# NVIDIA-NeMo/NeMo

Measured on AMD Instinct MI355X. Metric: audio-sec/s training throughput, Conformer-CTC-Large @ 1/2/4/8 MI355X, higher is better.
Workload: dtype bf16; 1 GPU; Conformer-CTC-Large bf16, batch=32x20s synthetic 16 kHz clips per GPU, 1xMI355X (BASELINE.json configs[1]); global_batch=32, parallelism=dp1

## Files before the change

include/mi355x_asr.h:

```cpp
#ifndef MI355X_ASR_H
#define MI355X_ASR_H
#ifdef __cplusplus
extern "C" {
#endif

#define MI355X_DT_F32 0
#define MI355X_DT_BF16 1

enum {
  MI355X_EPI_STORE = 0,
  MI355X_EPI_SWISH_DROP = 1,
  MI355X_EPI_RESID = 2,
  MI355X_EPI_DSWISH = 3,
  MI355X_EPI_RELU_MASK = 4,
  MI355X_EPI_MUL_POS = 5,
  MI355X_EPI_SWISH_DROP_G = 6,
  MI355X_EPI_DSWISH_G = 7
};
typedef struct mi355x_gemm_desc {
  const void* A; const void* B; void* C;
  int M, N, K;
  long long lda, ldb, ldc;
  long long c_col_stride;
  int transA, transB;
  int in_dtype;
  int c_dtype;
  int batch, nb0;
  long long sA0, sA1, sB0, sB1, sC0, sC1;
  const void* bias;
  float alpha;
  int epilogue;
  int atomic;
  int splitk;
  const void* aux_in; int aux_in_dtype;
  void* aux_out; int aux_out_dtype;
  long long ldaux;
  unsigned drop_key, drop_threshold; float drop_scale;
  const void* row_len; int rows_per_b; int rows_inner;
  long long colsum_stride;
  void* colsum_out;
  const struct mi355x_conv_gather* gather;
  const struct mi355x_row_map* rowmap;
} mi355x_gemm_desc;
typedef struct mi355x_conv_gather {
  int nI, nJ, SI, SJ, C, si, sj, ntaps; int di[9], dj[9];
  int operand;
} mi355x_conv_gather;
typedef struct mi355x_row_map { int nI, nJ, OI, OJ, si, sj, oi, oj; } mi355x_row_map;
int mi355x_gemm(const mi355x_gemm_desc* desc, void* stream);
int mi355x_gemm_config(int key, int value);
int mi355x_gemm_plan(const mi355x_gemm_desc* desc, int out[8]);
int mi355x_gemm_grouped(const mi355x_gemm_desc* descs, int n, void* stream);

int mi355x_ffn_fwd(const void* y, long long ldy, const void* w1_packed, const void* b1, const void* w2_packed, const void* b2,
                   const void* x_resid, long long ldx, void* h, long long ldh, void* out, long long ldo, int M, int d_model,
                   int d_ff, float alpha, unsigned drop_in_key, unsigned drop_in_threshold, float drop_in_scale,
                   unsigned drop_res_key, unsigned drop_res_threshold, float drop_res_scale, void* stream);
int mi355x_ffn_bwd_dgrad(const void* df, long long lddf, const void* w2t_packed, const void* w1t_packed, const void* h,
                         long long ldh, void* dh, void* act, void* dy, long long lddy, int M, int d_model, int d_ff,
                         unsigned drop_in_key, unsigned drop_in_threshold, float drop_in_scale, void* stream);

typedef struct mi355x_ffn_pack_entry { const void* src; void* k512; void* kchunk; int d_ff; int is_w2; } mi355x_ffn_pack_entry;
int mi355x_ffn_pack(const void* table_dev, int n_entries, int max_d_ff, void* stream);

int mi355x_logmel_fwd(const void* audio, const void* audio_len, const void* window, int win, int hop, int n_fft,
                      const void* fb_start, const void* fb_len, const void* fb_off, const void* fb_w, int n_mels,
                      float preemph, float dither, unsigned seed, float log_guard, void* out, int B, int S, int T,
                      void* stream);
int mi355x_logmel_config(int variant);
int mi355x_feat_normalize(const void* x, const void* seq_len, void* y, int y_dtype, int B, int n_mels, int T,
                          int normalize, float pad_value, void* stream);

int mi355x_subsample_conv1_fwd(const void* mel , const void* w , const void* bias,
                               void* out , int out_dtype, const void* len0, const void* len1, int B, int F,
                               int T, int C, void* stream);
int mi355x_subsample_conv1_bwd(const void* dout, int dtype, const void* mel, const void* len0, void* dw, void* db, int B,
                               int F, int T, int C, void* scratch ,
                               long long scratch_elems, void* stream);
int mi355x_im2col_3x3s2(const void* in , void* col , int dtype, int B, int T1, int F1, int C,
                        void* stream);
int mi355x_col2im_3x3s2_relu(const void* dcol, const void* act, void* din, int dtype, int B, int T1, int F1, int C,
                             void* stream);
int mi355x_subsample_conv1_fwd_pad(const void* mel, const void* w, const void* bias, void* out, int out_dtype, const void* len0,
                                   const void* len1, int B, int F, int T, int C, int pad, void* stream);
int mi355x_subsample_conv1_bwd_pad(const void* dout, int dtype, const void* mel, const void* len0, void* dw, void* db, int B,
                                   int F, int T, int C, int pad, void* scratch, long long scratch_elems, void* stream);
int mi355x_im2col_3x3s2_pad(const void* in, void* col, int dtype, int B, int T1, int F1, int C, int pad, void* stream);
int mi355x_col2im_3x3s2_relu_pad(const void* dcol, const void* act, void* din, int dtype, int B, int T1, int F1, int C, int pad,
                                 void* stream);

int mi355x_dwconv2d_s2_fwd(const void* in, const void* w, const void* bias, void* out, int dtype, int B, int T1, int F1, int C,
                           void* stream);
int mi355x_dwconv2d_s2_bwd(const void* dout, const void* in, const void* w, void* din, void* dw, void* dbias, int dtype, int B,
                           int T1, int F1, int C, void* scratch, long long scratch_elems, void* stream);
int mi355x_dwconv2d_s2_fwd_pad(const void* in, const void* w, const void* bias, void* out, int dtype, int B, int T1, int F1, int C,
                               int pad, void* stream);
int mi355x_dwconv2d_s2_bwd_pad(const void* dout, const void* in, const void* w, void* din, void* dw, void* dbias, int dtype, int B,
                               int T1, int F1, int C, int pad, void* scratch, long long scratch_elems, void* stream);

int mi355x_embed_sos_fwd(const void* targets , const void* emb , void* out, int dtype, int B, int U,
                         int H, int blank, void* stream);
int mi355x_embed_sos_bwd(const void* targets, const void* dx , int dtype, void* demb , int B, int U, int H,
                         int blank, void* stream);
int mi355x_lstm_cell_fwd(void* z, const void* b_hh, const void* c_prev, void* c, void* h, void* h_lp, int lp_dtype, int B, int H,
                         void* stream);
int mi355x_lstm_cell_bwd(const void* dh, void* dc, const void* act, const void* c, const void* c_prev, void* dz, int dz_dtype,
                         int B, int H, void* stream);
int mi355x_joint_combine_fwd(const void* f, const void* g, void* h, int dtype, unsigned drop_key, unsigned drop_threshold,
                             float drop_scale, int B, int T, int U1, int J, void* stream);
int mi355x_joint_combine_bwd(void* dh, const void* h, void* df, int dtype, float drop_scale, int B, int T, int U1, int J,
                             void* stream);
int mi355x_cast_rows(const void* src, long long ld_in, void* dst, int dst_dtype, long long ld_out, long long M, int N, int Np,
                     float alpha, void* stream);

int mi355x_scale_bias_fwd(const void* x, const void* scale, const void* bias, void* y, int y_dtype, long long M, int d, int ld,
                          void* stream);
int mi355x_scale_bias_bwd(const void* dy, int dy_dtype, int ld, const void* x, const void* scale, void* dres, void* dscale,
                          void* dbias, long long M, int d, void* scratch, long long scratch_elems, void* stream);
int mi355x_cast_pitched(const void* x, void* y, int y_dtype, long long M, int d, int ld, float alpha, unsigned drop_key,
                        unsigned drop_threshold, float drop_scale, void* stream);
int mi355x_swish_mask_fwd(const void* in, void* out, int dtype, const void* len, int T, long long M, int C, void* stream);
int mi355x_swish_mask_bwd(const void* in, const void* dout, void* din, int dtype, const void* len, int T, long long M, int C,
                          void* stream);
int mi355x_time_reduce_dwconv_fwd(const void* x, const void* len, const void* w, const void* bias, void* out, int out_dtype, int B,
                                  int T, int d, int ld, void* stream);
int mi355x_time_reduce_dwconv_bwd(const void* dout, int dout_dtype, int ld, const void* x, const void* len, const void* w, void* dx,
                                  void* dw, void* dbias, int B, int T, int d, void* stream);
int mi355x_time_recover_fwd(const void* skip, const void* ys, void* out, int B, int T, int d, void* stream);
int mi355x_time_recover_bwd(const void* dx, void* dys, int dys_dtype, int B, int T, int d, int ld, void* stream);

int mi355x_layernorm_fwd(const void* x, int x_dtype, const void* gamma, const void* beta, void* y, int y_dtype, void* mean,
                         void* rstd, int M, int d, float eps, void* stream);
int mi355x_layernorm2_fwd(const void* x, const void* gamma1, const void* beta1, void* y1, void* mean1, void* rstd1,
                          const void* gamma2, const void* beta2, void* y2, int y2_dtype, void* mean2, void* rstd2, int M, int d,
// ... 233 lines not shown
```

nemo_amd/_lib.py:

```python
from __future__ import annotations

import ctypes as C
import os

import torch

_HERE = os.path.dirname(os.path.abspath(__file__))
LIB_PATH = os.environ.get("MI355X_ASR_LIB", os.path.join(_HERE, "lib", "libmi355x_asr.so"))

vp, i32, i64, f32, f64, u32 = C.c_void_p, C.c_int, C.c_longlong, C.c_float, C.c_double, C.c_uint


class GemmDesc(C.Structure):
    _fields_ = [
        ("A", vp), ("B", vp), ("C", vp),
        ("M", i32), ("N", i32), ("K", i32),
        ("lda", i64), ("ldb", i64), ("ldc", i64), ("c_col_stride", i64),
        ("transA", i32), ("transB", i32),
        ("in_dtype", i32), ("c_dtype", i32),
        ("batch", i32), ("nb0", i32),
        ("sA0", i64), ("sA1", i64), ("sB0", i64), ("sB1", i64), ("sC0", i64), ("sC1", i64),
        ("bias", vp), ("alpha", f32),
        ("epilogue", i32), ("atomic", i32), ("splitk", i32),
        ("aux_in", vp), ("aux_in_dtype", i32),
        ("aux_out", vp), ("aux_out_dtype", i32),
        ("ldaux", i64),
        ("drop_key", u32), ("drop_threshold", u32), ("drop_scale", f32),
        ("row_len", vp), ("rows_per_b", i32), ("rows_inner", i32),
        ("colsum_stride", i64), ("colsum_out", vp),
        ("gather", vp), ("rowmap", vp),
    ]


class ConvGather(C.Structure):
    _fields_ = [("nI", i32), ("nJ", i32), ("SI", i32), ("SJ", i32), ("C", i32), ("si", i32), ("sj", i32), ("ntaps", i32),
                ("di", i32 * 9), ("dj", i32 * 9), ("operand", i32)]


class RowMap(C.Structure):
    _fields_ = [("nI", i32), ("nJ", i32), ("OI", i32), ("OJ", i32), ("si", i32), ("sj", i32), ("oi", i32), ("oj", i32)]


class FfnPackEntry(C.Structure):
    _fields_ = [("src", vp), ("k512", vp), ("kchunk", vp), ("d_ff", i32), ("is_w2", i32)]


class PackEntry(C.Structure):
    _fields_ = [
        ("src", vp), ("dst", vp),
        ("rows", i32), ("cols", i32), ("nr2", i32), ("nc2", i32),
        ("sr1", i64), ("sr2", i64), ("sc1", i64), ("sc2", i64), ("pitch", i64),
        ("tile_begin", i64),
    ]


SIGNATURES = {
    "mi355x_gemm": [C.POINTER(GemmDesc), vp],
    "mi355x_gemm_grouped": [C.POINTER(GemmDesc), i32, vp],
    "mi355x_gemm_config": [i32, i32],
    "mi355x_gemm_plan": [C.POINTER(GemmDesc), C.POINTER(i32 * 8)],
    "mi355x_set_step_counter": [vp],
    "mi355x_set_null_launch": [i32],
    "mi355x_ffn_fwd": [vp, i64, vp, vp, vp, vp, vp, i64, vp, i64, vp, i64, i32, i32, i32, f32, u32, u32, f32, u32, u32, f32, vp],
    "mi355x_ffn_pack": [vp, i32, i32, vp],
    "mi355x_ffn_bwd_dgrad": [vp, i64, vp, vp, vp, i64, vp, vp, vp, i64, i32, i32, i32, u32, u32, f32, vp],
    "mi355x_logmel_fwd": [vp, vp, vp, i32, i32, i32, vp, vp, vp, vp, i32, f32, f32, u32, f32, vp, i32, i32, i32, vp],
    "mi355x_feat_normalize": [vp, vp, vp, i32, i32, i32, i32, i32, f32, vp],
    "mi355x_subsample_conv1_fwd": [vp, vp, vp, vp, i32, vp, vp, i32, i32, i32, i32, vp],
    "mi355x_subsample_conv1_bwd": [vp, i32, vp, vp, vp, vp, i32, i32, i32, i32, vp, i64, vp],
    "mi355x_im2col_3x3s2": [vp, vp, i32, i32, i32, i32, i32, vp],
    "mi355x_col2im_3x3s2_relu": [vp, vp, vp, i32, i32, i32, i32, i32, vp],
    "mi355x_dwconv2d_s2_fwd": [vp, vp, vp, vp, i32, i32, i32, i32, i32, vp],
    "mi355x_dwconv2d_s2_bwd": [vp, vp, vp, vp, vp, vp, i32, i32, i32, i32, i32, vp, i64, vp],
    "mi355x_subsample_conv1_fwd_pad": [vp, vp, vp, vp, i32, vp, vp, i32, i32, i32, i32, i32, vp],
    "mi355x_subsample_conv1_bwd_pad": [vp, i32, vp, vp, vp, vp, i32, i32, i32, i32, i32, vp, i64, vp],
    "mi355x_im2col_3x3s2_pad": [vp, vp, i32, i32, i32, i32, i32, i32, vp],
    "mi355x_col2im_3x3s2_relu_pad": [vp, vp, vp, i32, i32, i32, i32, i32, i32, vp],
    "mi355x_dwconv2d_s2_fwd_pad": [vp, vp, vp, vp, i32, i32, i32, i32, i32, i32, vp],
    "mi355x_dwconv2d_s2_bwd_pad": [vp, vp, vp, vp, vp, vp, i32, i32, i32, i32, i32, i32, vp, i64, vp],
    "mi355x_embed_sos_fwd": [vp, vp, vp, i32, i32, i32, i32, i32, vp],
    "mi355x_embed_sos_bwd": [vp, vp, i32, vp, i32, i32, i32, i32, vp],
    "mi355x_lstm_cell_fwd": [vp, vp, vp, vp, vp, vp, i32, i32, i32, vp],
    "mi355x_lstm_cell_bwd": [vp, vp, vp, vp, vp, vp, i32, i32, i32, vp],
    "mi355x_joint_combine_fwd": [vp, vp, vp, i32, u32, u32, f32, i32, i32, i32, i32, vp],
    "mi355x_joint_combine_bwd": [vp, vp, vp, i32, f32, i32, i32, i32, i32, vp],
    "mi355x_cast_rows": [vp, i64, vp, i32, i64, i64, i32, i32, f32, vp],
    "mi355x_layernorm_fwd": [vp, i32, vp, vp, vp, i32, vp, vp, i32, i32, f32, vp],
    "mi355x_layernorm2_fwd": [vp, vp, vp, vp, vp, vp, vp, vp, vp, i32, vp, vp, i32, i32, f32, vp],
    "mi355x_layernorm2_bwd": [vp, i32, vp, vp, vp, vp, vp, vp, vp, vp, vp, vp, vp, vp, vp, vp, i32, i32, vp, f32, u32, u32, f32, vp],
    "mi355x_layernorm_bwd": [vp, i32, vp, i32, vp, vp, vp, vp, i32, vp, vp, i32, i32, vp],
    "mi355x_layernorm_bwd_cast": [vp, i32, vp, i32, vp, vp, vp, vp, i32, vp, vp, i32, i32, vp, f32, u32, u32, f32, vp],
    "mi355x_colsum": [vp, i32, i64, vp, i32, i32, f32, vp],
    "mi355x_log_softmax_fwd": [vp, i64, vp, i64, i32, i32, vp],
    "mi355x_log_softmax_bwd": [vp, vp, i64, vp, i32, i64, i32, i32, f32, vp],
    "mi355x_scale_bias_fwd": [vp, vp, vp, vp, i32, i64, i32, i32, vp],
    "mi355x_scale_bias_bwd": [vp, i32, i32, vp, vp, vp, vp, vp, i64, i32, vp, i64, vp],
    "mi355x_cast_pitched": [vp, vp, i32, i64, i32, i32, f32, u32, u32, f32, vp],
    "mi355x_swish_mask_fwd": [vp, vp, i32, vp, i32, i64, i32, vp],
    "mi355x_swish_mask_bwd": [vp, vp, vp, i32, vp, i32, i64, i32, vp],
    "mi355x_time_reduce_dwconv_fwd": [vp, vp, vp, vp, vp, i32, i32, i32, i32, i32, vp],
    "mi355x_time_reduce_dwconv_bwd": [vp, i32, i32, vp, vp, vp, vp, vp, vp, i32, i32, i32, vp],
    "mi355x_time_recover_fwd": [vp, vp, vp, i32, i32, i32, vp],
    "mi355x_time_recover_bwd": [vp, vp, i32, i32, i32, i32, i32, vp],
    "mi355x_glu_fwd": [vp, vp, i32, vp, i32, i64, i32, vp, vp],
    "mi355x_glu_bwd": [vp, vp, vp, i32, vp, i32, i64, i32, vp, vp],
    "mi355x_rows_pack": [vp, vp, i32, i64, i64, vp, vp, i32, i64, i32, i32, vp],
    "mi355x_drop_scale_cast": [vp, i32, vp, i32, i64, f32, u32, u32, f32, vp],
    "mi355x_qbias": [vp, i64, vp, vp, vp, vp, i32, i64, i32, vp],
    "mi355x_add2": [vp, vp, i32, vp, i32, i64, i64, i32, vp],
    "mi355x_ctc_greedy_decode": [vp, vp, vp, vp, vp, i32, i32, i32, i32, vp],
    "mi355x_ctc_greedy_decode_ts": [vp, vp, vp, vp, vp, vp, vp, i32, i32, i32, i32, vp],
    "mi355x_ctc_align": [vp, vp, vp, vp, vp, vp, vp, vp, vp, i32, i32, i32, i32, i32, vp],
    "mi355x_fill_rects": [vp, vp, i32, i32, i32, i32, f32, vp],
    "mi355x_specaug_rects": [vp, vp, vp, vp, vp, vp, i32, i32, i32, i32, i32, f32, i32, i32, vp],
    "mi355x_add2_colsum": [vp, vp, vp, i64, i64, i32, vp, vp, i64, vp],
    "mi355x_relpos_softmax_fwd": [vp, vp, vp, vp, i32, vp, i32, i32, i32, i32, i32, f32, u32, u32, f32, vp],
    "mi355x_relpos_softmax_fwd_ctx": [vp, vp, vp, vp, i32, vp, i32, i32, i32, i32, i32, f32, u32, u32, f32, i32, i32, i32, vp],
    "mi355x_relpos_softmax_bwd": [vp, i32, vp, vp, vp, i32, i32, i32, i32, i32, i32, f32, u32, u32, f32, vp],
    "mi355x_relpos_flash_fwd": [vp, i64, vp, i64, vp, vp, vp, vp, vp, i64, vp, i32, i32, i32, i32, i32, f32, u32, u32, f32, vp, vp],
    "mi355x_attn_delta": [vp, vp, vp, vp, i32, i32, i32, i32, vp, vp, vp],
    "mi355x_attn_bwd_prep": [vp, vp, vp, vp, vp, i64, vp, vp, vp, vp, i32, i32, i32, i32, vp, vp, vp],
    "mi355x_relpos_flash_bwd_dq": [vp, vp, vp, i64, vp, i64, vp, vp, vp, vp, vp, vp, vp, vp, i64, vp, vp, i64, i32, i32, i32, i32, i64,
                                   f32, u32, u32, f32, vp, vp],
    "mi355x_relpos_flash_bwd_dkv": [vp, vp, vp, i64, vp, i64, vp, vp, vp, vp, vp, i64, i32, i32, i32, i32, i32, f32, u32, u32, f32, vp, vp],
    "mi355x_relpos_flash_bwd_dpos": [vp, vp, vp, vp, i64, vp, vp, i64, i32, i32, i32, i32, i64, vp, vp],
    "mi355x_relpos_ds_elems": [i32, i32, i32],
    "mi355x_relpos_dpos_partial_elems": [i32, i32, i32],
    "mi355x_dwconv_fwd": [vp, vp, vp, vp, i32, vp, i32, i32, i32, i32, vp],
    "mi355x_dwconv_fwd_ctx": [vp, vp, vp, vp, i32, vp, i32, i32, i32, i32, i32, vp],
    "mi355x_dwconv_fwd_glu": [vp, vp, vp, vp, vp, vp, vp, i32, vp, i32, i32, i32, i32, i32, vp],
    "mi355x_dwconv_bwd": [vp, vp, vp, vp, vp, vp, i32, i32, i32, i32, i32, vp, i64, vp],
    "mi355x_dwconv_bwd_ctx": [vp, vp, vp, vp, vp, vp, i32, i32, i32, i32, i32, i32, vp, i64, vp],
    "mi355x_dwconv_bwd_bnswish": [vp, vp, vp, vp, vp, vp, vp, f64, vp, i32, vp, vp, vp, vp, vp, vp, vp, vp, vp, i32, i32, i32, i32, i32, i32, vp, i64, i32, vp],
    "mi355x_dwconv_tap_reduce": [vp, i64, i32, i32, i32, vp, vp, vp],
    "mi355x_bn_finalize": [vp, f64, vp, vp, vp, vp, f32, f32, i32, vp],
    "mi355x_bn_finalize_dev_count": [vp, vp, vp, vp, vp, vp, f32, f32, i32, vp],
    "mi355x_bn_eval_stats": [vp, vp, vp, vp, f32, i32, vp],
    "mi355x_bn_swish_fwd": [vp, vp, vp, vp, vp, vp, i32, i64, i32, vp],
    "mi355x_bn_swish_bwd_reduce": [vp, vp, vp, vp, vp, vp, vp, vp, vp, i32, i64, i32, vp, i64, vp],
    "mi355x_bn_stats_swish_fwd": [vp, vp, f64, vp, vp, vp, vp, vp, vp, vp, vp, f32, f32, i32, i64, i32, vp],
    "mi355x_bn_swish_bwd_apply": [vp, vp, vp, vp, vp, vp, vp, f64, i32, vp, i32, i64, i32, vp],
    "mi355x_bn_swish_bwd_apply_dev_count": [vp, vp, vp, vp, vp, vp, vp, vp, i32, vp, i32, i64, i32, vp],
    "mi355x_bn_param_grad": [vp, vp, vp, i32, vp],
# ... 83 lines not shown
```

nemo_amd/csrc/common.h:

```cpp
#pragma once
#include <hip/hip_runtime.h>
#include <stdint.h>

#define MI_OK 0
#define MI_ERR_ARG 1
#define MI_ERR_LAUNCH 2

#define MI_DT_F32 0
#define MI_DT_BF16 1

typedef uint16_t bf16_t;
typedef __attribute__((ext_vector_type(8))) __bf16 bf16x8;
typedef __attribute__((ext_vector_type(16))) float f32x16;
typedef __attribute__((ext_vector_type(4))) float f32x4;
typedef __attribute__((ext_vector_type(4))) uint32_t u32x4;
typedef __attribute__((ext_vector_type(2))) uint32_t u32x2;

static inline void mi_clear_errors() { (void)hipGetLastError(); }
static inline int mi_check_launch() {
  hipError_t e = hipGetLastError();
  return e == hipSuccess ? MI_OK : 1000 + (int)e;
}

extern "C" int mi355x_null_launch_flag;
// ... 98 lines not shown
  if (d.threshold == 0u) return 1.f;
  uint32_t s = drop_group_seed(d, idx >> 3);
  const uint32_t e = idx & 7u;
  for (uint32_t j = 0; j <= e; ++j) s = xorshift32(s);
  return s >= d.threshold ? d.scale : 0.f;
}
__device__ __forceinline__ void drop_mask8(const DropCfg& d, uint32_t idx8, float (&m)[8]) {
  if (d.threshold == 0u) {
#pragma unroll
    for (int j = 0; j < 8; ++j) m[j] = 1.f;
    return;
  }
  uint32_t s = drop_group_seed(d, idx8 >> 3);
#pragma unroll
  for (int j = 0; j < 8; ++j) { s = xorshift32(s); m[j] = s >= d.threshold ? d.scale : 0.f; }
}
__device__ __forceinline__ void drop_mask8u(const DropCfg& d, uint32_t idx, float (&m)[8]) {
  if (d.threshold == 0u || (idx & 7u) == 0u) { drop_mask8(d, idx, m); return; }
  if ((idx & 7u) == 4u) {
    uint32_t s = drop_group_seed(d, idx >> 3);
#pragma unroll
    for (int j = 0; j < 4; ++j) s = xorshift32(s);
#pragma unroll
    for (int j = 0; j < 4; ++j) { s = xorshift32(s); m[j] = s >= d.threshold ? d.scale : 0.f; }
    s = drop_group_seed(d, (idx >> 3) + 1u);
#pragma unroll
    for (int j = 0; j < 4; ++j) { s = xorshift32(s); m[4 + j] = s >= d.threshold ? d.scale : 0.f; }
    return;
  }
#pragma unroll
  for (int j = 0; j < 8; ++j) m[j] = drop_mask(d, idx + j);
}
__device__ __forceinline__ void drop_mask4u(const DropCfg& d, uint32_t idx, float (&m)[4]) {
  if (d.threshold == 0u) {
#pragma unroll
    for (int j = 0; j < 4; ++j) m[j] = 1.f;
    return;
  }
  const uint32_t o = idx & 7u;
  if (o == 0u || o == 4u) {
    uint32_t s = drop_group_seed(d, idx >> 3);
    if (o) {
#pragma unroll
      for (int j = 0; j < 4; ++j) s = xorshift32(s);
    }
#pragma unroll
    for (int j = 0; j < 4; ++j) { s = xorshift32(s); m[j] = s >= d.threshold ? d.scale : 0.f; }
    return;
  }
#pragma unroll
  for (int j = 0; j < 4; ++j) m[j] = drop_mask(d, idx + j);
}
__device__ __forceinline__ float hash_normal(uint32_t key, uint32_t idx) {
  uint32_t a = mix32(mix32(idx ^ key) + 0x9E3779B9u);
  uint32_t b = mix32(a ^ 0x85ebca6bU ^ (key * 0xc2b2ae35U));
  float u1 = ((float)(a >> 8) + 1.0f) * (1.0f / 16777217.0f);
  float u2 = (float)(b >> 8) * (1.0f / 16777216.0f);
  return sqrtf(-2.f * __logf(u1)) * __cosf(6.28318530718f * u2);
}

template <typename TT> struct VecIO;
template <> struct VecIO<bf16_t> {
  static constexpr int V = 8;
  static __device__ __forceinline__ void load(const bf16_t* p, float* dst) {
    const u32x4 t = *reinterpret_cast<const u32x4*>(p);
#pragma unroll
    for (int j = 0; j < 4; ++j) { dst[2 * j] = __uint_as_float(t[j] << 16); dst[2 * j + 1] = __uint_as_float(t[j] & 0xffff0000u); }
  }
  static __device__ __forceinline__ void store(bf16_t* p, const float* v) {
    u32x4 t = {pack_bf2(v[0], v[1]), pack_bf2(v[2], v[3]), pack_bf2(v[4], v[5]), pack_bf2(v[6], v[7])};
    *reinterpret_cast<u32x4*>(p) = t;
  }
};
template <> struct VecIO<float> {
  static constexpr int V = 4;
  static __device__ __forceinline__ void load(const float* p, float* dst) {
    const float4 t = *reinterpret_cast<const float4*>(p);
    dst[0] = t.x; dst[1] = t.y; dst[2] = t.z; dst[3] = t.w;
  }
  static __device__ __forceinline__ void store(float* p, const float* v) {
    *reinterpret_cast<float4*>(p) = make_float4(v[0], v[1], v[2], v[3]);
  }
};

static __global__ __launch_bounds__(256) void tap_reduce_kernel(const float* __restrict__ partial, int nparts, int KS, int d,
                                                                float* __restrict__ dw, float* __restrict__ dbias) {
  const int e = blockIdx.x * 256 + threadIdx.x;
  if (e >= (KS + 1) * d) return;
  const int k = e / d, c = e - k * d;
  const int per = (nparts + gridDim.y - 1) / gridDim.y;
  const int p0 = blockIdx.y * per, p1 = min(nparts, p0 + per);
  float a0 = 0.f, a1 = 0.f, a2 = 0.f, a3 = 0.f;
  const long long ps = (long long)(KS + 1) * d;
  const float* src = partial + (long long)k * d + c;
  int p = p0;
  for (; p + 4 <= p1; p += 4) {
    a0 += src[(p + 0) * ps]; a1 += src[(p + 1) * ps]; a2 += src[(p + 2) * ps]; a3 += src[(p + 3) * ps];
  }
  for (; p < p1; ++p) a0 += src[p * ps];
  const float acc = (a0 + a1) + (a2 + a3);
  if (k < KS) atomicAdd(dw + c * KS + k, acc);
  else if (dbias) atomicAdd(dbias + c, acc);
}

template <typename TOut>
static __global__ __launch_bounds__(256) void partials_reduce_kernel(const float* __restrict__ partial, int nparts, int n,
                                                                     TOut* __restrict__ out) {
  const int i = blockIdx.x * 256 + threadIdx.x;
  if (i >= n) return;
  const int per = (nparts + gridDim.y - 1) / gridDim.y;
  const int p0 = blockIdx.y * per, p1 = min(nparts, p0 + per);
  float a0 = 0.f, a1 = 0.f, a2 = 0.f, a3 = 0.f;
  int p = p0;
  for (; p + 4 <= p1; p += 4) {
    a0 += partial[(long long)(p + 0) * n + i]; a1 += partial[(long long)(p + 1) * n + i];
    a2 += partial[(long long)(p + 2) * n + i]; a3 += partial[(long long)(p + 3) * n + i];
  }
  for (; p < p1; ++p) a0 += partial[(long long)p * n + i];
  atomicAdd(out + i, (TOut)((a0 + a1) + (a2 + a3)));
}
```

nemo_amd/csrc/gemm.hip:

```cpp
#include <stdlib.h>
#include "common.h"
#include <atomic>
#include "mi355x_asr.h"

enum {
  EPI_STORE = 0,
  EPI_SWISH_DROP = 1,
  EPI_RESID = 2,
  EPI_DSWISH = 3,
  EPI_RELU_MASK = 4,
  EPI_MUL_POS = 5,
};

#define BM 128
#define BN 128
#define BK 64

struct GemmP {
  const void* A; const void* B; void* C;
  int M, N, K;
  long long lda, ldb, ldc, csc;
  int transA, transB;
  int batch, nb0;
  long long sA0, sA1, sB0, sB1, sC0, sC1;
  const float* bias; float alpha;
  int epi; int c_dt; int atomic;
  const void* aux_in; int auxin_dt; void* aux_out; int auxout_dt; long long ldaux;
  DropCfg drop;
  int swish_g;
  const long long* row_len; int rows_per_b; int rows_inner;
  int splitk; int ktiles_per_split;
  long long colsum_stride;
  float* colsum_out;
  int vec_ok;
  int v8_delay;
  int g_on, g_nI, g_nJ, g_SI, g_SJ, g_C, g_si, g_sj, g_ntaps;
  unsigned long long g_dip, g_djp;
  int r_on, r_nI, r_nJ, r_OI, r_OJ, r_si, r_sj, r_oi, r_oj;
};

__device__ __forceinline__ int tap_delta(unsigned long long packed, int tap) {
  return (int)((packed >> (__builtin_amdgcn_readfirstlane(tap) * 4)) & 15ull) - 8;
}

__device__ __forceinline__ int fdiv24(int m, int d, float inv_d) {
  int q = (int)((float)m * inv_d);
  const int r = m - q * d;
  q += (r >= d) - (r < 0);
  return q;
}
__device__ __forceinline__ long long crow(const GemmP& p, int m) {
  if (!p.r_on) return m;
  const int per_b = p.r_nI * p.r_nJ;
  int b, i;
  if ((unsigned)p.M < (1u << 24)) {
    b = fdiv24(m, per_b, __builtin_amdgcn_rcpf((float)per_b));
    const int r = m - b * per_b;
    i = fdiv24(r, p.r_nJ, __builtin_amdgcn_rcpf((float)p.r_nJ));
  } else {
    b = m / per_b;
    i = (m - b * per_b) / p.r_nJ;
  }
  const int r = m - b * per_b;
  const int j = r - i * p.r_nJ;
  return ((long long)b * p.r_OI + i * p.r_si + p.r_oi) * p.r_OJ + j * p.r_sj + p.r_oj;
}

__device__ __forceinline__ float ldx(const void* p, long long i, int dt) {
  return dt == MI_DT_F32 ? ((const float*)p)[i] : bf2f(((const bf16_t*)p)[i]);
}
__device__ __forceinline__ void stx(void* p, long long i, int dt, float v) {
  if (dt == MI_DT_F32) ((float*)p)[i] = v; else ((bf16_t*)p)[i] = f2bf(v);
}

__device__ __forceinline__ void swish_pair(float h, float dm, float& act, float& g) {
  const float s = sigmoidf_(h);
  const float sw = h * s;
  act = sw * dm;
  g = fmaf(sw, 1.f - s, s) * dm;
}

__device__ __forceinline__ void epilogue(const GemmP& p, int z, long long coff, int m, int n, float acc) {
  const long long mr = crow(p, m);
  const long long ci = coff + mr * p.ldc + (long long)n * p.csc;
  const long long ai = coff + mr * p.ldaux + n;
  float v = acc;
  if (p.bias) v += p.bias[n];
  const uint32_t didx = (uint32_t)z * (uint32_t)(p.M * p.N) + (uint32_t)m * (uint32_t)p.N + (uint32_t)n;
  switch (p.epi) {
    case EPI_STORE: v *= p.alpha * drop_mask(p.drop, didx); break;
    case EPI_SWISH_DROP:
      if (p.swish_g) {
        float a_, g_;
        swish_pair(v, drop_mask(p.drop, didx), a_, g_);
        stx(p.aux_out, ai, p.auxout_dt, g_);
        v = a_;
      } else {
        stx(p.aux_out, ai, p.auxout_dt, v);
        v = swishf_(v) * drop_mask(p.drop, didx);
      }
      break;
    case EPI_RESID:
      v = ((const float*)p.aux_in)[ai] + p.alpha * v * drop_mask(p.drop, didx);
      break;
    case EPI_DSWISH:
      v = p.swish_g ? v * ldx(p.aux_in, ai, p.auxin_dt) : v * drop_mask(p.drop, didx) * swish_grad(ldx(p.aux_in, ai, p.auxin_dt));
      break;
    case EPI_RELU_MASK: {
      int b = m / p.rows_per_b;
      int t = (m - b * p.rows_per_b) / p.rows_inner;
      v = (v > 0.f && (long long)t < p.row_len[b]) ? v : 0.f;
    } break;
    case EPI_MUL_POS: v = ldx(p.aux_in, ai, p.auxin_dt) > 0.f ? v : 0.f; break;
  }
  if (p.atomic) atomicAdd(&((float*)p.C)[ci], v);
  else stx(p.C, ci, p.c_dt, v);
}

__device__ __forceinline__ void ld8x(const void* p, long long i, int dt, float (&v)[8]) {
  if (dt == MI_DT_F32) {
    const float4 a = *reinterpret_cast<const float4*>((const float*)p + i);
    const float4 b = *reinterpret_cast<const float4*>((const float*)p + i + 4);
    v[0] = a.x; v[1] = a.y; v[2] = a.z; v[3] = a.w; v[4] = b.x; v[5] = b.y; v[6] = b.z; v[7] = b.w;
  } else {
    const u32x4 t = *reinterpret_cast<const u32x4*>((const bf16_t*)p + i);
#pragma unroll
    for (int j = 0; j < 4; ++j) { v[2 * j] = __uint_as_float(t[j] << 16); v[2 * j + 1] = __uint_as_float(t[j] & 0xffff0000u); }
  }
}
__device__ __forceinline__ void st8x(void* p, long long i, int dt, const float (&v)[8]) {
  if (dt == MI_DT_F32) {
    *reinterpret_cast<float4*>((float*)p + i) = make_float4(v[0], v[1], v[2], v[3]);
    *reinterpret_cast<float4*>((float*)p + i + 4) = make_float4(v[4], v[5], v[6], v[7]);
  } else {
    u32x4 t = {pack_bf2(v[0], v[1]), pack_bf2(v[2], v[3]), pack_bf2(v[4], v[5]), pack_bf2(v[6], v[7])};
    *reinterpret_cast<u32x4*>((bf16_t*)p + i) = t;
  }
}
__device__ __forceinline__ void epilogue8(const GemmP& p, int z, long long coff, int m, int n, float (&v)[8]) {
  const long long mr = crow(p, m);
  const long long ci = coff + mr * p.ldc + n;
  const long long ai = coff + mr * p.ldaux + n;
  if (p.bias) {
    float b[8];
    ld8x(p.bias, n, MI_DT_F32, b);
#pragma unroll
    for (int j = 0; j < 8; ++j) v[j] += b[j];
  }
// ... 81 lines not shown
  if (p.bias) {
    float b[4];
    ld4x(p.bias, n, MI_DT_F32, b);
#pragma unroll
    for (int j = 0; j < 4; ++j) v[j] += b[j];
  }
  const uint32_t didx = (uint32_t)z * (uint32_t)(p.M * p.N) + (uint32_t)m * (uint32_t)p.N + (uint32_t)n;
  float dm[4];
  drop_mask4u(p.drop, didx, dm);
  switch (p.epi) {
    case EPI_STORE:
#pragma unroll
      for (int j = 0; j < 4; ++j) v[j] *= p.alpha * dm[j];
      break;
    case EPI_SWISH_DROP:
      if (p.swish_g) {
        float g[4];
#pragma unroll
        for (int j = 0; j < 4; ++j) swish_pair(v[j], dm[j], v[j], g[j]);
        st4x(p.aux_out, ai, p.auxout_dt, g);
      } else {
        st4x(p.aux_out, ai, p.auxout_dt, v);
#pragma unroll
        for (int j = 0; j < 4; ++j) v[j] = swishf_(v[j]) * dm[j];
      }
      break;
    case EPI_RESID: {
      float r[4];
      ld4x(p.aux_in, ai, MI_DT_F32, r);
#pragma unroll
      for (int j = 0; j < 4; ++j) v[j] = r[j] + p.alpha * v[j] * dm[j];
    } break;
    case EPI_DSWISH: {
      float h[4];
      ld4x(p.aux_in, ai, p.auxin_dt, h);
      if (p.swish_g) {
#pragma unroll
        for (int j = 0; j < 4; ++j) v[j] *= h[j];
      } else {
#pragma unroll
        for (int j = 0; j < 4; ++j) v[j] = v[j] * dm[j] * swish_grad(h[j]);
      }
    } break;
    case EPI_RELU_MASK: {
      const int b = m / p.rows_per_b;
      const int t = (m - b * p.rows_per_b) / p.rows_inner;
      const bool ok = (long long)t < p.row_len[b];
#pragma unroll
      for (int j = 0; j < 4; ++j) v[j] = (ok && v[j] > 0.f) ? v[j] : 0.f;
    } break;
    case EPI_MUL_POS: {
      float h[4];
      ld4x(p.aux_in, ai, p.auxin_dt, h);
#pragma unroll
      for (int j = 0; j < 4; ++j) v[j] = h[j] > 0.f ? v[j] : 0.f;
    } break;
  }
  if (p.atomic) {
#pragma unroll
    for (int j = 0; j < 4; ++j) atomicAdd(&((float*)p.C)[ci + j], v[j]);
  } else {
    st4x(p.C, ci, p.c_dt, v);
  }
}
__device__ __forceinline__ void epilogue_chunk(const GemmP& p, int z, long long coff, int m, int n, float (&v)[8]) {
  const int nv = p.N - n;
  if ((p.vec_ok & 1) && nv >= 8) { epilogue8(p, z, coff, m, n, v); return; }
  int j0 = 0;
  if ((p.vec_ok & 2) && nv >= 4) {
    float w[4] = {v[0], v[1], v[2], v[3]};
    epilogue4(p, z, coff, m, n, w);
    j0 = 4;
    if ((p.vec_ok & 2) && nv >= 8) {
      float w2[4] = {v[4], v[5], v[6], v[7]};
      epilogue4(p, z, coff, m, n + 4, w2);
      return;
    }
  }
  for (int j = j0; j < 8; ++j)
    if (n + j < p.N) epilogue(p, z, coff, m, n + j, v[j]);
}


template <int EPI, int ITERS, int ROW_STEP, int TW = BN, bool UNAL = false, bool PART = false>
__device__ __forceinline__ void fast_epilogue(const GemmP& p, const float* sC, int z, long long coff, int m_first, int n0,
                                              int row_l0) {
  constexpr int LDS_C = TW + 4;
  constexpr bool AUX_IN = EPI == EPI_RESID || EPI == EPI_DSWISH || EPI == EPI_MUL_POS;
  const int c8 = (threadIdx.x & (TW / 8 - 1)) * 8;
  const int n = n0 + c8;
  if (PART) {
    if (n >= p.N) return;
    if (n + 8 > p.N) {
#pragma unroll 2
      for (int it = 0; it < ITERS; ++it) {
        const int m = m_first + it * ROW_STEP;
        if (m >= p.M) break;
        const float4 a = *reinterpret_cast<const float4*>(sC + (row_l0 + it * ROW_STEP) * LDS_C + c8);
        float w[4] = {a.x, a.y, a.z, a.w};
        epilogue4(p, z, coff, m, n, w);
      }
      return;
    }
  }
  float b8[8];
  if (p.bias) ld8x(p.bias, n, MI_DT_F32, b8);
  else {
#pragma unroll
    for (int j = 0; j < 8; ++j) b8[j] = 0.f;
  }
  const uint32_t dbase = (uint32_t)z * (uint32_t)(p.M * p.N) + (uint32_t)n;
  const bool lin = (EPI != EPI_MUL_POS) || !p.r_on;
  const long long ci_l = coff + (long long)m_first * p.ldc + n, ai_l = coff + (long long)m_first * p.ldaux + n;
  const long long ci_s = (long long)ROW_STEP * p.ldc, ai_s = (long long)ROW_STEP * p.ldaux;
  const uint32_t db_l = dbase + (uint32_t)m_first * (uint32_t)p.N, db_s = (uint32_t)ROW_STEP * (uint32_t)p.N;
  float aux[AUX_IN ? ITERS : 1][8];
  if (AUX_IN) {
#pragma unroll
    for (int it = 0; it < ITERS; ++it) {
      const int m = m_first + it * ROW_STEP;
      const long long ai0 = lin ? ai_l + it * ai_s : coff + crow(p, m) * p.ldaux + n;
      if (m < p.M) ld8x(p.aux_in, ai0, EPI == EPI_RESID ? MI_DT_F32 : p.auxin_dt, aux[it]);
    }
  }
  float4 ra[ITERS], rb[ITERS];
#pragma unroll
  for (int it = 0; it < ITERS; ++it) {
    const float* src = sC + (row_l0 + it * ROW_STEP) * LDS_C + c8;
    if (TW == 256) {
      const int hi = (threadIdx.x >> 4) & 1;
      const float4 x = *reinterpret_cast<const float4*>(src + 4 * hi);
      const float4 y = *reinterpret_cast<const float4*>(src + 4 * (1 - hi));
      ra[it] = hi ? y : x; rb[it] = hi ? x : y;
    } else {
      ra[it] = *reinterpret_cast<const float4*>(src);
      rb[it] = *reinterpret_cast<const float4*>(src + 4);
    }
  }
#pragma unroll
  for (int it = 0; it < ITERS; ++it) {
    const int m = m_first + it * ROW_STEP;
    if (m >= p.M) continue;
    const float4 a = ra[it], b = rb[it];
    float v[8] = {a.x + b8[0], a.y + b8[1], a.z + b8[2], a.w + b8[3], b.x + b8[4], b.y + b8[5], b.z + b8[6], b.w + b8[7]};
    float dm[8];
    if (UNAL) drop_mask8u(p.drop, db_l + (uint32_t)it * db_s, dm);
    else drop_mask8(p.drop, db_l + (uint32_t)it * db_s, dm);
    const long long mrow = lin ? 0 : crow(p, m);
    const long long ci = lin ? ci_l + it * ci_s : coff + mrow * p.ldc + n;
    const long long ai = lin ? ai_l + it * ai_s : coff + mrow * p.ldaux + n;
    if (EPI == EPI_STORE) {
#pragma unroll
      for (int j = 0; j < 8; ++j) v[j] *= p.alpha * dm[j];
    } else if (EPI == EPI_SWISH_DROP) {
      if (p.swish_g) {
        float g[8];
#pragma unroll
        for (int j = 0; j < 8; ++j) swish_pair(v[j], dm[j], v[j], g[j]);
        st8x(p.aux_out, ai, p.auxout_dt, g);
      } else {
        st8x(p.aux_out, ai, p.auxout_dt, v);
#pragma unroll
        for (int j = 0; j < 8; ++j) v[j] = swishf_(v[j]) * dm[j];
      }
    } else if (EPI == EPI_RESID) {
#pragma unroll
      for (int j = 0; j < 8; ++j) v[j] = aux[AUX_IN ? it : 0][j] + p.alpha * v[j] * dm[j];
    } else if (EPI == EPI_DSWISH) {
      if (p.swish_g) {
#pragma unroll
        for (int j = 0; j < 8; ++j) v[j] *= aux[AUX_IN ? it : 0][j];
      } else {
#pragma unroll
        for (int j = 0; j < 8; ++j) v[j] = v[j] * dm[j] * swish_grad(aux[AUX_IN ? it : 0][j]);
      }
    } else if (EPI == EPI_RELU_MASK) {
      const int bb = m / p.rows_per_b;
      const int t = (m - bb * p.rows_per_b) / p.rows_inner;
      const bool ok = (long long)t < p.row_len[bb];
#pragma unroll
      for (int j = 0; j < 8; ++j) v[j] = (ok && v[j] > 0.f) ? v[j] : 0.f;
    } else {
#pragma unroll
      for (int j = 0; j < 8; ++j) v[j] = aux[AUX_IN ? it : 0][j] > 0.f ? v[j] : 0.f;
    }
#if defined(V8_EPI_ABL) && V8_EPI_ABL == 3
    asm volatile("" :: "v"(v[0]), "v"(v[1]), "v"(v[2]), "v"(v[3]), "v"(v[4]), "v"(v[5]), "v"(v[6]), "v"(v[7]), "v"(ci));
#else
    st8x(p.C, ci, p.c_dt, v);
#endif
  }
}
template <int ITERS, int ROW_STEP, int TW = BN, bool UNAL = false, bool PART = false>
__device__ __forceinline__ void fast_epilogue_any(const GemmP& p, const float* sC, int z, long long coff, int m_first, int n0,
                                                  int row_l0) {
  switch (p.epi) {
    case EPI_STORE: fast_epilogue<EPI_STORE, ITERS, ROW_STEP, TW, UNAL, PART>(p, sC, z, coff, m_first, n0, row_l0); break;
    case EPI_SWISH_DROP: fast_epilogue<EPI_SWISH_DROP, ITERS, ROW_STEP, TW, UNAL, PART>(p, sC, z, coff, m_first, n0, row_l0); break;
    case EPI_RESID: fast_epilogue<EPI_RESID, ITERS, ROW_STEP, TW, UNAL, PART>(p, sC, z, coff, m_first, n0, row_l0); break;
    case EPI_DSWISH: fast_epilogue<EPI_DSWISH, ITERS, ROW_STEP, TW, UNAL, PART>(p, sC, z, coff, m_first, n0, row_l0); break;
    case EPI_RELU_MASK: fast_epilogue<EPI_RELU_MASK, ITERS, ROW_STEP, TW, UNAL, PART>(p, sC, z, coff, m_first, n0, row_l0); break;
    default: fast_epilogue<EPI_MUL_POS, ITERS, ROW_STEP, TW, UNAL, PART>(p, sC, z, coff, m_first, n0, row_l0); break;
  }
}


__device__ __forceinline__ int lds_off(int r, int chunk) {
  return r * BK + ((chunk ^ ((r >> 1) & 7)) << 3);
}

struct StageN { u32x4 v[4]; };
__device__ __forceinline__ void load_n(StageN& s, const bf16_t* base, long long ld, int row0, int rows, int k0, int K) {
#pragma unroll
  for (int i = 0; i < 4; ++i) {
    const int q = threadIdx.x + i * 256;
    const int r = q >> 3, ck = q & 7;
    const int gr = row0 + r, gk = k0 + ck * 8;
    u32x4 v = {0u, 0u, 0u, 0u};
    if (gr < rows && gk < K) v = *reinterpret_cast<const u32x4*>(base + (long long)gr * ld + gk);
    s.v[i] = v;
  }
}
__device__ __forceinline__ void store_n(const StageN& s, bf16_t* lds) {
#pragma unroll
  for (int i = 0; i < 4; ++i) {
    const int q = threadIdx.x + i * 256;
    const int r = q >> 3, ck = q & 7;
    *reinterpret_cast<u32x4*>(lds + lds_off(r, ck)) = s.v[i];
  }
}
typedef __attribute__((address_space(3))) void lds_void_t;
typedef const __attribute__((address_space(1))) void glb_void_t;
__device__ __attribute__((aligned(16))) uint32_t g_zero16[4] = {0u, 0u, 0u, 0u};
__device__ __forceinline__ void glds_n(const bf16_t* base, long long ld, int row0, int rows, int k0, int K, bf16_t* lds_tile) {
  const int wave = threadIdx.x >> 6;
#pragma unroll
  for (int i = 0; i < 4; ++i) {
    const int q = threadIdx.x + i * 256;
    const int r = q >> 3, ck = q & 7;
    const int gck = ck ^ ((r >> 1) & 7);
    int gr = row0 + r;
    gr = gr < rows ? gr : rows - 1;
    const int gk = k0 + gck * 8;
    const bf16_t* src = (gk < K) ? base + (long long)gr * ld + gk : reinterpret_cast<const bf16_t*>(g_zero16);
    bf16_t* dst = lds_tile + (wave * 64 + i * 256) * 8;
    __builtin_amdgcn_global_load_lds((glb_void_t*)src, (lds_void_t*)dst, 16, 0, 0);
  }
}
struct StageT { u32x4 v[4]; };
__device__ __forceinline__ void load_t(StageT& s, const bf16_t* base, long long ld, int col0, int cols, int k0, int K) {
  const int g = threadIdx.x & 15, c = threadIdx.x >> 4;
  const int gc = col0 + c * 8;
#pragma unroll
  for (int j = 0; j < 4; ++j) {
    const int gk = k0 + g * 4 + j;
    u32x4 v = {0u, 0u, 0u, 0u};
    if (gk < K && gc < cols) v = *reinterpret_cast<const u32x4*>(base + (long long)gk * ld + gc);
    s.v[j] = v;
  }
}
__device__ __forceinline__ void store_t(const StageT& s, bf16_t* lds) {
  const int g = threadIdx.x & 15, c = threadIdx.x >> 4;
#pragma unroll
  for (int e = 0; e < 8; ++e) {
    const int w = e >> 1, hi = e & 1;
    uint32_t x0 = s.v[0][w], x1 = s.v[1][w], x2 = s.v[2][w], x3 = s.v[3][w];
    uint32_t lo01, lo23;
// ... 251 lines not shown
    g.row[c] = m;
    g.off[c] = ((b * p.g_SI + g.i[c] * p.g_si) * p.g_SJ + g.j[c] * p.g_sj) * p.g_C + (g.colok[c] ? gc : 0);
  }
}
template <int R>
__device__ __forceinline__ void gatherT_issue(DmaGatherT<R>& g, const GemmP& p, const bf16_t* base, int tap,
                                              bf16_t* lds_tile, const bool load = true ) {
  const int wave = threadIdx.x >> 6;
  const int di = tap_delta(p.g_dip, tap), dj = tap_delta(p.g_djp, tap);
  const int toff = (di * p.g_SJ + dj) * p.g_C;
  const int step_j = BK * p.g_sj * p.g_C;
  const int wrap_j = p.g_si * p.g_SJ * p.g_C - p.g_nJ * p.g_sj * p.g_C;
  const int wrap_i = p.g_SI * p.g_SJ * p.g_C - p.g_nI * p.g_si * p.g_SJ * p.g_C;
#pragma unroll
  for (int c = 0; c < DmaGatherT<R>::PER; ++c) {
    const int si = g.i[c] * p.g_si + di, sj = g.j[c] * p.g_sj + dj;
    const bool ok = g.colok[c] && g.row[c] < p.K && (unsigned)si < (unsigned)p.g_SI && (unsigned)sj < (unsigned)p.g_SJ;
    const bf16_t* src = ok ? base + (g.off[c] + toff) : reinterpret_cast<const bf16_t*>(g_zero16);
    bf16_t* dst = lds_tile + (wave * 64 + c * 512) * 8;
    if (load) __builtin_amdgcn_global_load_lds((glb_void_t*)src, (lds_void_t*)dst, 16, 0, 0);
    g.row[c] += BK; g.j[c] += BK; g.off[c] += step_j;
    while (g.j[c] >= p.g_nJ) { g.j[c] -= p.g_nJ; ++g.i[c]; g.off[c] += wrap_j; }
    while (g.i[c] >= p.g_nI) { g.i[c] -= p.g_nI; g.off[c] += wrap_i; }
  }
}

template <int R>
__device__ __forceinline__ void dma_issue(const DmaSrc<R>& d, int it, int k0, int K, bool ktail, bf16_t* lds_tile) {
  const int wave = threadIdx.x >> 6;
  const bool tail = ktail && (k0 + BK > K);
  const unsigned long long zero = (unsigned long long)(const void*)g_zero16;
#pragma unroll
  for (int i = 0; i < DmaSrc<R>::PER; ++i) {
    unsigned long long src = (unsigned long long)(const void*)(d.ptr[i] + (long long)it * d.step[i]);
    if (tail) src = (k0 + d.kin[i] < K) ? src : zero;
    bf16_t* dst = lds_tile + (wave * 64 + i * 512) * 8;
    __builtin_amdgcn_global_load_lds((glb_void_t*)src, (lds_void_t*)dst, 16, 0, 0);
  }
}

template <bool T, int R>
__device__ __forceinline__ bf16x8 frag_v2(const bf16_t* tile, int row_tile, int kk, int lane) {
  if (!T) {
    return *reinterpret_cast<const bf16x8*>(tile + lds_off(row_tile + (lane & 31), kk * 2 + (lane >> 5)));
  } else {
    const int t = lane & 15, g4 = (lane >> 4) & 1, lh = lane >> 5;
    const int col = row_tile + g4 * 16 + (t & 3) * 4;
    union { bf16x8 v; s16x4 h[2]; } u;
#pragma unroll
    for (int r = 0; r < 2; ++r) {
      const int krow = kk * 16 + lh * 8 + r * 4 + (t >> 2);
      const int off = krow * R + ((((col >> 3) ^ ((t >> 2) << 2))) << 3) + (col & 7);
      u.h[r] = __builtin_amdgcn_ds_read_tr16_b64_v4i16((lds_s16x4_t*)(tile + off));
    }
    return u.v;
  }
}

typedef __attribute__((address_space(3))) const char lds_cchar_t;
__device__ __forceinline__ uint32_t lds_addr(const void* p) { return (uint32_t)(uintptr_t)(lds_cchar_t*)p; }
union FragU { bf16x8 v; s16x4 h[2]; };
template <int OFF>
__device__ __forceinline__ void tr_rd(s16x4& dst, uint32_t addr) {
  asm volatile("ds_read_b64_tr_b16 %0, %1 offset:%2" : "=v"(dst) : "v"(addr), "i"(OFF) : "memory");
}
template <int R>
__device__ __forceinline__ uint32_t tr_base(const bf16_t* tile, int row_tile, int lane) {
  const int t = lane & 15, g4 = (lane >> 4) & 1, lh = lane >> 5;
  const int col = row_tile + g4 * 16 + (t & 3) * 4;
  const int krow = lh * 8 + (t >> 2);
  return lds_addr(tile) + (uint32_t)((krow * R + ((((col >> 3) ^ ((t >> 2) << 2))) << 3) + (col & 7)) * 2);
}
template <int R, int KK>
__device__ __forceinline__ void tr_frag_rd(FragU& f, uint32_t base) {
  tr_rd<(KK * 16) * R * 2>(f.h[0], base);
  tr_rd<(KK * 16 + 4) * R * 2>(f.h[1], base);
}
__device__ __forceinline__ u32x2 lds_rd64_sync(uint32_t addr) {
  u32x2 v;
  asm volatile("ds_read_b64 %0, %1\n\ts_waitcnt lgkmcnt(0)" : "=v"(v) : "v"(addr) : "memory");
  return v;
}

template <bool TA, bool TB, bool REG = false>
__device__ __forceinline__ void gemm_v2_body(const GemmP& p, bf16_t* smem2, const int bid, const int kslice, const int z
                                             , const bool direct = false
) {
  const int tn = (p.N + BN - 1) / BN, tm = (p.M + BM2 - 1) / BM2;
  const int ntiles = tm * tn;
  const int q8 = ntiles >> 3, r8 = ntiles & 7;
  const int xcd = bid & 7, idx = bid >> 3;
  const int logical = direct ? bid : (xcd < r8 ? xcd * (q8 + 1) : r8 * (q8 + 1) + (xcd - r8) * q8) + idx;
  const int tile_m = logical / tn, tile_n = logical - tile_m * tn;
  const int m0 = tile_m * BM2, n0 = tile_n * BN;
  const int z0 = z % p.nb0, z1 = z / p.nb0;
  const bf16_t* A = (const bf16_t*)p.A + z0 * p.sA0 + z1 * p.sA1;
  const bf16_t* B = (const bf16_t*)p.B + z0 * p.sB0 + z1 * p.sB1;
  const long long coff = z0 * p.sC0 + z1 * p.sC1;
  const int nk_total = (p.K + BK - 1) / BK;
  int kt0 = 0, kt1 = nk_total;
  if (p.splitk > 1) {
    kt0 = kslice * p.ktiles_per_split;
    kt1 = min(nk_total, kt0 + p.ktiles_per_split);
    if (kt0 >= kt1) return;
  }
#ifdef GEMM_ABLATE
  const int dbg = p.vec_ok >> 8;
  const int nk = (dbg & 2) ? 0 : kt1 - kt0;
#else
  const int nk = kt1 - kt0;
#endif
  const int lane = threadIdx.x & 63, wave = threadIdx.x >> 6;
  const int wm = wave >> 1, wn = wave & 1;
  const int lr = lane & 31, lh = lane >> 5;

  f32x16 acc[2][2];
#pragma unroll
  for (int i = 0; i < 2; ++i)
#pragma unroll
    for (int j = 0; j < 2; ++j)
#pragma unroll
      for (int r = 0; r < 16; ++r) acc[i][j][r] = 0.f;

  DmaSrc<BM2> dA;
  DmaSrc<BN> dB;
  DmaGather<BM2> gA;
  const bool gatherA = !TA && p.g_on == 1;
  if (gatherA) gather_setup<BM2>(gA, p, A, m0);
  else dma_setup<TA, BM2>(dA, A, p.lda, m0, p.M, kt0 * BK);
  DmaGatherT<BN> gB;
  const bool gatherB = TB && p.g_on == 2;
  if (gatherB) gatherT_setup<BN>(gB, p, n0, p.N, kt0 * BK);
  else dma_setup<TB, BN>(dB, B, p.ldb, n0, p.N, kt0 * BK);
  const bool ktail = (p.K & (BK - 1)) != 0;
  auto issue_a = [&](int it) {
    bf16_t* st = smem2 + (it % 3) * NT2_STAGE;
    if (gatherA) gather_issue<BM2>(gA, p, kt0 + it, st);
    else dma_issue<BM2>(dA, it, (kt0 + it) * BK, p.K, ktail, st);
  };
  auto issue_b = [&](int it) {
    bf16_t* st = smem2 + (it % 3) * NT2_STAGE;
    if (gatherB) gatherT_issue<BN>(gB, p, (const bf16_t*)p.B, z0, st + BM2 * BK);
    else dma_issue<BN>(dB, it, (kt0 + it) * BK, p.K, ktail, st + BM2 * BK);
  };
  auto issue = [&](int it) { issue_a(it); issue_b(it); };
  const int cs_step = tn < 8 ? tn : 8;
  const bool do_colsum = TA && p.colsum_out != nullptr && tile_n < cs_step;
  float csum[4] = {0.f, 0.f, 0.f, 0.f};

  constexpr bool PIPELINED = TA && TB;
  if constexpr (REG) {
  static_assert(!REG || (!TA && !TB), "register prefetch: K-contiguous operands");
  const char* Ab = (const char*)A + (long long)kt0 * (BK * 2);
  const char* Bb = (const char*)B + (long long)kt0 * (BK * 2);
  uint32_t oa[4], ob[2];
#pragma unroll
  for (int i = 0; i < 4; ++i) {
    const int q = threadIdx.x + i * 512;
    const int r = q >> 3, ck = q & 7;
    const int gck = ck ^ ((r >> 1) & 7);
    int ga = m0 + r; ga = ga < p.M ? ga : p.M - 1;
    oa[i] = (uint32_t)((long long)ga * p.lda + gck * 8) * 2u;
    if (i < 2) {
      int gb = n0 + r; gb = gb < p.N ? gb : p.N - 1;
      ob[i] = (uint32_t)((long long)gb * p.ldb + gck * 8) * 2u;
    }
  }
// ... 167 lines not shown
      } else
#endif
#pragma unroll
      for (int i = 0; i < 2; ++i)
#pragma unroll
        for (int j = 0; j < 2; ++j)
          acc[i][j] = __builtin_amdgcn_mfma_f32_32x32x16_bf16(af[kk][i], bfr[kk][j], acc[i][j], 0, 0, 0);
    }
    if (TA && do_colsum) {
      const int col = lane * 4;
      for (int kr = tile_n; kr < 8; kr += cs_step) {
        const int krow = wave * 8 + kr;
        const int off = krow * BM2 + (((col >> 3) ^ ((krow & 3) << 2)) << 3) + (col & 7);
        const u32x2 v = *reinterpret_cast<const u32x2*>(a_s + off);
        csum[0] += __uint_as_float(v[0] << 16); csum[1] += __uint_as_float(v[0] & 0xffff0000u);
        csum[2] += __uint_as_float(v[1] << 16); csum[3] += __uint_as_float(v[1] & 0xffff0000u);
      }
    }
    if (it + 2 < nk) asm volatile("s_waitcnt vmcnt(6)" ::: "memory"); else asm volatile("s_waitcnt vmcnt(0)" ::: "memory");
    asm volatile("s_waitcnt lgkmcnt(0)" ::: "memory");
    __builtin_amdgcn_s_barrier();
  }

  }

  float* sC = reinterpret_cast<float*>(smem2);
#ifdef GEMM_ABLATE
  if (dbg & 1) {
    float sacc = 0.f;
#pragma unroll
    for (int i = 0; i < 2; ++i)
#pragma unroll
      for (int j = 0; j < 2; ++j)
#pragma unroll
        for (int r = 0; r < 16; ++r) sacc += acc[i][j][r];
    if (sacc == 123.456f) ((float*)p.C)[0] = sacc;
    return;
  }
#endif
  if (TA && do_colsum) {
#pragma unroll
    for (int e = 0; e < 4; ++e) sC[wave * BM2 + lane * 4 + e] = csum[e];
    __syncthreads();
    if (threadIdx.x < BM2) {
      float v = 0.f;
#pragma unroll
      for (int w = 0; w < 8; ++w) v += sC[w * BM2 + threadIdx.x];
      const int m = m0 + threadIdx.x;
      if (m < p.M) atomicAdd(p.colsum_out + z0 * p.colsum_stride + m, v);
    }
    __syncthreads();
  }

  constexpr int LDS_C = BN + 4;
#pragma unroll
  for (int i = 0; i < 2; ++i)
#pragma unroll
    for (int j = 0; j < 2; ++j)
#pragma unroll
      for (int r = 0; r < 16; ++r) {
        const int row_l = wm * 64 + i * 32 + (r & 3) + 8 * (r >> 2) + 4 * lh;
        sC[row_l * LDS_C + wn * 64 + j * 32 + lr] = acc[i][j][r];
      }
  __syncthreads();
  if (p.atomic) {
    const bool plain = p.epi == EPI_STORE && !p.bias && p.alpha == 1.f && p.drop.threshold == 0u && !p.r_on;
    if (plain) {
      float* Cb = (float*)p.C + coff;
#pragma unroll 4
      for (int e = threadIdx.x; e < BM2 * BN; e += 512) {
        const int row_l = e >> 7, col = e & (BN - 1);
        const int m = m0 + row_l, n = n0 + col;
        if (m < p.M && n < p.N) atomicAdd(Cb + (long long)m * p.ldc + (long long)n * p.csc, sC[row_l * LDS_C + col]);
      }
    } else {
      for (int e = threadIdx.x; e < BM2 * BN; e += 512) {
        const int row_l = e >> 7, col = e & (BN - 1);
        const int m = m0 + row_l, n = n0 + col;
        if (m < p.M && n < p.N) epilogue(p, z, coff, m, n, sC[row_l * LDS_C + col]);
      }
    }
    return;
  }
  if ((p.vec_ok & 1) && !(p.N & 3)) {
    if (n0 + BN <= p.N) {
      if (p.N & 7) fast_epilogue_any<8, 32, BN, true>(p, sC, z, coff, m0 + (threadIdx.x >> 4), n0, threadIdx.x >> 4);
      else fast_epilogue_any<8, 32>(p, sC, z, coff, m0 + (threadIdx.x >> 4), n0, threadIdx.x >> 4);
      return;
    }
    if (p.vec_ok & 2) {
      fast_epilogue_any<8, 32, BN, true, true>(p, sC, z, coff, m0 + (threadIdx.x >> 4), n0, threadIdx.x >> 4);
      return;
    }
  }
#pragma unroll 2
  for (int it = 0; it < 8; ++it) {
    const int row_l = (threadIdx.x >> 4) + 32 * it;
    const int c8 = (threadIdx.x & 15) * 8;
    const int m = m0 + row_l, n = n0 + c8;
    if (m < p.M && n < p.N) {
      float v[8];
      const float4 a = *reinterpret_cast<const float4*>(sC + row_l * LDS_C + c8);
      const float4 b = *reinterpret_cast<const float4*>(sC + row_l * LDS_C + c8 + 4);
      v[0] = a.x; v[1] = a.y; v[2] = a.z; v[3] = a.w; v[4] = b.x; v[5] = b.y; v[6] = b.z; v[7] = b.w;
      epilogue_chunk(p, z, coff, m, n, v);
    }
  }
}

template <bool TA, bool TB, bool REG = false>
__global__ __launch_bounds__(512) void gemm_bf16_v2_kernel(GemmP p) {
  drop_resolve(p.drop);
  extern __shared__ __attribute__((aligned(16))) bf16_t smem2[];
  gemm_v2_body<TA, TB, REG>(p, smem2, blockIdx.x, blockIdx.y, blockIdx.z);
}

#define GRP_MAX 40
struct GroupP {
  const void* A[GRP_MAX]; const void* B[GRP_MAX]; void* C[GRP_MAX]; float* colsum[GRP_MAX];
  int M[GRP_MAX], N[GRP_MAX];
  long long lda[GRP_MAX], ldb[GRP_MAX], ldc[GRP_MAX];
  int tile_begin[GRP_MAX + 1];
  int n, K, splitk, ktiles_per_split;
};
__global__ __launch_bounds__(512) void gemm_bf16_grouped_tn_kernel(GroupP g) {
  extern __shared__ __attribute__((aligned(16))) bf16_t smem2[];
  int pi = 0;
  const int tiles_total = g.tile_begin[g.n];
  const int W = tiles_total * g.splitk;
  const int L = (int)blockIdx.y * (int)gridDim.x + (int)blockIdx.x;
  const int q8w = W >> 3, r8w = W & 7, xw = L & 7;
  const int w = (xw < r8w ? xw * (q8w + 1) : r8w * (q8w + 1) + (xw - r8w) * q8w) + (L >> 3);
  while (pi + 1 < g.n && w >= g.splitk * g.tile_begin[pi + 1]) ++pi;
  const int ntile_p = g.tile_begin[pi + 1] - g.tile_begin[pi];
  const int rel = w - g.splitk * g.tile_begin[pi];
  const int exp_ks = rel / ntile_p, exp_tile = rel - exp_ks * ntile_p;
  GemmP p;
  p.A = g.A[pi]; p.B = g.B[pi]; p.C = g.C[pi];
  p.M = g.M[pi]; p.N = g.N[pi]; p.K = g.K;
  p.lda = g.lda[pi]; p.ldb = g.ldb[pi]; p.ldc = g.ldc[pi]; p.csc = 1;
  p.transA = 1; p.transB = 1; p.batch = 1; p.nb0 = 1;
  p.sA0 = p.sA1 = p.sB0 = p.sB1 = p.sC0 = p.sC1 = 0;
  p.bias = nullptr; p.alpha = 1.f; p.epi = EPI_STORE; p.c_dt = MI_DT_F32; p.atomic = 1; p.swish_g = 0;
  p.aux_in = nullptr; p.auxin_dt = 0; p.aux_out = nullptr; p.auxout_dt = 0; p.ldaux = 0;
  p.drop.key = 0u; p.drop.threshold = 0u; p.drop.scale = 1.f; p.drop.step = nullptr;
  p.row_len = nullptr; p.rows_per_b = 1; p.rows_inner = 1;
  p.splitk = g.splitk; p.ktiles_per_split = g.ktiles_per_split;
  p.colsum_stride = 0; p.colsum_out = g.colsum[pi];
  p.vec_ok = 0; p.g_on = 0; p.r_on = 0;
  gemm_v2_body<true, true>(p, smem2, exp_tile, exp_ks, 0, true);
}

#define BN4 256
#define NT4_STAGE ((BM2 + BN4) * BK)

__device__ __forceinline__ void v4_round_out(const GemmP& p, const float* sC, int z, long long coff, int m0, int n0, int rbase,
                                          bool fast, const int hstride = 128) {
  constexpr int LDS_C = BN4 + 4;
  if (fast) {
    const int rl0 = threadIdx.x >> 5;
    fast_epilogue_any<2, 16, BN4>(p, sC, z, coff, m0 + rbase + rl0, n0, rl0);
    fast_epilogue_any<2, 16, BN4>(p, sC + 32 * LDS_C, z, coff, m0 + hstride + rbase + rl0, n0, rl0);
  } else if (p.atomic) {
    const bool plain = p.epi == EPI_STORE && !p.bias && p.alpha == 1.f && p.drop.threshold == 0u && !p.r_on;
    float* Cb = (float*)p.C + coff;
#pragma unroll 4
    for (int e = threadIdx.x; e < 64 * BN4; e += 512) {
      const int rl = e >> 8, col = e & (BN4 - 1);
      const int m = m0 + (rl >> 5) * hstride + rbase + (rl & 31), n = n0 + col;
      if (m < p.M && n < p.N) {
        if (plain) atomicAdd(Cb + (long long)m * p.ldc + (long long)n * p.csc, sC[rl * LDS_C + col]);
        else epilogue(p, z, coff, m, n, sC[rl * LDS_C + col]);
      }
    }
  } else {
    for (int it = 0; it < 4; ++it) {
      const int rl = (threadIdx.x >> 5) + 16 * it;
      const int c8 = (threadIdx.x & 31) * 8;
      const int m = m0 + (rl >> 5) * hstride + rbase + (rl & 31), n = n0 + c8;
      if (m < p.M && n < p.N) {
        float v[8];
        const float4 a = *reinterpret_cast<const float4*>(sC + rl * LDS_C + c8);
        const float4 b = *reinterpret_cast<const float4*>(sC + rl * LDS_C + c8 + 4);
        v[0] = a.x; v[1] = a.y; v[2] = a.z; v[3] = a.w; v[4] = b.x; v[5] = b.y; v[6] = b.z; v[7] = b.w;
        epilogue_chunk(p, z, coff, m, n, v);
      }
    }
  }
}

__device__ __forceinline__ void v4_tile_epilogue(const GemmP& p, f32x16 (&acc)[4][2], float* sC, int z, long long coff, int m0,
                                                 int n0, int wm, int wn, int lr, int lh) {
  constexpr int LDS_C = BN4 + 4;
  const bool fast = (p.vec_ok & 1) && !(p.N & 7) && n0 + BN4 <= p.N && !p.atomic;
#pragma nounroll
  for (int i = 0; i < 4; ++i) {
    f32x16 t0, t1;
// ... 324 lines not shown
  auto step_spread = [&](RegTile& t, int wr, int rd, int next_it) {
    const bf16_t* a_s = smem6 + rd * NT4_STAGE;
    const bf16_t* b_s = a_s + BM2 * BK;
    bf16_t* st = smem6 + wr * NT4_STAGE;
    const bool in = next_it < nk;
    const uint32_t msk = in ? 0xffffffffu : 0u;
    const char* ga = in ? A + (long long)next_it * (BK * 2) : reinterpret_cast<const char*>(g_zero16);
    const char* gb = in ? B + (long long)next_it * (BK * 2) : reinterpret_cast<const char*>(g_zero16);
#pragma unroll
    for (int kk = 0; kk < 4; ++kk) {
      bf16x8 af[4], bfr[2];
#pragma unroll
      for (int j = 0; j < 2; ++j) bfr[j] = frag_v2<false, BN4>(b_s, wn * 64 + j * 32, kk, lane);
#pragma unroll
      for (int i = 0; i < 4; ++i) af[i] = frag_v2<false, BM2>(a_s, wm * 128 + i * 32, kk, lane);
#pragma unroll
      for (int c = 0; c < 2; ++c) {
        const int i = (kk & 1) * 2 + c;
        if (kk < 2) {
          *reinterpret_cast<u32x4*>(st + (threadIdx.x + i * 512) * 8) = t.a[i];
          t.a[i] = *reinterpret_cast<const u32x4*>(ga + (oa[i] & msk));
        } else {
          *reinterpret_cast<u32x4*>(st + BM2 * BK + (threadIdx.x + i * 512) * 8) = t.b[i];
          t.b[i] = *reinterpret_cast<const u32x4*>(gb + (ob[i] & msk));
        }
      }
#pragma unroll
      for (int i = 0; i < 4; ++i)
#pragma unroll
        for (int j = 0; j < 2; ++j)
          acc[i][j] = __builtin_amdgcn_mfma_f32_32x32x16_bf16(af[i], bfr[j], acc[i][j], 0, 0, 0);
      __builtin_amdgcn_sched_barrier(0);
    }
  };

  RegTile r0, r1;
  load_tile(r0, 0);
  load_tile(r1, 1);
  store_tile(r0, 0);
  load_tile(r0, 2);
  __syncthreads();
  for (int it = 0; it < nk; it += 2) {
    if constexpr (G == 1) {
      step_spread(r1, 1, 0, it + 3);
      __syncthreads();
      step_spread(r0, 0, 1, it + 4);
      __syncthreads();
    } else {
      store_tile(r1, 1);
      load_tile(r1, it + 3);
      compute(0);
      __syncthreads();
      store_tile(r0, 0);
      load_tile(r0, it + 4);
      compute(1);
      __syncthreads();
    }
  }
  v4_tile_epilogue(p, acc, reinterpret_cast<float*>(smem6), z, coff, m0, n0, wm, wn, lr, lh);
}

#define V8_HALF_B 16384
#define V8_BUF_B 65536
#ifdef V8_TRACE
__device__ unsigned long long* g_v8_trace = nullptr;
extern "C" int mi355x_gemm_debug_trace(void* buf) {
  return hipMemcpyToSymbol(HIP_SYMBOL(g_v8_trace), &buf, sizeof(buf)) == hipSuccess ? 0 : 1;
}
#define V8_STAMP(i)                                                                                              \
  if (g_v8_trace && threadIdx.x == 0) {                                                                          \
    unsigned long long tr_, tc_;                                                                                 \
    asm volatile("s_memrealtime %0\n\ts_memtime %1\n\ts_waitcnt lgkmcnt(0)" : "=s"(tr_), "=s"(tc_)::"memory");  \
    const int wg_ = blockIdx.x + gridDim.x * (blockIdx.y + gridDim.y * blockIdx.z);                              \
    g_v8_trace[wg_ * 16 + 2 * (i)] = tr_; g_v8_trace[wg_ * 16 + 2 * (i) + 1] = tc_;                              \
  }
#else
#define V8_STAMP(i)
#endif
template <int OFF>
__device__ __forceinline__ void v8_rd128(bf16x8& dst, uint32_t addr) {
  asm volatile("ds_read_b128 %0, %1 offset:%2" : "=v"(dst) : "v"(addr), "n"(OFF) : "memory");
}

template <int EPI>
__device__ __forceinline__ void v8_round_fast(const GemmP& p, const float* win, const float (&b8)[8], int z, long long coff, int m_base,
                                              int hstride, int n0) {
  constexpr bool AUX_IN = EPI == EPI_RESID || EPI == EPI_DSWISH || EPI == EPI_MUL_POS;
  const int k = threadIdx.x & 31, rl0 = threadIdx.x >> 5;
  const int n = n0 + k * 8;
  const bool lin = (EPI != EPI_MUL_POS) || !p.r_on;
  int mrow[4];
  long long ci[4], ai[4];
#pragma unroll
  for (int it = 0; it < 4; ++it) {
    mrow[it] = m_base + (it >> 1) * hstride + rl0 + 16 * (it & 1);
    const long long mr = lin ? (long long)mrow[it] : crow(p, mrow[it] < p.M ? mrow[it] : p.M - 1);
    ci[it] = coff + mr * p.ldc + n;
    ai[it] = coff + mr * p.ldaux + n;
  }
  float aux[AUX_IN ? 4 : 1][8];
  if (AUX_IN) {
#pragma unroll
    for (int it = 0; it < 4; ++it)
      if (mrow[it] < p.M) ld8x(p.aux_in, ai[it], EPI == EPI_RESID ? MI_DT_F32 : p.auxin_dt, aux[it]);
  }
  const int hi = (threadIdx.x >> 4) & 1, sw = rl0 & 7;
  float4 x[4], y[4];
#pragma unroll
  for (int it = 0; it < 4; ++it) {
    const float* row = win + (rl0 + 16 * it) * 256;
    x[it] = *reinterpret_cast<const float4*>(row + (((2 * k + hi) ^ sw) << 2));
    y[it] = *reinterpret_cast<const float4*>(row + (((2 * k + 1 - hi) ^ sw) << 2));
  }
  const uint32_t dbase = (uint32_t)z * (uint32_t)(p.M * p.N) + (uint32_t)n;
#pragma unroll
  for (int it = 0; it < 4; ++it) {
    const int m = mrow[it];
    if (m >= p.M) continue;
    const float4 a = hi ? y[it] : x[it], b = hi ? x[it] : y[it];
    float v[8] = {a.x + b8[0], a.y + b8[1], a.z + b8[2], a.w + b8[3], b.x + b8[4], b.y + b8[5], b.z + b8[6], b.w + b8[7]};
    float dm[8];
    drop_mask8(p.drop, dbase + (uint32_t)m * (uint32_t)p.N, dm);
    if (EPI == EPI_STORE) {
#pragma unroll
      for (int j = 0; j < 8; ++j) v[j] *= p.alpha * dm[j];
    } else if (EPI == EPI_SWISH_DROP) {
      if (p.swish_g) {
        float g[8];
#pragma unroll
        for (int j = 0; j < 8; ++j) swish_pair(v[j], dm[j], v[j], g[j]);
        st8x(p.aux_out, ai[it], p.auxout_dt, g);
      } else {
        st8x(p.aux_out, ai[it], p.auxout_dt, v);
#pragma unroll
        for (int j = 0; j < 8; ++j) v[j] = swishf_(v[j]) * dm[j];
      }
    } else if (EPI == EPI_RESID) {
#pragma unroll
      for (int j = 0; j < 8; ++j) v[j] = aux[AUX_IN ? it : 0][j] + p.alpha * v[j] * dm[j];
    } else if (EPI == EPI_DSWISH) {
      if (p.swish_g) {
#pragma unroll
        for (int j = 0; j < 8; ++j) v[j] *= aux[AUX_IN ? it : 0][j];
      } else {
#pragma unroll
        for (int j = 0; j < 8; ++j) v[j] = v[j] * dm[j] * swish_grad(aux[AUX_IN ? it : 0][j]);
      }
    } else if (EPI == EPI_RELU_MASK) {
      const int bb = m / p.rows_per_b;
      const int t = (m - bb * p.rows_per_b) / p.rows_inner;
      const bool ok = (long long)t < p.row_len[bb];
#pragma unroll
      for (int j = 0; j < 8; ++j) v[j] = (ok && v[j] > 0.f) ? v[j] : 0.f;
    } else {
#pragma unroll
      for (int j = 0; j < 8; ++j) v[j] = aux[AUX_IN ? it : 0][j] > 0.f ? v[j] : 0.f;
    }
#if defined(V8_EPI_ABL) && V8_EPI_ABL == 3
    asm volatile("" :: "v"(v[0]), "v"(v[1]), "v"(v[2]), "v"(v[3]), "v"(v[4]), "v"(v[5]), "v"(v[6]), "v"(v[7]), "v"(ci[it]));
#else
    st8x(p.C, ci[it], p.c_dt, v);
#endif
  }
}

#define V8_ES_SWISH_G_DROP 1
#define V8_ES_SWISH_G 2
#define V8_ES_DSWISH_G 3
#define V8_ES_STORE 4
template <int OFF>
__device__ __forceinline__ void v8_rdw(f32x4& dst, uint32_t addr) {
  asm volatile("ds_read_b128 %0, %1 offset:%2" : "=v"(dst) : "v"(addr), "n"(OFF) : "memory");
}
template <int EPI, bool DROP, bool FULL>
__device__ __forceinline__ void v8_round_spec(const GemmP& p, const float* win, const float (&b8)[8], int z, long long coff, int m_base,
                                              int n0) {
  static_assert(EPI == EPI_STORE || EPI == EPI_SWISH_DROP || EPI == EPI_DSWISH, "specialised kinds");
  const int k = threadIdx.x & 31, rl0 = threadIdx.x >> 5;
  const uint32_t vC = (uint32_t)(rl0 * p.ldc + k * 8) * 2u, vA = (uint32_t)(rl0 * p.ldaux + k * 8) * 2u;
  u32x4 h4[EPI == EPI_DSWISH ? 4 : 1];
  if (EPI == EPI_DSWISH) {
#pragma unroll
    for (int it = 0; it < 4; ++it) {
      const int ro = (it >> 1) * 64 + 16 * (it & 1);
      if (FULL || m_base + ro + rl0 < p.M)
        h4[EPI == EPI_DSWISH ? it : 0] =
            *reinterpret_cast<const u32x4*>((const char*)p.aux_in + (coff + (long long)(m_base + ro) * p.ldaux + n0) * 2 + vA);
    }
  }
  const int hi = (threadIdx.x >> 4) & 1, sw = rl0 & 7;
  const uint32_t wrow = lds_addr(win) + (uint32_t)rl0 * 1024u;
  const uint32_t ax = wrow + (uint32_t)(((2 * k + hi) ^ sw) << 4), ay = wrow + (uint32_t)(((2 * k + 1 - hi) ^ sw) << 4);
  f32x4 x[4], y[4];
  v8_rdw<0>(x[0], ax); v8_rdw<0>(y[0], ay);
  v8_rdw<16384>(x[1], ax); v8_rdw<16384>(y[1], ay);
  v8_rdw<32768>(x[2], ax); v8_rdw<32768>(y[2], ay);
  v8_rdw<49152>(x[3], ax); v8_rdw<49152>(y[3], ay);
  if (!FULL)
    asm volatile("s_waitcnt lgkmcnt(0)" : "+v"(x[0]), "+v"(y[0]), "+v"(x[1]), "+v"(y[1]), "+v"(x[2]), "+v"(y[2]), "+v"(x[3]), "+v"(y[3]) : : "memory");
  const uint32_t d0 = (uint32_t)z * (uint32_t)(p.M * p.N) + (uint32_t)(n0 + k * 8) + (uint32_t)(m_base + rl0) * (uint32_t)p.N;
#pragma unroll
  for (int it = 0; it < 4; ++it) {
    const int ro = (it >> 1) * 64 + 16 * (it & 1);
    if (!FULL && m_base + ro + rl0 >= p.M) continue;
    if (FULL) {
      if (it == 0) asm volatile("s_waitcnt lgkmcnt(6)" : "+v"(x[0]), "+v"(y[0]) : : "memory");
      else if (it == 1) asm volatile("s_waitcnt lgkmcnt(4)" : "+v"(x[1]), "+v"(y[1]) : : "memory");
      else if (it == 2) asm volatile("s_waitcnt lgkmcnt(2)" : "+v"(x[2]), "+v"(y[2]) : : "memory");
      else asm volatile("s_waitcnt lgkmcnt(0)" : "+v"(x[3]), "+v"(y[3]) : : "memory");
    }
    const f32x4 a = hi ? y[it] : x[it], b = hi ? x[it] : y[it];
    float v[8] = {a[0] + b8[0], a[1] + b8[1], a[2] + b8[2], a[3] + b8[3], b[0] + b8[4], b[1] + b8[5], b[2] + b8[6], b[3] + b8[7]};
    float dm[8];
    if (DROP) {
      uint32_t s = drop_group_seed(p.drop, (d0 + (uint32_t)ro * (uint32_t)p.N) >> 3);
#pragma unroll
      for (int j = 0; j < 8; ++j) { s = xorshift32(s); dm[j] = s >= p.drop.threshold ? p.drop.scale : 0.f; }
    } else {
#pragma unroll
      for (int j = 0; j < 8; ++j) dm[j] = 1.f;
    }
    if (EPI == EPI_STORE) {
#pragma unroll
      for (int j = 0; j < 8; ++j) v[j] *= p.alpha * dm[j];
    } else if (EPI == EPI_SWISH_DROP) {
      float g[8];
#pragma unroll
      for (int j = 0; j < 8; ++j) swish_pair(v[j], dm[j], v[j], g[j]);
      const u32x4 t = {pack_bf2(g[0], g[1]), pack_bf2(g[2], g[3]), pack_bf2(g[4], g[5]), pack_bf2(g[6], g[7])};
      *reinterpret_cast<u32x4*>((char*)p.aux_out + (coff + (long long)(m_base + ro) * p.ldaux + n0) * 2 + vA) = t;
    } else {
      const u32x4 t = h4[EPI == EPI_DSWISH ? it : 0];
#pragma unroll
      for (int j = 0; j < 4; ++j) {
        v[2 * j] *= __uint_as_float(t[j] << 16);
        v[2 * j + 1] *= __uint_as_float(t[j] & 0xffff0000u);
      }
    }
    const u32x4 t = {pack_bf2(v[0], v[1]), pack_bf2(v[2], v[3]), pack_bf2(v[4], v[5]), pack_bf2(v[6], v[7])};
    *reinterpret_cast<u32x4*>((char*)p.C + (coff + (long long)(m_base + ro) * p.ldc + n0) * 2 + vC) = t;
  }
}

template <int G, bool TN, int AH = 2, int ES = 0>
__device__ __forceinline__ void gemm_v8_body(const GemmP& p, bf16_t* smem8, const int tile_m, const int tile_n, const int kslice,
                                             const int z) {
  const int tn = (p.N + BN4 - 1) / BN4;
  static_assert(AH == 2 || (AH == 1 && G == 0 && !TN), "the one-A-half tile: dense K-contiguous operands");
  constexpr int BMT = 128 * AH;
  constexpr int BUF_B = (AH + 2) * V8_HALF_B;
  const int m0 = tile_m * BMT, n0 = tile_n * BN4;
  const int z0 = z % p.nb0, z1 = z / p.nb0;
  const bf16_t* A = (const bf16_t*)p.A + z0 * p.sA0 + z1 * p.sA1;
  const bf16_t* B = (const bf16_t*)p.B + z0 * p.sB0 + z1 * p.sB1;
  const long long coff = z0 * p.sC0 + z1 * p.sC1;
  if constexpr (!TN) {
    const bool mask_tile = p.epi == EPI_RELU_MASK && !p.r_on;
    const bool gate_tile = p.epi == EPI_MUL_POS && p.row_len != nullptr;
    if ((mask_tile || gate_tile) && p.splitk <= 1 && !p.aux_out && p.c_dt == MI_DT_BF16 && p.csc == 1 && (p.vec_ok & 1) && !(p.N & 7)) {
      const int mlast = min(m0 + BMT, p.M) - 1;
      const int b0 = m0 / p.rows_per_b, b1 = mlast / p.rows_per_b;
      const int t0 = (m0 - b0 * p.rows_per_b) / p.rows_inner;
      if (b0 == b1 && (long long)t0 >= p.row_len[b0]) {
        bf16_t* Cz = (bf16_t*)p.C + coff;
        const int ncol = min(BN4, p.N - n0), nrow = mlast - m0 + 1, cpr = ncol >> 3;
        const u32x4 zero = {0u, 0u, 0u, 0u};
        for (int e = threadIdx.x; e < nrow * cpr; e += 512) {
          const int r = e / cpr, c = e - r * cpr;
          *reinterpret_cast<u32x4*>(Cz + crow(p, m0 + r) * p.ldc + n0 + c * 8) = zero;
        }
        return;
      }
    }
  }
  const int nk_total = (p.K + BK - 1) / BK;
  int kt0 = 0, kt1 = nk_total;
  if (p.splitk > 1) {
    kt0 = kslice * p.ktiles_per_split;
    kt1 = min(nk_total, kt0 + p.ktiles_per_split);
    if (kt0 >= kt1) return;
  }
  const int nk = kt1 - kt0;
  const int lane = threadIdx.x & 63;
  const int wave = __builtin_amdgcn_readfirstlane(threadIdx.x >> 6);
  const int wm = wave >> 2, wn = wave & 3;

  f32x4 acc[AH][4][2][2];
#pragma unroll
  for (int h = 0; h < AH; ++h)
#pragma unroll
    for (int mi = 0; mi < 4; ++mi)
#pragma unroll
      for (int hb = 0; hb < 2; ++hb)
#pragma unroll
        for (int ni = 0; ni < 2; ++ni) acc[h][mi][hb][ni] = f32x4{0.f, 0.f, 0.f, 0.f};

  uint32_t oA[2][2], oB[2][2], gin[2][2];
  uint32_t okbits = 0u;
  int g2i[2], g2j[2], g2off[2], g2row[2];
#pragma unroll
  for (int h = 0; h < 2; ++h)
#pragma unroll
    for (int i = 0; i < 2; ++i) {
      const int q = threadIdx.x + i * 512;
      gin[h][i] = 0u;
      if constexpr (!TN) {
        const int r = q >> 3, gck = (q & 7) ^ ((r >> 1) & 7);
        int ga = m0 + h * 128 + r; ga = ga < p.M ? ga : p.M - 1;
        int gb = n0 + h * 128 + r; gb = gb < p.N ? gb : p.N - 1;
        oB[h][i] = (uint32_t)((long long)gb * p.ldb + gck * 8) * 2u;
        if constexpr (G == 1) {
          const int per_b = p.g_nI * p.g_nJ;
          const int b = ga / per_b, rr = ga - b * per_b;
          const int oi = rr / p.g_nJ, oj = rr - oi * p.g_nJ;
          const int gi = oi * p.g_si, gj = oj * p.g_sj;
          oA[h][i] = (uint32_t)((((long long)b * p.g_SI + gi) * p.g_SJ + gj) * p.g_C + gck * 8) * 2u;
          uint32_t in = 0u;
          for (int t = 0; t < p.g_ntaps; ++t) {
            const int di = tap_delta(p.g_dip, t), dj = tap_delta(p.g_djp, t);
            if ((unsigned)(gi + di) < (unsigned)p.g_SI && (unsigned)(gj + dj) < (unsigned)p.g_SJ) in |= 1u << t;
          }
          gin[h][i] = in;
        } else {
          oA[h][i] = (uint32_t)((long long)ga * p.lda + gck * 8) * 2u;
        }
      } else {
        const int k = q >> 4, c = (q & 15) ^ ((k & 3) << 2) ^ (((k >> 3) & 1) << 1);
        const int ga = m0 + h * 128 + c * 8, gb = n0 + h * 128 + c * 8;
        if (ga < p.M) okbits |= 1u << (h * 2 + i);
        if (gb < p.N) okbits |= 16u << (h * 2 + i);
        oA[h][i] = (uint32_t)((long long)k * p.lda + ga) * 2u;
        if constexpr (G == 2) {
          oB[h][i] = (uint32_t)gb * 2u;
          if (h == 0) {
            const int m = kt0 * BK + k;
            const int per_b = p.g_nI * p.g_nJ;
            const int b = m / per_b, rr = m - b * per_b;
            g2i[i] = rr / p.g_nJ;
            g2j[i] = rr - g2i[i] * p.g_nJ;
            g2row[i] = m;
            g2off[i] = ((b * p.g_SI + g2i[i] * p.g_si) * p.g_SJ + g2j[i] * p.g_sj) * p.g_C;
          }
        } else {
          oB[h][i] = (uint32_t)((long long)k * p.ldb + gb) * 2u;
        }
      }
// ... 231 lines not shown
  stage(0, 0, true, 0); stage(1, 0, true, 0); stage(2, 0, true, 0);
  stage(0, 1, true, 1); stage(1, 1, true, 1); stage(2, 1, true, 1);
  asm volatile("s_waitcnt vmcnt(6)" ::: "memory");
  __builtin_amdgcn_s_barrier();
  V8_STAMP(1);
  if (wm == 1) __builtin_amdgcn_s_barrier();
  __builtin_amdgcn_sched_barrier(0);
  int bcur = 0, bnew = 2;
#pragma nounroll
  for (int t = 0; t < nk; ++t) {
    const uint32_t bo = (uint32_t)bcur * BUF_B;
    const uint32_t ra[4] = {fra[0] + bo, fra[1] + bo, 0u, 0u};
    const uint32_t rb[2] = {frb[0] + bo, frb[1] + bo};
    V8_RD_B(0);
    V8_RD_A(0);
    if (t + 2 < nk) stage(0, t + 2, true, bnew);
    __builtin_amdgcn_sched_barrier(0);
    __builtin_amdgcn_s_barrier();
    asm volatile("s_waitcnt lgkmcnt(0)" : V8_PIN_A, V8_PIN_B(0) : : "memory");
    V8_MM(0, 0);
    V8_RD_B(1);
    if (t + 2 < nk) {
      stage(2, t + 2, true, bnew);
      stage(1, t + 2, true, bnew);
      asm volatile("s_waitcnt vmcnt(6)" ::: "memory");
    } else {
      asm volatile("s_waitcnt vmcnt(0)" ::: "memory");
    }
    __builtin_amdgcn_sched_barrier(0);
    __builtin_amdgcn_s_barrier();
    asm volatile("s_waitcnt lgkmcnt(0)" : V8_PIN_B(1) : : "memory");
    V8_MM(0, 1);
    bcur = bcur == 2 ? 0 : bcur + 1;
    bnew = bnew == 2 ? 0 : bnew + 1;
  }
  }
  if (wm == 0) __builtin_amdgcn_s_barrier();
#undef V8_FRAG_A
#undef V8_FRAG_B
#undef V8_RD_A
#undef V8_RD_B
#undef V8_PIN_A
#undef V8_PIN_B
#undef V8_MM
  __syncthreads();
  V8_STAMP(2);

  float* sC = reinterpret_cast<float*>(smem8);
  if (do_colsum) {
#pragma unroll
    for (int e = 0; e < 4; ++e) sC[wave * BM2 + lane * 4 + e] = csum[e];
    __syncthreads();
    if (threadIdx.x < BM2) {
      float v = 0.f;
#pragma unroll
      for (int w = 0; w < 8; ++w) v += sC[w * BM2 + threadIdx.x];
      const int m = m0 + threadIdx.x;
      if (m < p.M) atomicAdd(p.colsum_out + z0 * p.colsum_stride + m, v);
    }
    __syncthreads();
  }

  const bool fast = (p.vec_ok & 1) && !(p.N & 7) && n0 + BN4 <= p.N && !p.atomic;
#define V8_PICK(H, M0)                                                                          \
  _Pragma("unroll") for (int a = 0; a < 2; ++a) _Pragma("unroll") for (int b = 0; b < 2; ++b)   \
  _Pragma("unroll") for (int c = 0; c < 2; ++c) tq[a][b][c] = acc[H][M0 + a][b][c];
#define V8_PICK_ROUND()                                                    \
  switch (r) {                                                             \
    case 0: V8_PICK(0, 0) break;                                           \
    case 1: V8_PICK(0, 2) break;                                           \
    default:                                                               \
      if constexpr (AH == 2) {                                             \
        if (r == 2) { V8_PICK(1, 0) } else { V8_PICK(1, 2) }               \
      }                                                                    \
      break;                                                               \
  }
  if (fast) {
    float b8[8];
    if (p.bias) ld8x(p.bias, n0 + (threadIdx.x & 31) * 8, MI_DT_F32, b8);
    else {
#pragma unroll
      for (int j = 0; j < 8; ++j) b8[j] = 0.f;
    }
#pragma nounroll
    for (int r = 0; r < 2 * AH; ++r) {
      f32x4 tq[2][2][2];
      V8_PICK_ROUND()
#if defined(V8_EPI_ABL) && V8_EPI_ABL == 1
      asm volatile("" :: "v"(tq[0][0][0]), "v"(tq[0][0][1]), "v"(tq[0][1][0]), "v"(tq[0][1][1]), "v"(tq[1][0][0]), "v"(tq[1][0][1]), "v"(tq[1][1][0]), "v"(tq[1][1][1]));
      continue;
#endif
      float* win = sC + (r & 1) * (64 * 256);
#pragma unroll
      for (int a = 0; a < 2; ++a)
#pragma unroll
        for (int b = 0; b < 2; ++b)
#pragma unroll
          for (int c = 0; c < 2; ++c)
            *reinterpret_cast<f32x4*>(win + (wm * 32 + a * 16 + l15) * 256 + (((b * 32 + wn * 8 + c * 4 + l4) ^ (l15 & 7)) << 2)) = tq[a][b][c];
#if defined(V8_EPI_ABL) && V8_EPI_ABL == 2
      continue;
#endif
      __syncthreads();
      const int mb = m0 + (r >> 1) * 128 + (r & 1) * 32;
      if constexpr (ES != 0) {
        static_assert(G == 0 && !TN && AH == 2, "specialised rounds: the dense NT 256x256 kernel");
#define V8_SPEC(EPI_, DROP_) \
  if (mb + 96 <= p.M) v8_round_spec<EPI_, DROP_, true>(p, win, b8, z, coff, mb, n0); \
  else v8_round_spec<EPI_, DROP_, false>(p, win, b8, z, coff, mb, n0);
        if constexpr (ES == V8_ES_SWISH_G_DROP) { V8_SPEC(EPI_SWISH_DROP, true) }
        else if constexpr (ES == V8_ES_SWISH_G) { V8_SPEC(EPI_SWISH_DROP, false) }
        else if constexpr (ES == V8_ES_DSWISH_G) { V8_SPEC(EPI_DSWISH, false) }
        else { V8_SPEC(EPI_STORE, false) }
#undef V8_SPEC
        continue;
      }
      switch (p.epi) {
        case EPI_STORE: v8_round_fast<EPI_STORE>(p, win, b8, z, coff, mb, 64, n0); break;
        case EPI_SWISH_DROP: v8_round_fast<EPI_SWISH_DROP>(p, win, b8, z, coff, mb, 64, n0); break;
        case EPI_RESID: v8_round_fast<EPI_RESID>(p, win, b8, z, coff, mb, 64, n0); break;
        case EPI_DSWISH: v8_round_fast<EPI_DSWISH>(p, win, b8, z, coff, mb, 64, n0); break;
        case EPI_RELU_MASK: v8_round_fast<EPI_RELU_MASK>(p, win, b8, z, coff, mb, 64, n0); break;
        default: v8_round_fast<EPI_MUL_POS>(p, win, b8, z, coff, mb, 64, n0); break;
      }
    }
  } else {
    constexpr int LDS_C = BN4 + 4;
#pragma nounroll
    for (int r = 0; r < 2 * AH; ++r) {
      f32x4 tq[2][2][2];
      V8_PICK_ROUND()
      if (r) __syncthreads();
#pragma unroll
      for (int a = 0; a < 2; ++a)
#pragma unroll
        for (int b = 0; b < 2; ++b)
#pragma unroll
          for (int c = 0; c < 2; ++c)
            *reinterpret_cast<f32x4*>(sC + (wm * 32 + a * 16 + l15) * LDS_C + b * 128 + wn * 32 + c * 16 + l4 * 4) = tq[a][b][c];
      __syncthreads();
      v4_round_out(p, sC, z, coff, m0, n0, (r >> 1) * 128 + (r & 1) * 32, false, 64);
    }
  }
#undef V8_PICK_ROUND
#undef V8_PICK
#ifdef V8_TRACE
  asm volatile("s_waitcnt vmcnt(0)" ::: "memory");
  __syncthreads();
  V8_STAMP(3);
#endif
}

template <int G, bool TN, int AH = 2, int ES = 0>
__global__ __launch_bounds__(512) void gemm_bf16_v8_kernel(GemmP p) {
  drop_resolve(p.drop);
  extern __shared__ __attribute__((aligned(16))) bf16_t smem8[];
  const int tn = (p.N + BN4 - 1) / BN4, tm = (p.M + 128 * AH - 1) / (128 * AH);
  const int ntiles = tm * tn;
  int logical, z, ks;
  if constexpr (G == 2) {
    const int gx = gridDim.x, gy = gridDim.y, gz = gridDim.z;
    const int Wt = gx * gy * gz;
    const int L = (int)blockIdx.x + gx * ((int)blockIdx.y + gy * (int)blockIdx.z);
    const int q8w = Wt >> 3, r8w = Wt & 7, xw = L & 7;
    const int w = (xw < r8w ? xw * (q8w + 1) : r8w * (q8w + 1) + (xw - r8w) * q8w) + (L >> 3);
    const int ncombo = gx * gz;
    ks = w / ncombo;
    const int combo = w - ks * ncombo;
    z = combo / gx;
    logical = combo - z * gx;
  } else {
    const int bid = blockIdx.x;
    const int q8 = ntiles >> 3, r8 = ntiles & 7;
    const int xcd = bid & 7, idx = bid >> 3;
    logical = (xcd < r8 ? xcd * (q8 + 1) : r8 * (q8 + 1) + (xcd - r8) * q8) + idx;
    z = blockIdx.z;
    ks = blockIdx.y;
  }
  const int per_cb = tm * 8;
  const int cb = logical / per_cb, rem = logical - cb * per_cb;
  const int w8 = min(8, tn - cb * 8);
  const int tile_m = rem / w8, tile_n = cb * 8 + (rem - tile_m * w8);
  if (p.v8_delay > 0 && blockIdx.x < 256 && (blockIdx.x & 8)) {
    const unsigned long long t0 = wall_clock64();
    while (wall_clock64() - t0 < (unsigned long long)p.v8_delay) __builtin_amdgcn_s_sleep(16);
  }
  gemm_v8_body<G, TN, AH, ES>(p, smem8, tile_m, tile_n, ks, z);
}

__global__ __launch_bounds__(512) void gemm_bf16_grouped_tn8_kernel(GroupP g) {
  extern __shared__ __attribute__((aligned(16))) bf16_t smem8[];
  int pi = 0;
  const int tiles_total = g.tile_begin[g.n];
  const int W = tiles_total * g.splitk;
  const int L = (int)blockIdx.y * (int)gridDim.x + (int)blockIdx.x;
  const int q8w = W >> 3, r8w = W & 7, xw = L & 7;
  const int w = (xw < r8w ? xw * (q8w + 1) : r8w * (q8w + 1) + (xw - r8w) * q8w) + (L >> 3);
  while (pi + 1 < g.n && w >= g.splitk * g.tile_begin[pi + 1]) ++pi;
  const int ntile_p = g.tile_begin[pi + 1] - g.tile_begin[pi];
  const int rel = w - g.splitk * g.tile_begin[pi];
  const int exp_ks = rel / ntile_p, exp_tile = rel - exp_ks * ntile_p;
  GemmP p;
  p.A = g.A[pi]; p.B = g.B[pi]; p.C = g.C[pi];
  p.M = g.M[pi]; p.N = g.N[pi]; p.K = g.K;
  p.lda = g.lda[pi]; p.ldb = g.ldb[pi]; p.ldc = g.ldc[pi]; p.csc = 1;
  p.transA = 1; p.transB = 1; p.batch = 1; p.nb0 = 1;
  p.sA0 = p.sA1 = p.sB0 = p.sB1 = p.sC0 = p.sC1 = 0;
// ... 387 lines not shown
  }
  const int lane = threadIdx.x & 63, wave = threadIdx.x >> 6;
  const int q = lane & 31, lh = lane >> 5;
  const int rb = (wave >> 1) * 32, cb = (wave & 1) * 32;
  f32x16 acc;
#pragma unroll
  for (int r = 0; r < 16; ++r) acc[r] = 0.f;
  for (int k0 = k_begin; k0 < k_end; k0 += 16) {
#pragma unroll
    for (int i = 0; i < 4; ++i) {
      const int e = threadIdx.x + i * 256;
      int r, k;
      if (p.transA) { r = e & 63; k = e >> 6; } else { k = e & 15; r = e >> 4; }
      float v = 0.f;
      if (m0 + r < p.M && k0 + k < k_end) v = A[(long long)(m0 + r) * sar + (long long)(k0 + k) * sak];
      As[k][r] = v;
      if (p.transB) { r = e & 63; k = e >> 6; } else { k = e & 15; r = e >> 4; }
      v = 0.f;
      if (n0 + r < p.N && k0 + k < k_end) v = B[(long long)(n0 + r) * sbr + (long long)(k0 + k) * sbk];
      Bs[k][r] = v;
    }
    __syncthreads();
#pragma unroll
    for (int k = 0; k < 16; k += 2)
      acc = __builtin_amdgcn_mfma_f32_32x32x2f32(As[k + lh][rb + q], Bs[k + lh][cb + q], acc, 0, 0, 0);
    __syncthreads();
  }
#pragma unroll
  for (int r = 0; r < 16; ++r) {
    const int m = m0 + rb + (r & 3) + 8 * (r >> 2) + 4 * lh, n = n0 + cb + q;
    if (m < p.M && n < p.N) epilogue(p, z, coff, m, n, acc[r]);
  }
}

static int env_int(const char* name, int dflt) {
  const char* e = getenv(name);
  return (e && e[0]) ? atoi(e) : dflt;
}
static const struct { const char* env; int dflt; } g_knob[11] = {
    {nullptr, 0}, {nullptr, 0}, {nullptr, 0}, {"MI355X_F32_MFMA", 1}, {"MI355X_GEMM_V4", 1}, {"MI355X_GEMM_V5", 1}, {"MI355X_GEMM_V6", 0},
    {"MI355X_GEMM_V7", 1}, {"MI355X_GEMM_V8", 1}, {"MI355X_GEMM_V8_DELAY", 0}, {"MI355X_GEMM_V8_EPI", 1}};
static std::atomic<int> g_mode[11] = {{-1}, {-1}, {-1}, {-1}, {-1}, {-1}, {-1}, {-1}, {-1}, {-1}, {-1}};
static int mode_now(int key) {
  int v = g_mode[key].load(std::memory_order_relaxed);
  if (v < 0) {
    int expected = -1;
    g_mode[key].compare_exchange_strong(expected, env_int(g_knob[key].env, g_knob[key].dflt), std::memory_order_relaxed);
    v = g_mode[key].load(std::memory_order_relaxed);
  }
  return v;
}
static thread_local int g_last_path = 0;
extern "C" int mi355x_gemm_config(int key, int value) {
  if (key == 11) return g_last_path;
  if (key < 3 || key > 10) return -1;
  mode_now(key);
  return g_mode[key].exchange(value, std::memory_order_relaxed);
}

struct GemmModes {
  int k[11];
  int v2;
  int few_tiles;
};
static GemmModes gemm_modes_now() {
  static const int v2 = env_int("MI355X_GEMM_V2", 1) ? 1 : 0, few = env_int("MI355X_GEMM_FEW_TILES", 0);
  GemmModes m = {};
  for (int key = 3; key <= 10; ++key) m.k[key] = mode_now(key);
  m.v2 = v2; m.few_tiles = few;
  return m;
}

enum GemmKernel {
  GK_NONE = -1,
  GK_S_NT, GK_S_NN, GK_S_TN, GK_S_TT,
  GK_V2_NT, GK_V2_NT_REG, GK_V2_NN, GK_V2_TN,
  GK_V4_NT, GK_V4_NT_GA, GK_V4_NN, GK_V4_TN, GK_V4_TN_GB,
  GK_V6_0, GK_V6_1,
  GK_V8_NT, GK_V8_NT_GA, GK_V8_TN, GK_V8_TN_GB,
  GK_V8_ES0 = GK_V8_TN_GB, GK_V8_ES1, GK_V8_ES2, GK_V8_ES3, GK_V8_ES4,
  GK_V8_HALF,
  GK_V5_STORE, GK_V5_SWISH_DROP, GK_V5_RESID, GK_V5_DSWISH,
  GK_F32, GK_F32_MFMA,
  GK_COUNT
};
struct GemmPlan {
  int kernel;
  int gx, gy, gz, block, lds;
  int v8_delay;
  int path;
  int v5_ntiles, v5_tn;
};

static int cdiv(int a, int b) { return (a + b - 1) / b; }
static int splitk_norm(int nk, int want, int min_kt, int* ktiles_per_split) {
  int sk = want > 1 ? want : 1;
  if (sk > nk) sk = nk;
  *ktiles_per_split = cdiv(nk, sk);
  if (*ktiles_per_split < min_kt) *ktiles_per_split = min_kt;
  return cdiv(nk, *ktiles_per_split);
}
static double round_eff(long long blocks) { return (double)blocks / (double)(((blocks + 255) / 256) * 256); }
static bool cols_waste_ok(int N) { return (long long)cdiv(N, 256) * 256 * 8 <= (long long)N * 9; }
static bool fills_chip(long long blocks, int N, double eff_ref) {
  return blocks >= 224 && cols_waste_ok(N) && round_eff(blocks) >= 0.9 * eff_ref;
}
static bool off_ok(long long rows, long long ld, int bits) { return rows * ld < (1LL << bits); }
static bool dense_nt_whole(const GemmP& p) { return !p.transA && !p.transB && !p.g_on && !(p.K % BK); }

static int gemm_fill(const mi355x_gemm_desc* d, GemmP* out) {
  if (!d || !d->A || !d->B || !d->C || d->M <= 0 || d->N <= 0 || d->K <= 0) return MI_ERR_ARG;
  if (d->in_dtype != MI_DT_F32 && d->in_dtype != MI_DT_BF16) return MI_ERR_ARG;
  if ((d->transA && d->lda * 64 >= (1LL << 31)) || (d->transB && d->ldb * 64 >= (1LL << 31))) return MI_ERR_ARG;
  GemmP& p = *out;
  p.A = d->A; p.B = d->B; p.C = d->C;
  p.M = d->M; p.N = d->N; p.K = d->K;
  p.lda = d->lda; p.ldb = d->ldb; p.ldc = d->ldc; p.csc = d->c_col_stride > 0 ? d->c_col_stride : 1;
  p.transA = d->transA; p.transB = d->transB;
  p.batch = d->batch > 0 ? d->batch : 1; p.nb0 = d->nb0 > 0 ? d->nb0 : p.batch;
  p.sA0 = d->sA0; p.sA1 = d->sA1; p.sB0 = d->sB0; p.sB1 = d->sB1; p.sC0 = d->sC0; p.sC1 = d->sC1;
  p.bias = (const float*)d->bias; p.alpha = d->alpha;
  p.epi = d->epilogue; p.c_dt = d->c_dtype; p.atomic = d->atomic;
  p.swish_g = 0;
  if (p.epi == 6) { p.epi = EPI_SWISH_DROP; p.swish_g = 1; }
  else if (p.epi == 7) { p.epi = EPI_DSWISH; p.swish_g = 1; }
  p.aux_in = d->aux_in; p.auxin_dt = d->aux_in_dtype; p.aux_out = d->aux_out; p.auxout_dt = d->aux_out_dtype;
  p.ldaux = d->ldaux;
  p.drop = mi_drop(d->drop_key, d->drop_threshold, d->drop_scale);
  p.colsum_out = (float*)d->colsum_out; p.colsum_stride = d->colsum_stride;
  p.g_on = 0; p.r_on = 0; p.v8_delay = 0;
  if (d->gather) {
    const mi355x_conv_gather& g = *d->gather;
    if (d->in_dtype != MI_DT_BF16 || g.C <= 0 || (g.C & 7) || g.ntaps < 1 || g.ntaps > 9 || g.nI <= 0 || g.nJ <= 0 ||
        g.SI <= 0 || g.SJ <= 0 || (g.operand != 0 && g.operand != 1))
      return MI_ERR_ARG;
    if (g.operand == 0) {
      if (d->transA || p.batch != 1 || (g.C & 63) || d->K != g.ntaps * g.C || d->M % (g.nI * g.nJ) != 0) return MI_ERR_ARG;
    } else {
      const long long src_elems = (long long)(d->K / (g.nI * g.nJ)) * g.SI * g.SJ * g.C;
      if (src_elems >= (1LL << 31)) return MI_ERR_ARG;
      if (!d->transA || !d->transB || p.batch != g.ntaps || p.nb0 != p.batch || d->N != g.C || d->K % (g.nI * g.nJ) != 0 ||
          ((uintptr_t)d->B & 15))
        return MI_ERR_ARG;
    }
    p.g_on = 1 + g.operand; p.g_nI = g.nI; p.g_nJ = g.nJ; p.g_SI = g.SI; p.g_SJ = g.SJ; p.g_C = g.C; p.g_si = g.si; p.g_sj = g.sj;
    p.g_ntaps = g.ntaps;
    p.g_dip = 0ull; p.g_djp = 0ull;
    for (int t = 0; t < g.ntaps; ++t) {
      if (g.di[t] < -7 || g.di[t] > 7 || g.dj[t] < -7 || g.dj[t] > 7) return MI_ERR_ARG;
      p.g_dip |= (unsigned long long)(g.di[t] + 8) << (4 * t);
      p.g_djp |= (unsigned long long)(g.dj[t] + 8) << (4 * t);
    }
  }
  if (d->rowmap) {
    const mi355x_row_map& r = *d->rowmap;
    if (r.nI <= 0 || r.nJ <= 0 || r.OI <= 0 || r.OJ <= 0 || d->M % (r.nI * r.nJ) != 0 || p.batch != 1) return MI_ERR_ARG;
    p.r_on = 1; p.r_nI = r.nI; p.r_nJ = r.nJ; p.r_OI = r.OI; p.r_OJ = r.OJ; p.r_si = r.si; p.r_sj = r.sj; p.r_oi = r.oi;
    p.r_oj = r.oj;
  }
  p.row_len = (const long long*)d->row_len; p.rows_per_b = d->rows_per_b > 0 ? d->rows_per_b : 1;
  p.rows_inner = d->rows_inner > 0 ? d->rows_inner : 1;
  if (p.epi < EPI_STORE || p.epi > EPI_MUL_POS) return MI_ERR_ARG;
  if (p.atomic && p.c_dt != MI_DT_F32) return MI_ERR_ARG;
  if ((p.epi == EPI_RESID || p.epi == EPI_DSWISH || p.epi == EPI_MUL_POS) && !p.aux_in) return MI_ERR_ARG;
  if (p.epi == EPI_SWISH_DROP && !p.aux_out) return MI_ERR_ARG;
  if (p.epi == EPI_RELU_MASK && !p.row_len) return MI_ERR_ARG;
  if (p.colsum_out && (!p.transA || d->in_dtype != MI_DT_BF16 || p.nb0 != p.batch)) return MI_ERR_ARG;
  p.splitk = splitk_norm(cdiv(p.K, BK), d->splitk, 1, &p.ktiles_per_split);
  if (p.splitk > 1 && !p.atomic) return MI_ERR_ARG;
  {
    const int auxin_dt = p.epi == EPI_RESID ? MI_DT_F32 : p.auxin_dt;
    auto pitch8 = [](long long ld, int dt) { return dt == MI_DT_F32 ? !(ld & 3) : !(ld & 7); };
    bool base = p.csc == 1 && !((uintptr_t)p.C & 31) && !(p.sC0 & 7) && !(p.sC1 & 7);
    if (p.aux_in) base = base && !((uintptr_t)p.aux_in & 31);
    if (p.aux_out) base = base && !((uintptr_t)p.aux_out & 31);
    if (p.bias) base = base && !((uintptr_t)p.bias & 31);
    bool ok = base && pitch8(p.ldc, p.c_dt), ok4 = base && !(p.ldc & 3);
    if (p.aux_in) { ok = ok && pitch8(p.ldaux, auxin_dt); ok4 = ok4 && !(p.ldaux & 3); }
    if (p.aux_out) { ok = ok && pitch8(p.ldaux, p.auxout_dt); ok4 = ok4 && !(p.ldaux & 3); }
    p.vec_ok = (ok ? 1 : 0) | (ok4 ? 2 : 0);
#ifdef GEMM_ABLATE
    { const char* e = getenv("MI355X_GEMM_DBG"); if (e) p.vec_ok |= atoi(e) << 8; }
#endif
  }
  if (d->in_dtype != MI_DT_BF16) return MI_OK;
  if ((p.lda & 7) || (p.ldb & 7) || ((uintptr_t)p.A & 15) || ((uintptr_t)p.B & 15)) return MI_ERR_ARG;
  if ((p.sA0 & 7) || (p.sA1 & 7) || (p.sB0 & 7) || (p.sB1 & 7)) return MI_ERR_ARG;
  const int K8 = (p.K + 7) & ~7;
  if (!p.transA && !p.g_on && p.lda < K8) return MI_ERR_ARG;
  if (!p.transB && p.ldb < K8) return MI_ERR_ARG;
  if (p.transA && p.lda < ((p.M + 7) & ~7)) return MI_ERR_ARG;
  if (p.transB && p.g_on != 2 && p.ldb < ((p.N + 7) & ~7)) return MI_ERR_ARG;
  if (p.g_on && !(p.M >= 192 && p.N >= 96)) return MI_ERR_ARG;
  return MI_OK;
}

static GemmPlan gemm_plan(const GemmP& p, bool bf16, const GemmModes& m) {
  GemmPlan pl = {};
  auto launch = [&pl](int kernel, long long gx, int gy, int gz, int block, int lds) {
    pl.kernel = kernel; pl.gx = (int)gx; pl.gy = gy; pl.gz = gz; pl.block = block; pl.lds = lds;
    return pl;
  };
  const int sk = p.splitk, nk = cdiv(p.K, BK);
  if (!bf16) return launch(m.k[3] ? GK_F32_MFMA : GK_F32, cdiv(p.M, 64) * cdiv(p.N, 64), sk, p.batch, 256, 0);
  const bool nt = !p.transA && !p.transB, tnl = p.transA && p.transB;
  const int tm = cdiv(p.M, BM), tn = cdiv(p.N, BN), tm2 = cdiv(p.M, BM2), tn4 = cdiv(p.N, BN4);
  const long long per_tile = (long long)sk * p.batch;
  const long long blocks2 = (long long)tm2 * tn * per_tile, blocks4 = (long long)tm2 * tn4 * per_tile;
  const bool few_tiles = !p.g_on && !p.r_on && !p.atomic && blocks2 <= m.few_tiles && p.N <= 1024 && (long long)tm * tn * per_tile > blocks2;
  if (!(m.v2 && p.M >= 192 && p.N >= 96 && !(p.transA && !p.transB) && !few_tiles)) {
    if (p.g_on) return launch(GK_NONE, 0, 0, 0, 0, 0);
    return launch(p.transA ? (p.transB ? GK_S_TN : GK_S_TT) : (p.transB ? GK_S_NN : GK_S_NT), tm * tn, sk, p.batch, 256, 0);
  }
  const int nk_wg = sk > 1 ? p.ktiles_per_split : nk;
  const double eff2 = round_eff(blocks2);
  const bool fills = fills_chip(blocks4, p.N, eff2);
  const int v8_mode = m.k[8];
  bool v8_can = (nt || tnl) && nk_wg >= 2 && nk - (sk - 1) * nk_wg >= 2  && p.N > 128;
  if (nt) {
    v8_can = v8_can && p.g_on != 2 && !(p.K % BK) && off_ok(p.N, p.ldb, 31);
    if (p.g_on == 1)
      v8_can = v8_can && !(p.g_C % BK) && off_ok((long long)(p.M / (p.g_nI * p.g_nJ)) * p.g_SI * p.g_SJ, p.g_C, 31);
    else v8_can = v8_can && off_ok(p.M, p.lda, 31);
  } else if (tnl) {
    v8_can = v8_can && p.g_on != 1 && off_ok(64, p.lda, 30) && (p.g_on == 2 || off_ok(64, p.ldb, 30));
  }
  const bool v5_keeps = nt && !p.g_on && p.epi == EPI_STORE && p.N >= 1536 && nk >= 8 && nk <= 9 && !p.atomic && sk == 1 &&
                        !(p.N % BN) && m.k[5] && v8_mode != 4 && round_eff(blocks4) < 0.85;
  if (v8_can && nt && !p.g_on && !fills && fills_chip((long long)tm * tn4 * per_tile, p.N, eff2) &&
      ((v8_mode == 5 && nk >= 12) || (v8_mode == 2 && blocks4 < 224))) {
    pl.path = 810;
    return launch(GK_V8_HALF, tm * tn4, sk, p.batch, 512, 9 * V8_HALF_B);
  }
  if (v8_can && (v8_mode == 2 || (v8_mode >= 1 && fills && !v5_keeps && (nt || v8_mode == 3)))) {
    if (nt && blocks4 > 256 && nk <= 16) pl.v8_delay = m.k[9];
    int es = 0;
    if (m.k[10] && nt && !p.g_on && !p.r_on && !p.atomic && sk == 1 && p.csc == 1 && p.c_dt == MI_DT_BF16 && p.ldc < (1 << 24) &&
        p.ldaux < (1 << 24)) {
      if (p.epi == EPI_SWISH_DROP && p.swish_g && p.auxout_dt == MI_DT_BF16) es = p.drop.threshold ? V8_ES_SWISH_G_DROP : V8_ES_SWISH_G;
      else if (p.epi == EPI_DSWISH && p.swish_g && p.auxin_dt == MI_DT_BF16) es = V8_ES_DSWISH_G;
      else if (p.epi == EPI_STORE && !p.drop.threshold) es = V8_ES_STORE;
    }
    pl.path = 800 + es;
    const int generic = nt ? (p.g_on == 1 ? GK_V8_NT_GA : GK_V8_NT) : (p.g_on == 2 ? GK_V8_TN_GB : GK_V8_TN);
    return launch(es ? GK_V8_ES0 + es : generic, tm2 * tn4, sk, p.batch, 512, 2 * V8_BUF_B);
  }
  const int v5_mode = m.k[5];
  const bool v5_epi = (p.epi == EPI_STORE && (v5_mode == 2 || p.N >= 1536)) || (p.epi == EPI_SWISH_DROP && v5_mode == 2) ||
                      (p.epi == EPI_RESID && p.c_dt == MI_DT_F32) || (p.epi == EPI_DSWISH && p.auxin_dt == MI_DT_BF16);
  if (v5_mode && nt && !p.g_on && !p.r_on && !p.atomic && p.batch == 1 && sk == 1 && (p.vec_ok & 1) && !(p.N % BN) && nk >= 8 &&
      (nk <= 9 || v5_mode == 2) && tm2 * tn >= 256 && v5_epi && off_ok(p.M, p.lda, 31) && off_ok(p.N, p.ldb, 31) &&
      off_ok(p.M, p.ldc, 31) && off_ok(p.M, p.ldaux, 31)) {
    pl.v5_ntiles = tm2 * tn; pl.v5_tn = tn;
    return launch(GK_V5_STORE + p.epi, 256, 1, 1, 512, V5_LDS_BYTES);
  }
  if ((m.k[4] == 2 && p.N > 128) || (m.k[4] == 1 && fills)) {
    if (m.k[6] && dense_nt_whole(p) && sk == 1 && !(p.K % (2 * BK)) && p.K >= 4 * BK && off_ok(p.M, p.lda, 30) && off_ok(p.N, p.ldb, 30))
      return launch(m.k[6] == 2 ? GK_V6_0 : GK_V6_1, tm2 * tn4, 1, p.batch, 512, 2 * NT4_STAGE * 2);
    const int k4 = nt ? (p.g_on == 1 ? GK_V4_NT_GA : GK_V4_NT) : !p.transA ? GK_V4_NN : (p.g_on == 2 ? GK_V4_TN_GB : GK_V4_TN);
    return launch(k4, tm2 * tn4, sk, p.batch, 512, 2 * NT4_STAGE * 2);
  }
  const bool reg_ok = m.k[7] && dense_nt_whole(p) && nk_wg >= 4 && !(nk_wg & 1) && (sk == 1 || !(nk % nk_wg)) &&
                      off_ok(p.M, p.lda, 30) && off_ok(p.N, p.ldb, 30);
  return launch(nt ? (reg_ok ? GK_V2_NT_REG : GK_V2_NT) : !p.transA ? GK_V2_NN : GK_V2_TN, tm2 * tn, sk, p.batch, 512, 3 * NT2_STAGE * 2);
}

static bool lds_attr_once(std::atomic<int>& state, const void* fn, int lds) {
  int s = state.load(std::memory_order_acquire);
  if (!s && lds > 0) {
    s = hipFuncSetAttribute(fn, hipFuncAttributeMaxDynamicSharedMemorySize, lds) == hipSuccess ? 1 : 2;
    state.store(s, std::memory_order_release);
  }
  return s != 2;
}

typedef void (*gemm_fn)(GemmP);
typedef void (*gemm_v5_fn)(GemmP, int, int);
static int gemm_launch(const GemmPlan& pl, const GemmP& p, hipStream_t s) {
  static const void* const kernels[GK_COUNT] = {
      (const void*)gemm_bf16_kernel<false, false>, (const void*)gemm_bf16_kernel<false, true>, (const void*)gemm_bf16_kernel<true, true>,
      (const void*)gemm_bf16_kernel<true, false>,
      (const void*)gemm_bf16_v2_kernel<false, false>, (const void*)gemm_bf16_v2_kernel<false, false, true>,
      (const void*)gemm_bf16_v2_kernel<false, true>, (const void*)gemm_bf16_v2_kernel<true, true>,
      (const void*)gemm_bf16_v4_kernel<false, false, 0>, (const void*)gemm_bf16_v4_kernel<false, false, 1>,
      (const void*)gemm_bf16_v4_kernel<false, true, 0>, (const void*)gemm_bf16_v4_kernel<true, true, 0>,
      (const void*)gemm_bf16_v4_kernel<true, true, 2>,
      (const void*)gemm_bf16_v6_kernel<0>, (const void*)gemm_bf16_v6_kernel<1>,
      (const void*)gemm_bf16_v8_kernel<0, false>, (const void*)gemm_bf16_v8_kernel<1, false>, (const void*)gemm_bf16_v8_kernel<0, true>,
      (const void*)gemm_bf16_v8_kernel<2, true>,
      (const void*)gemm_bf16_v8_kernel<0, false, 2, V8_ES_SWISH_G_DROP>, (const void*)gemm_bf16_v8_kernel<0, false, 2, V8_ES_SWISH_G>,
      (const void*)gemm_bf16_v8_kernel<0, false, 2, V8_ES_DSWISH_G>, (const void*)gemm_bf16_v8_kernel<0, false, 2, V8_ES_STORE>,
      (const void*)gemm_bf16_v8_kernel<0, false, 1>,
      (const void*)gemm_bf16_v5_kernel<EPI_STORE>, (const void*)gemm_bf16_v5_kernel<EPI_SWISH_DROP>,
      (const void*)gemm_bf16_v5_kernel<EPI_RESID>, (const void*)gemm_bf16_v5_kernel<EPI_DSWISH>,
      (const void*)gemm_f32_kernel, (const void*)gemm_f32_mfma_kernel};
  static std::atomic<int> attr[GK_COUNT];
  const void* fn = kernels[pl.kernel];
  if (!lds_attr_once(attr[pl.kernel], fn, pl.lds)) { (void)hipGetLastError(); return MI_ERR_LAUNCH; }
  auto issue = [&](auto kernel, auto... more) { MI_LAUNCH(kernel, dim3(pl.gx, pl.gy, pl.gz), dim3(pl.block), pl.lds, s, p, more...); };
  if (pl.kernel >= GK_V5_STORE && pl.kernel <= GK_V5_DSWISH) issue((gemm_v5_fn)fn, pl.v5_ntiles, pl.v5_tn);
  else issue((gemm_fn)fn);
  return MI_OK;
}

extern "C" int mi355x_gemm(const mi355x_gemm_desc* d, void* stream) {
  mi_clear_errors();
  g_last_path = 0;
  GemmP p;
  int rc = gemm_fill(d, &p);
  if (rc != MI_OK) return rc;
  const GemmPlan pl = gemm_plan(p, d->in_dtype == MI_DT_BF16, gemm_modes_now());
  if (pl.kernel == GK_NONE) return MI_ERR_ARG;
  p.v8_delay = pl.v8_delay;
  rc = gemm_launch(pl, p, (hipStream_t)stream);
  if (rc != MI_OK) return rc;
  g_last_path = pl.path;
  return mi_check_launch();
}

extern "C" int mi355x_gemm_plan(const mi355x_gemm_desc* d, int out[8]) {
  GemmP p;
  const int rc = gemm_fill(d, &p);
  if (rc != MI_OK) return rc;
  const GemmPlan pl = gemm_plan(p, d->in_dtype == MI_DT_BF16, gemm_modes_now());
  if (pl.kernel == GK_NONE) return MI_ERR_ARG;
  const int v[8] = {pl.kernel, pl.path, pl.gx, pl.gy, pl.gz, pl.block, pl.lds, pl.v8_delay};
  for (int i = 0; i < 8; ++i) out[i] = v[i];
  return MI_OK;
}

static int group_tiles(GroupP& g, int bn) {
  int tiles = 0;
  for (int i = 0; i <= GRP_MAX; ++i) {
    g.tile_begin[i] = tiles;
    if (i < g.n) tiles += cdiv(g.M[i], BM2) * cdiv(g.N[i], bn);
  }
  return tiles;
}
static int group_fill(const mi355x_gemm_desc* descs, int n, GroupP* out) {
  if (!descs || n < 1 || n > GRP_MAX) return MI_ERR_ARG;
  GroupP& g = *out;
  g.n = n; g.K = descs[0].K;
  for (int i = 0; i < n; ++i) {
    const mi355x_gemm_desc& d = descs[i];
    if (!d.A || !d.B || !d.C || d.M <= 0 || d.N <= 0 || d.K != g.K || d.K <= 0) return MI_ERR_ARG;
    if (d.in_dtype != MI_DT_BF16 || d.c_dtype != MI_DT_F32 || !d.transA || !d.transB || !d.atomic) return MI_ERR_ARG;
    if (d.batch > 1 || d.bias || d.aux_in || d.aux_out || d.gather || d.rowmap || d.epilogue != EPI_STORE) return MI_ERR_ARG;
    if (d.alpha != 1.f || d.c_col_stride > 1 || d.drop_threshold != 0u) return MI_ERR_ARG;
    if ((d.lda & 7) || (d.ldb & 7) || ((uintptr_t)d.A & 15) || ((uintptr_t)d.B & 15)) return MI_ERR_ARG;
    if (d.lda < ((d.M + 7) & ~7) || d.ldb < ((d.N + 7) & ~7)) return MI_ERR_ARG;
    g.A[i] = d.A; g.B[i] = d.B; g.C[i] = d.C; g.colsum[i] = (float*)d.colsum_out;
    g.M[i] = d.M; g.N[i] = d.N; g.lda[i] = d.lda; g.ldb[i] = d.ldb; g.ldc[i] = d.ldc;
  }
  return MI_OK;
}
static int group_plan(GroupP& g, int want_sk, int v8_mode, int* tiles) {
  const int nk = cdiv(g.K, BK);
  bool ok8 = (v8_mode == 2 || v8_mode == 3) && nk >= 4;
  for (int i = 0; i < g.n; ++i) ok8 = ok8 && g.N[i] > 128 && off_ok(64, g.lda[i], 30) && off_ok(64, g.ldb[i], 30);
  if (ok8) {
    *tiles = group_tiles(g, BN4);
    int best = 1;
    double best_score = -1.0;
    for (int c = 1; c <= 16; ++c) {
      if (c > 1 && nk / c < 16) break;
      const double score = round_eff((long long)*tiles * c) - 0.01 * c;
      if (score > best_score + 1e-9) { best = c; best_score = score; }
    }
    g.splitk = splitk_norm(nk, want_sk > 1 ? best : 1, 2, &g.ktiles_per_split);
    if (nk - (g.splitk - 1) * g.ktiles_per_split >= 2) return 1;
  }
  *tiles = group_tiles(g, BN);
  g.splitk = splitk_norm(nk, want_sk, 1, &g.ktiles_per_split);
  return 0;
}

extern "C" int mi355x_gemm_grouped(const mi355x_gemm_desc* descs, int n, void* stream) {
  mi_clear_errors();
  GroupP g;
  const int rc = group_fill(descs, n, &g);
  if (rc != MI_OK) return rc;
  int tiles = 0;
  const int k8 = group_plan(g, descs[0].splitk, mode_now(8), &tiles);
  static void (*const kernels[2])(GroupP) = {gemm_bf16_grouped_tn_kernel, gemm_bf16_grouped_tn8_kernel};
  static std::atomic<int> attr[2];
  const int lds = k8 ? 2 * V8_BUF_B : 3 * NT2_STAGE * 2;
  if (!lds_attr_once(attr[k8], (const void*)kernels[k8], lds)) { (void)hipGetLastError(); return MI_ERR_LAUNCH; }
  MI_LAUNCH(kernels[k8], dim3(tiles, g.splitk, 1), dim3(512), lds, (hipStream_t)stream, g);
  return mi_check_launch();
}
```

nemo_amd/csrc/subsample.hip:

```cpp
#include "common.h"
#include "mi355x_asr.h"

#define DISPATCH_DT(dt, T, ...)                                      \
  if ((dt) == MI_DT_F32) { typedef float T; __VA_ARGS__; }           \
  else { typedef bf16_t T; __VA_ARGS__; }


#define C1_TR 4
template <typename TO>
__global__ __launch_bounds__(256) void conv1_fwd_kernel(const float* __restrict__ mel, const float* __restrict__ w,
                                                        const float* __restrict__ bias, TO* __restrict__ out,
                                                        const long long* __restrict__ len0, const long long* __restrict__ len1,
                                                        int B, int F, int T, int T1, int F1, int C, int pad) {
  constexpr int V = VecIO<TO>::V;
  extern __shared__ float patch[];
  const int FW = F + pad + 1, NR = 2 * C1_TR + 1;
  const int b = blockIdx.y, t1_0 = blockIdx.x * C1_TR;
  const int tlim = (int)min((long long)T, len0[b]);
  for (int i = threadIdx.x; i < NR * FW; i += 256) {
    const int rr = i / FW, fi = i - rr * FW;
    const int t = 2 * t1_0 - pad + rr, f = fi - pad;
    float v = 0.f;
    if (t >= 0 && t < tlim && f >= 0 && f < F) v = mel[((long long)b * F + f) * T + t];
    patch[i] = v;
  }
  __syncthreads();
  const int CP = C / V;
  const int FS = 256 / CP;
  const int ck = threadIdx.x % CP, fs = threadIdx.x / CP;
  if (fs >= FS) return;
  const int l1 = (int)min((long long)T1, len1[b]);
  {
    const int c = ck * V;
    float wk[9][V], bs[V];
#pragma unroll
    for (int j = 0; j < V; ++j) {
      bs[j] = bias[c + j];
#pragma unroll
      for (int k = 0; k < 9; ++k) wk[k][j] = w[(c + j) * 9 + k];
    }
    for (int tr = 0; tr < C1_TR; ++tr) {
      const int t1 = t1_0 + tr;
      if (t1 >= T1) break;
      const bool tvalid = t1 < l1;
      const float* prow = patch + 2 * tr * FW;
      for (int f1 = fs; f1 < F1; f1 += FS) {
        float m[9];
#pragma unroll
        for (int kh = 0; kh < 3; ++kh)
#pragma unroll
          for (int kw = 0; kw < 3; ++kw) m[kh * 3 + kw] = prow[kh * FW + 2 * f1 + kw];
        float o[V];
#pragma unroll
        for (int j = 0; j < V; ++j) {
          float a = bs[j];
#pragma unroll
          for (int k = 0; k < 9; ++k) a = fmaf(wk[k][j], m[k], a);
          o[j] = (tvalid && a > 0.f) ? a : 0.f;
        }
        VecIO<TO>::store(out + (((long long)b * T1 + t1) * F1 + f1) * C + c, o);
      }
    }
  }
}

#define C1_TB 32
template <typename TO>
__global__ __launch_bounds__(256) void conv1_bwd_kernel(const TO* __restrict__ dout, const float* __restrict__ mel,
                                                        const long long* __restrict__ len0, float* __restrict__ dw,
                                                        float* __restrict__ db, float* __restrict__ partial, int B, int F, int T,
                                                        int T1, int F1, int C, int pad) {
  constexpr int V = VecIO<TO>::V;
  extern __shared__ float smem[];
  const int TW = 2 * C1_TB + 1, FW = F + pad + 1;
  float* mel_s = smem;
  float* red = smem + FW * TW;
  const int b = blockIdx.y;
  const int t1_0 = blockIdx.x * C1_TB, t1_end = min(T1, t1_0 + C1_TB);
  const int tbase = 2 * t1_0 - pad;
  const int tlim = (int)min((long long)T, len0[b]);
  for (int i = threadIdx.x; i < FW * TW; i += 256) {
    const int fi = i / TW, tt = i - fi * TW;
    const int f = fi - pad, t = tbase + tt;
    float v = 0.f;
    if (f >= 0 && f < F && t >= 0 && t < tlim) v = mel[((long long)b * F + f) * T + t];
    mel_s[i] = v;
  }
  __syncthreads();
  const int wave = __builtin_amdgcn_readfirstlane(threadIdx.x >> 6), lane = threadIdx.x & 63;
  const int part = blockIdx.y * gridDim.x + blockIdx.x;
  const int CL = (C / V >= 64 || (64 % (C / V))) ? 64 : C / V;
  const int NF = 64 / CL;
  const int lane_c = lane % CL, fsub = lane / CL;
  for (int c0 = 0; c0 < C; c0 += CL * V) {
    const int c = c0 + lane_c * V;
    float gw[9][V], gb[V];
#pragma unroll
    for (int j = 0; j < V; ++j) {
      gb[j] = 0.f;
#pragma unroll
      for (int k = 0; k < 9; ++k) gw[k][j] = 0.f;
    }
    if (c < C) {
      for (int t1 = t1_0 + wave; t1 < t1_end; t1 += 4) {
        const float* mrow = mel_s + 2 * (t1 - t1_0);
        const TO* gp = dout + ((long long)b * T1 + t1) * F1 * C + c;
#pragma unroll 4
        for (int f1 = fsub; f1 < F1; f1 += NF) {
          float g[V];
          VecIO<TO>::load(gp + (long long)f1 * C, g);
          float m[9];
#pragma unroll
          for (int kh = 0; kh < 3; ++kh)
#pragma unroll
            for (int kw = 0; kw < 3; ++kw) m[kh * 3 + kw] = mrow[(2 * f1 + kw) * TW + kh];
#pragma unroll
          for (int j = 0; j < V; ++j) {
            gb[j] += g[j];
#pragma unroll
            for (int k = 0; k < 9; ++k) gw[k][j] = fmaf(g[j], m[k], gw[k][j]);
          }
        }
      }
    }
    for (int off = CL; off < 64; off <<= 1) {
#pragma unroll
      for (int j = 0; j < V; ++j) {
        gb[j] += __shfl_xor(gb[j], off, 64);
#pragma unroll
        for (int k = 0; k < 9; ++k) gw[k][j] += __shfl_xor(gw[k][j], off, 64);
      }
    }
#pragma unroll
    for (int k = 0; k < 10; ++k) {
      __syncthreads();
#pragma unroll
      for (int j = 0; j < V; ++j) red[wave * 64 * V + lane_c * V + j] = k < 9 ? gw[k < 9 ? k : 0][j] : gb[j];
      __syncthreads();
      for (int e = threadIdx.x; e < CL * V; e += 256) {
        const int cc = c0 + e;
        if (cc >= C) continue;
        const float v = (red[e] + red[64 * V + e]) + (red[2 * 64 * V + e] + red[3 * 64 * V + e]);
        if (partial) partial[((long long)part * 10 + k) * C + cc] = v;
        else if (k < 9) atomicAdd(dw + cc * 9 + k, v);
        else atomicAdd(db + cc, v);
      }
    }
  }
}

template <typename TT>
__global__ __launch_bounds__(256) void im2col_kernel(const TT* __restrict__ in, TT* __restrict__ col, int B, int T1, int F1,
                                                     int T2, int F2, int C, int pad) {
  constexpr int V = sizeof(TT) == 2 ? 8 : 4;
  const int cv = C / V;
  const long long total = (long long)B * T2 * F2 * 9 * cv;
  for (long long i = blockIdx.x * 256LL + threadIdx.x; i < total; i += (long long)gridDim.x * 256) {
    const int c = (int)(i % cv);
    long long r = i / cv;
    const int tap = (int)(r % 9); r /= 9;
    const int f2 = (int)(r % F2); r /= F2;
    const int t2 = (int)(r % T2);
    const int b = (int)(r / T2);
    const int kh = tap / 3, kw = tap - kh * 3;
    const int t1 = 2 * t2 + kh - pad, f1 = 2 * f2 + kw - pad;
    u32x4 v = {0u, 0u, 0u, 0u};
    if (t1 >= 0 && t1 < T1 && f1 >= 0 && f1 < F1)
      v = *reinterpret_cast<const u32x4*>(in + (((long long)b * T1 + t1) * F1 + f1) * C + c * V);
    *reinterpret_cast<u32x4*>(col + ((((long long)b * T2 + t2) * F2 + f2) * 9 + tap) * C + c * V) = v;
// ... 119 lines not shown
```

nemo_amd/modules/conformer_encoder.py:

```python
from __future__ import annotations

import math
import os
from collections import OrderedDict
from typing import Optional

import torch
from torch import nn

from .. import ops
from ..core import (AcousticEncodedRepresentation, BoolType, ChannelType, LengthsType, NeuralModule, NeuralType, SpectrogramType,
                    typecheck)
from ..flat import FlatParams
from ..packing import PackPlan

INF_VAL = 10000.0


def _pad8(n):
    return (n + 7) // 8 * 8


class _FeedForward(nn.Module):
    def __init__(self, d_model, d_ff, use_bias=True):
# ... 190 lines not shown
            raise NotImplementedError("MI355X ConformerEncoder does not implement: " + ", ".join(bad))
        d_ff = d_model * ff_expansion_factor
        self.d_model, self.n_layers, self._feat_in = d_model, n_layers, feat_in
        self.n_heads, self.d_k, self.d_ff = n_heads, d_model // n_heads, d_ff
        self.conv_kernel_size = conv_kernel_size
        self.subsampling_factor = subsampling_factor
        self.att_context_style, self.self_attention_model = att_context_style, self_attention_model
        self.att_context_size_all, self.att_context_size, self.att_context_probs = self._calc_att_context(
            att_context_size, att_context_probs, att_context_style)
        if self_attention_model == "rel_pos_local_attn":
            if max(self.att_context_size) <= 0:
                raise ValueError("When using local attention, context size must be set > 0")
            if len(self.att_context_size_all) != 1 or self.att_context_size[0] != self.att_context_size[1]:
                raise NotImplementedError("MI355X ConformerEncoder: rel_pos_local_attn needs one window att_context_size = [w, w]")
            self.att_context_style = "regular"
        self._ctx = (0, -1, -1)
        self.sync_max_audio_length = sync_max_audio_length
        self.xscale = math.sqrt(d_model) if xscaling else None
        self.dropout, self.dropout_pre_encoder, self.dropout_att = dropout, dropout_pre_encoder, dropout_att
        self.dropout_emb = dropout_emb
        if subsampling_conv_channels == -1:
            subsampling_conv_channels = d_model
        self.subsampling = subsampling
        self.pre_encode = ConvSubsampling(subsampling, subsampling_factor, feat_in, d_model, subsampling_conv_channels,
                                          causal=causal_downsampling)
        self._feat_out = d_model
        self.pos_emb_max_len = pos_emb_max_len
        self.pos_enc = RelPositionalEncoding(d_model, dropout_pre_encoder, pos_emb_max_len, self.xscale, dropout_emb)
        self.conv_norm_type = conv_norm_type
        if conv_context_size is None:
            self.conv_context_size, self.conv_pad_left = None, -1
        else:
            if isinstance(conv_context_size, str):
                if conv_context_size != "causal":
                    raise ValueError("Invalid conv_context_size! It should be the string 'causal' or a list of two integers.")
                cc_ = [conv_kernel_size - 1, 0]
            else:
                cc_ = [int(v) for v in conv_context_size]
                if len(cc_) != 2 or cc_[0] + cc_[1] + 1 != conv_kernel_size:
                    raise ValueError(f"Invalid conv_context_size: {conv_context_size}!")
            self.conv_context_size = cc_
            self.conv_pad_left = -1 if cc_[0] == cc_[1] else cc_[0]
        self.layers = nn.ModuleList([ConformerLayer(d_model, d_ff, n_heads, conv_kernel_size, conv_norm_type) for _ in range(n_layers)])
        if feat_out > 0 and feat_out != d_model:
            self.out_proj = nn.Linear(d_model, feat_out)
            self._feat_out = feat_out
        else:
            self.out_proj = None
        self.layer_drop_probs = self._stochastic_depth_probs(n_layers, stochastic_depth_drop_prob, stochastic_depth_mode,
                                                             stochastic_depth_start_layer)
        self.capture_layers = []
        self.captured = {}
        self.max_audio_length = pos_emb_max_len
        self.streaming_cfg = None
        self._init_engine(compute_dtype, tail=lambda n: n.endswith("self_attn.linear_pos.weight"))

    def _init_engine(self, compute_dtype, tail=None):
        self.compute_dtype = compute_dtype
        self.sync_batchnorm = True
        self._syncbn_group = None
        self._syncbn_mailbox = None
        self._syncbn_mailbox_tried = False
        self.syncbn_profile = None
        self.use_flash_attention = True
        self.flash_pad_heads = os.environ.get("MI355X_FLASH_PAD_HEADS", "1") != "0"
        _pk = os.environ.get("MI355X_PACKED", "auto").lower()
        self.packed_rows = {"0": False, "false": False, "1": True, "true": True}.get(_pk, "auto")
        self.packed_min_padding = float(os.environ.get("MI355X_PACKED_MIN_PADDING", "0.02"))
        self.packed_last = None
        self.fuse_layer_boundary_norms = os.environ.get("MI355X_LN2", "1") != "0"
        self.fuse_boundary_bwd = os.environ.get("MI355X_LN2_BWD", "1") != "0"
        self.flash_delta_residual = os.environ.get("MI355X_FLASH_DELTA_LO", "1") != "0"
        self.grad_ready_hook = None
        self._flatp = FlatParams(self, tail=tail)
        self.wgrad_side_stream = os.environ.get("MI355X_WGRAD_STREAM", "1") != "0"
        self._wg_stream = None
        self._wgrad_join_per_layer = True
        self.wgrad_grouped = os.environ.get("MI355X_WGRAD_GROUPED", "1") != "0"
        self.wgrad_defer = int(os.environ.get("MI355X_WGRAD_DEFER", "1"))
        self.wgrad_layers = int(os.environ.get("MI355X_WGRAD_LAYERS", "2"))
        self.posproj_side = os.environ.get("MI355X_POSPROJ_SIDE", "1") != "0"
        self._wg_pending, self._wg_rows = None, None
        self.conv2_implicit = os.environ.get("MI355X_CONV2_IMPLICIT", "1") != "0"
        self.fuse_bn_dwconv_bwd = os.environ.get("MI355X_BN_DW_FUSE", "1") != "0"
        self.fuse_glu_dwconv_bwd = os.environ.get("MI355X_GLU_DW_FUSE", "1") != "0"
        self.tap_reduce_side = os.environ.get("MI355X_TAP_REDUCE_SIDE", "1") != "0"
        self.pad_tile_skip = os.environ.get("MI355X_PAD_SKIP", "1") != "0"
        self.fuse_glu_dwconv_fwd = os.environ.get("MI355X_GLU_DW_FUSE_FWD", "1") != "0"
        self.ln_cast_fuse = os.environ.get("MI355X_LN_CAST_FUSE", "1") != "0"
        self.ffn_fused = os.environ.get("MI355X_FFN_FUSED", "0") != "0"
        self.swish_g = os.environ.get("MI355X_SWISH_G", "1") != "0"
        self._saving = False
        self.dpos_side_stream = os.environ.get("MI355X_DPOS_STREAM", "1") != "0"
        self.sub_wgrad_side_stream = os.environ.get("MI355X_SUB_WGRAD_STREAM", "1") != "0"
        self._plans = {}
        self._ws = {}
        self._ws_retired = []
        self._pos_cache = {}
        self._step_seed = 0
        self._weights_version = -1
        self._token = None
        _g = os.environ.get("MI355X_GRAPHS", "auto")
        self.use_graphs = _g != "0"
        self.graph_auto = _g not in ("0", "1", "2")
        self.graph_tape = os.environ.get("MI355X_TAPE", "1") != "0"
        self.graph_bwd_live = os.environ.get("MI355X_GRAPHS_BWD_LIVE", "0") != "0"
        self.graph_warmup = 2
        self.graph_trials = 4
        self.max_graph_sets = int(os.environ.get("MI355X_GRAPH_SETS", "64"))
        self.graph_warmup_inherited = 1
        self.replayed_steps = self.live_steps = 0
        self._graph_sets = OrderedDict()
        self._cur_gs = None
        from ..arena import Arena
        _a = os.environ.get("MI355X_ARENA", "auto")
        self.use_arena = _a != "0"
        self.arena_forced = _a == "1"
        self._in_step = False
        self._arena_f, self._arena_b, self._arena = Arena("forward"), Arena("backward"), None
        self._fwd_serial = 0
        self._capture = None
        self._wg_forked = False
        self._force_pack = False
        self._step_word = None

    def set_max_audio_length(self, max_audio_length):
        self.max_audio_length = max_audio_length

    def update_max_seq_length(self, seq_length: int, device):
        if seq_length > self.max_audio_length:
            self.set_max_audio_length(seq_length)

    def flat_parameters(self) -> FlatParams:
        self._flatp.ensure()
        return self._flatp

    def weights_updated(self):
        self._weights_version += 1

    def load_state_dict(self, *a, **k):
        r = super().load_state_dict(*a, **k)
        self.weights_updated()
        return r

    @staticmethod
    def _calc_att_context(att_context_size, att_context_probs, att_context_style):
        if att_context_style not in ("regular", "chunked_limited"):
            raise ValueError(f"att_context_style={att_context_style}")
        if att_context_size:
            all_ = [list(x) for x in ([att_context_size] if isinstance(list(att_context_size)[0], int) else list(att_context_size))]
            for i, cs in enumerate(all_):
                if att_context_style == "chunked_limited":
                    if cs[0] > 0 and cs[0] % (cs[1] + 1) > 0:
                        raise ValueError(f"att_context_size[{i}][0] % (att_context_size[{i}][1] + 1) should be zero!")
                    if cs[1] < 0 and len(all_) <= 1:
                        raise ValueError(f"Right context (att_context_size[{i}][1]) can not be unlimited for chunked_limited style!")
        else:
            all_ = [[-1, -1]]
        if att_context_probs:
            if len(att_context_probs) != len(all_):
                raise ValueError("The size of the att_context_probs should be the same as att_context_size.")
            probs = list(att_context_probs)
            if sum(probs) != 1:
                raise ValueError("The sum of numbers in att_context_probs should be equal to one to be a distribution.")
        else:
            probs = [1.0 / len(all_)] * len(all_)
# ... 1268 lines not shown
            self._wgrad_flush()
            self._wg_pending, self._wg_rows = cur
            for j in js:
                layer_done(j)
        self._defer_flush = (lambda: flush_deferred(force=not pair)) if defer else None
        for i in range(self.n_layers - 1, -1, -1):
            if i in cap_grads:
                dx = dx + to_rows(cap_grads[i], i)
            sd = S.sd[i] if getattr(S, "sd", None) else None
            if sd is None:
                dx = self._layer_bwd(i, self.layers[i], dx, S, S.layers[i], W, Wf)
            elif sd[0] == "drop":
                self._layer_bwd(i, self.layers[i], torch.zeros_like(dx), S, S.layers[i], W, Wf)
            else:
                din = self._layer_bwd(i, self.layers[i], dx * sd[1], S, S.layers[i], W, Wf)
                dx = torch.add(din, dx, alpha=1.0 - sd[1])
            S.layers[i] = None
            if defer:
                dfr = self._wg_deferred
                if pair and dfr is not None and len(dfr[2]) < nlay and dfr[1] == self._wg_rows:
                    self._wg_deferred = (dfr[0] + self._wg_pending, dfr[1], dfr[2] + [i])
                else:
                    flush_deferred()
                    self._wg_deferred = (self._wg_pending, self._wg_rows, [i])
                self._wg_pending, self._wg_rows = [], None
                continue
            self._wgrad_flush()
            layer_done(i)
        if defer:
            flush_deferred()
        self._defer_flush = None
        self._wg_pending = None
        if pk is not None:
            dxu = self._new(M, d, dtype=torch.float32, device=dev)
            ops.rows_unpack(dx, dxu, S.len2, pk.cu, T2, M, d)
            dx = dxu
        if self.posproj_side:
            with self._wgrad_scope(S.dp_all, S.pos):
                self._pos_proj_wgrad(S.dp_all, S.pos, P, cdt)
        else:
            self._wgrad_join(consume=True)
            self._pos_proj_wgrad(S.dp_all, S.pos, P, cdt)
        if self.grad_ready_hook is not None:
            if self.posproj_side and self._wgrad_join_per_layer:
                self._wgrad_join(consume=True)
            self._hook(*fp.tail_range())
        if getattr(S, "bypass", False):
            return None
        pe = self.pre_encode
        if self.subsampling == "dw_striding":
            return self._sub_bwd_dw(S, dx, W, cdt)
        dxs = self._new(M, d, dtype=cdt, device=dev)
        ops.drop_scale_cast(dx, dxs, M * d, (self.xscale or 1.0), S.drop_pre)
        with self._sub_wgrad_scope(dxs):
            ops.colsum(dxs, pe.out.bias.grad, M, d)
        tiles = self._tiles(d, C_, cdt == torch.bfloat16) * F2
        with self._sub_wgrad_scope(dxs, S.out2):
            ops.gemm(dxs, S.out2, pe.out.weight.grad, d, C_, M, d, F2 * C_, C_ * F2, transA=True, transB=True, atomic=True,
                     splitk=self._splitk(tiles, M, strided_c=True), batch=F2, nb0=F2, sB=(C_, 0), sC=(1, 0), c_col_stride=F2,
                     c_dtype=ops.F32)
        dout2 = self._new(B * T2 * F2, C_, dtype=cdt, device=dev)
        ops.gemm(dxs, W["pre.outt"], dout2, M, F2 * C_, d, d, W.pitch("pre.outt"), F2 * C_, epi=ops.EPI_MUL_POS, aux_in=S.out2,
                 row_len=S.len2 if self.pad_tile_skip else None, rows_per_b=T2, rows_inner=1)
        M2 = B * T2 * F2
        with self._sub_wgrad_scope(dout2):
            ops.colsum(dout2, pe.conv[2].bias.grad, M2, C_)
        implicit = self.conv2_implicit and self._conv2_implicit(cdt, C_, M2) and S.col is None
        tiles = self._tiles(C_, C_, cdt == torch.bfloat16) * 9
        if implicit:
            with self._sub_wgrad_scope(dout2, S.out1):
                ops.gemm(dout2, S.out1, pe.conv[2].weight.grad, C_, C_, M2, C_, C_, 9 * C_, transA=True, transB=True,
                         atomic=True, splitk=self._splitk(tiles, M2), batch=9, nb0=9, sC=(1, 0), c_col_stride=9,
                         c_dtype=ops.F32, row_len=S.len2 if self.pad_tile_skip else None, rows_per_b=T2 * F2, rows_inner=F2,
                         gather=dict(operand=1, nI=T2, nJ=F2, SI=T1, SJ=F1, C=C_, si=2, sj=2,
                                     taps=[(kh - pe._pad, kw - pe._pad) for kh in range(3) for kw in range(3)]))
        else:
            col = S.col
            if S.col_gen != self._col_gen:
                ops.im2col(S.out1, col, B, T1, F1, C_, pad=pe._pad)
                self._col_gen += 1
            ops.gemm(dout2, col, pe.conv[2].weight.grad, C_, C_, M2, C_, 9 * C_, 9 * C_, transA=True, transB=True,
                     atomic=True, splitk=self._splitk(tiles, M2), batch=9, nb0=9, sB=(C_, 0), sC=(1, 0), c_col_stride=9,
                     c_dtype=ops.F32)
        dout1 = self._buf("dout1", (B, T1, F1, C_), cdt, dev)
        if self.conv2_implicit and self._conv2_implicit(cdt, C_, M2):
            for pt in (0, 1):
                for pf in (0, 1):
                    nI, nJ = (T1 - pt + 1) // 2, (F1 - pf + 1) // 2
                    slots = self._dgrad_slots(pt, pf, pe._pad)
                    name = f"pre.w2d{pt}{pf}"
                    ops.gemm(dout2, W[name], dout1, B * nI * nJ, C_, len(slots) * C_, C_, W.pitch(name), C_,
                             epi=ops.EPI_MUL_POS, aux_in=S.out1, ldaux=C_, row_len=S.len2 if self.pad_tile_skip else None,
                             rows_per_b=nI * nJ, rows_inner=nJ,
                             gather=dict(nI=nI, nJ=nJ, SI=T2, SJ=F2, C=C_, si=1, sj=1,
                                         taps=[((pt + pe._pad - kh) // 2, (pf + pe._pad - kw) // 2) for kh, kw in slots]),
                             rowmap=dict(nI=nI, nJ=nJ, OI=T1, OJ=F1, si=2, sj=2, oi=pt, oj=pf))
        else:
            dcol = self._buf("dcol", (M2, 9 * C_), cdt, dev)
            ops.gemm(dout2, W["pre.w2t"], dcol, M2, 9 * C_, C_, C_, W.pitch("pre.w2t"), 9 * C_)
            ops.col2im_relu(dcol, S.out1, dout1, B, T1, F1, C_, pad=pe._pad)
        ops.conv1_bwd(dout1, S.mel, S.len0, pe.conv[0].weight.grad, pe.conv[0].bias.grad, C_, pad=pe._pad)
        self._wgrad_join()
        if self.grad_ready_hook is not None:
            self._hook(*fp.range_of("pre_encode."))

    def _ffn_bwd(self, pfx, ff, ln, saved, dr, W, M, d, dff, cdt, dev, df=None, next_cast=None, boundary=None):
        x, y, mean, rstd, h, a, d_in, d_res = saved
        if df is None:
            df = self._new(M, d, dtype=cdt, device=dev)
            ops.drop_scale_cast(dr, df, M * d, 0.5, d_res)
        dh = self._new(M, dff, dtype=cdt, device=dev)
        dy = self._new(M, d, dtype=cdt, device=dev)
        if a is None:
            a = self._new(M, dff, dtype=cdt, device=dev)
            ops.ffn_bwd_dgrad(df, W[pfx + ".w2tp"], W[pfx + ".w1tp"], h, dh, a, dy, M, d, dff, d_in)
            self._wgrad(df, d, 0, a, dff, 0, ff.linear2.weight.grad, d, dff, M, bias_grad=ff.linear2.bias.grad)
            self._wgrad(dh, dff, 0, y, d, 0, ff.linear1.weight.grad, dff, d, M, bias_grad=ff.linear1.bias.grad)
        else:
            self._wgrad(df, d, 0, a, dff, 0, ff.linear2.weight.grad, d, dff, M, bias_grad=ff.linear2.bias.grad)
            if d_in is None:
                ops.gemm(df, W[pfx + ".w2t"], dh, M, dff, d, d, W.pitch(pfx + ".w2t"), dff, epi=ops.EPI_DSWISH_G, aux_in=h)
            else:
                ops.gemm(df, W[pfx + ".w2t"], dh, M, dff, d, d, W.pitch(pfx + ".w2t"), dff, epi=ops.EPI_DSWISH, aux_in=h, drop=d_in)
            self._wgrad(dh, dff, 0, y, d, 0, ff.linear1.weight.grad, dff, d, M, bias_grad=ff.linear1.bias.grad)
            ops.gemm(dh, W[pfx + ".w1t"], dy, M, d, dff, dff, W.pitch(pfx + ".w1t"), d)
        nxt = self._cast_buf(next_cast, M, d, cdt, dev)
        if boundary is not None:
            ln_lo, r4, mean5, rstd5 = boundary
            dr_lo = self._new(M, d, dtype=torch.float32, device=dev)
            ops.layernorm2_bwd(dy, x, ln.weight, mean, rstd, ln.weight.grad, ln.bias.grad, dr, r4, ln_lo.weight, mean5, rstd5,
                               ln_lo.weight.grad, ln_lo.bias.grad, dr_lo, M, d, cast_out=nxt,
                               cast_scale=next_cast[0] if nxt is not None else 1.0,
                               cast_drop=next_cast[1] if nxt is not None else None)
            return dr_lo, nxt
        ops.layernorm_bwd(dy, x, ln.weight, mean, rstd, dr, True, ln.weight.grad, ln.bias.grad, M, d, cast_out=nxt,
                          cast_scale=next_cast[0] if nxt is not None else 1.0,
                          cast_drop=next_cast[1] if nxt is not None else None)
        return dr, nxt

    def _cast_buf(self, next_cast, M, d, cdt, dev):
        if next_cast is None or cdt != torch.bfloat16 or (M * d) % 8 or not self.ln_cast_fuse:
            return None
        return self._new(M, d, dtype=cdt, device=dev)

    def _attn_block_bwd(self, i, a, saved, dao, S, W, M, B, T2, d, dk, scale, cdt, dev):
        r1, y2, mean2, rstd2, qkv, p, qu, qv, s_, pd, ctx, d_att, d_ares, lse = saved
        self._wgrad(dao, d, 0, ctx, d, 0, a.linear_out.weight.grad, d, d, M, bias_grad=a.linear_out.bias.grad)
        dctx = self._new(M, d, dtype=cdt, device=dev)
        ops.gemm(dao, W[f"L{i}.att.wot"], dctx, M, d, d, d, W.pitch(f"L{i}.att.wot"), d)
        gu, gv_ = a.pos_bias_u.grad, a.pos_bias_v.grad
        adjacent = gv_.data_ptr() - gu.data_ptr() == 4 * d
        dqkv, dqu, dqv = self._attn_bwd((qu, qv, s_, pd, lse), qkv, p, a.pos_bias_u, a.pos_bias_v, ctx, dctx, S.len2, B, T2, d,
                                        dk, scale, d_att, cdt, dev, S.dpos_f32[i], S.dp_all[i],
                                        bias_grads=gu if (adjacent and lse is not None) else None, pk=getattr(S, "pk", None))
        if dqu is None:
            pass
        elif cdt == torch.bfloat16 and adjacent:
            ops.add2_colsum(dqu, dqv, dqkv, 3 * d, M, d, gu)
        else:
            ops.colsum(dqu, gu, M, d)
            ops.colsum(dqv, gv_, M, d)
            ops.add2(dqu, dqv, dqkv, 3 * d, M, d)
        gq, gk, gv = a.linear_q.weight.grad, a.linear_k.weight.grad, a.linear_v.weight.grad
        sw = (gk.data_ptr() - gq.data_ptr()) // 4
        sb = (a.linear_k.bias.grad.data_ptr() - a.linear_q.bias.grad.data_ptr()) // 4
        if (cdt == torch.bfloat16 and sw > 0 and (gv.data_ptr() - gk.data_ptr()) // 4 == sw
                and (a.linear_v.bias.grad.data_ptr() - a.linear_k.bias.grad.data_ptr()) // 4 == sb):
            if self._wg_pending is not None:
                for j, lin in enumerate((a.linear_q, a.linear_k, a.linear_v)):
                    self._wgrad(dqkv, 3 * d, j * d, y2, d, 0, lin.weight.grad, d, d, M, bias_grad=lin.bias.grad)
            else:
                with self._wgrad_scope(dqkv, y2):
                    ops.gemm(dqkv, y2, gq, d, d, M, 3 * d, d, d, transA=True, transB=True, atomic=True,
                             splitk=self._splitk(3 * self._tiles(d, d, True), M), batch=3, nb0=3, sA=(d, 0), sC=(sw, 0),
                             c_dtype=ops.F32, colsum_out=a.linear_q.bias.grad, colsum_stride=sb)
        else:
            for j, lin in enumerate((a.linear_q, a.linear_k, a.linear_v)):
                self._wgrad(dqkv, 3 * d, j * d, y2, d, 0, lin.weight.grad, d, d, M, bias_grad=lin.bias.grad)
        dy2 = self._new(M, d, dtype=cdt, device=dev)
        ops.gemm(dqkv, W[f"L{i}.att.wqkvt"], dy2, M, d, 3 * d, 3 * d, W.pitch(f"L{i}.att.wqkvt"), d)
        return dy2

    def _attn_block_bwd_padded(self, i, a, saved, dao, S, W, Wf, M, B, T2, d, dk, dkp, dA, scale, cdt, dev):
        r1, y2, mean2, rstd2, qkv, p, qu, qv, s_, pd, ctx, d_att, d_ares, lse = saved
# ... 158 lines not shown
```

nemo_amd/ops.py:

```python
from __future__ import annotations

import contextlib
import ctypes as C
from typing import Optional

import torch

from ._lib import ConvGather, GemmDesc, PackEntry, RowMap, check, lib

F32, BF16 = 0, 1
EPI_STORE, EPI_SWISH_DROP, EPI_RESID, EPI_DSWISH, EPI_RELU_MASK, EPI_MUL_POS, EPI_SWISH_DROP_G, EPI_DSWISH_G = range(8)

_DT = {torch.float32: F32, torch.bfloat16: BF16}


def dt(t) -> int:
    try:
        return _DT[t.dtype if isinstance(t, torch.Tensor) else t]
    except KeyError:
        raise ValueError(f"unsupported dtype {t.dtype if isinstance(t, torch.Tensor) else t}")


def _ptr(t: Optional[torch.Tensor]) -> int:
    if t is None:
        return 0
    if not t.is_cuda:
        raise RuntimeError("nemo_amd kernels run on MI355X only: got a CPU tensor (there is no CPU fallback)")
    return t.data_ptr()


def _stream() -> int:
    return torch.cuda.current_stream().cuda_stream


class Dropout:
    __slots__ = ("key", "threshold", "scale")

    def __init__(self, p: float = 0.0, seed: int = 0, site: int = 0):
        if p <= 0.0:
            self.key, self.threshold, self.scale = 0, 0, 1.0
        else:
            self.key = (seed * 0x9E3779B1 + site * 0x85EBCA77 + 0x1234567) & 0xFFFFFFFF
            self.threshold = max(1, min(0xFFFFFFFF, int(p * 4294967296.0)))
            self.scale = 1.0 / (1.0 - p)


NO_DROP = Dropout()

GEMM_PROFILE = None


def gemm_config(key: int, value: int) -> int:
    return lib.mi355x_gemm_config(key, value)


@contextlib.contextmanager
def gemm_modes(modes=None, **kv):
    modes = {**(modes or {}), **{int(k[1:]): v for k, v in kv.items()}}
    old = {}
    try:
        for k, v in modes.items():
            old[k] = gemm_config(k, v)
        yield
    finally:
        for k, v in old.items():
            gemm_config(k, v)


def gemm_plan(desc: GemmDesc):
    out = (C.c_int * 8)()
    rc = lib.mi355x_gemm_plan(C.byref(desc), C.byref(out))
    return rc, list(out)


STEP_WORD_INC = -1640531535


def set_step_counter(word: Optional[torch.Tensor]) -> None:
    if word is not None and (word.dtype != torch.int32 or word.numel() != 1):
        raise ValueError("the step word is one int32 on the device")
    check(lib.mi355x_set_step_counter(_ptr(word)), "set_step_counter")


def wgrad_grouped(problems, rows, splitk):
    n = len(problems)
    arr = (GemmDesc * n)()
    for d, (dY, ldy, y_off, X, ldx, x_off, dW, n_out, n_in, bias_grad) in zip(arr, problems):
        d.A = _ptr(dY) + y_off * dY.element_size()
        d.B = _ptr(X) + x_off * X.element_size()
        d.C = _ptr(dW)
        d.M, d.N, d.K = n_out, n_in, rows
        d.lda, d.ldb, d.ldc = ldy, ldx, n_in
        d.c_col_stride = 1
        d.transA = d.transB = 1
        d.in_dtype, d.c_dtype = BF16, F32
        d.batch = d.nb0 = 1
        d.alpha = 1.0
        d.epilogue, d.atomic, d.splitk = EPI_STORE, 1, splitk
        d.colsum_out = _ptr(bias_grad) if bias_grad is not None else 0
    if GEMM_PROFILE is None:
        check(lib.mi355x_gemm_grouped(arr, n, _stream()), "gemm_grouped")
        return
    e0, e1 = torch.cuda.Event(enable_timing=True), torch.cuda.Event(enable_timing=True)
    e0.record()
    check(lib.mi355x_gemm_grouped(arr, n, _stream()), "gemm_grouped")
    e1.record()
    GEMM_PROFILE.append(("bf16_TN", sum(q[7] * q[8] for q in problems), 1, rows, 1, e0, e1))


def gemm(A, B, Cm, M, N, K, lda, ldb, ldc, *, transA=False, transB=False, in_dtype=None, c_dtype=None, batch=1, nb0=0,
         sA=(0, 0), sB=(0, 0), sC=(0, 0), bias=None, alpha=1.0, epi=EPI_STORE, atomic=False, splitk=1, aux_in=None,
         aux_out=None, ldaux=0, drop: Dropout = NO_DROP, row_len=None, rows_per_b=1, rows_inner=1,
         a_off=0, b_off=0, c_off=0, c_col_stride=1, colsum_out=None, colsum_off=0, colsum_stride=0, gather=None,
         rowmap=None):
    d = GemmDesc()
    esA, esC = A.element_size(), Cm.element_size()
    d.A = _ptr(A) + a_off * esA
    d.B = _ptr(B) + b_off * B.element_size()
    d.C = _ptr(Cm) + c_off * esC
    d.M, d.N, d.K = M, N, K
    d.lda, d.ldb, d.ldc = lda, ldb, ldc
    d.c_col_stride = c_col_stride
    d.transA, d.transB = int(transA), int(transB)
    d.in_dtype = dt(A) if in_dtype is None else in_dtype
    d.c_dtype = dt(Cm) if c_dtype is None else c_dtype
    d.batch, d.nb0 = batch, (nb0 if nb0 > 0 else batch)
    d.sA0, d.sA1 = sA
    d.sB0, d.sB1 = sB
    d.sC0, d.sC1 = sC
    d.bias = _ptr(bias)
    d.alpha = alpha
    d.epilogue, d.atomic, d.splitk = epi, int(atomic), splitk
    d.aux_in = _ptr(aux_in)
    d.aux_in_dtype = dt(aux_in) if aux_in is not None else 0
    d.aux_out = _ptr(aux_out)
    d.aux_out_dtype = dt(aux_out) if aux_out is not None else 0
    d.ldaux = ldaux if ldaux else ldc
    d.drop_key, d.drop_threshold, d.drop_scale = drop.key, drop.threshold, drop.scale
    d.row_len = _ptr(row_len)
    d.rows_per_b, d.rows_inner = rows_per_b, rows_inner
    d.colsum_out = (_ptr(colsum_out) + 4 * colsum_off) if colsum_out is not None else 0
    d.colsum_stride = colsum_stride
    keep = []
    if gather is not None:
        g = ConvGather()
        g.nI, g.nJ, g.SI, g.SJ, g.C, g.si, g.sj = (gather[k] for k in ("nI", "nJ", "SI", "SJ", "C", "si", "sj"))
        g.ntaps = len(gather["taps"])
        g.operand = int(gather.get("operand", 0))
        for t, (di, dj) in enumerate(gather["taps"]):
            g.di[t], g.dj[t] = di, dj
        keep.append(g)
        d.gather = C.cast(C.pointer(g), C.c_void_p)
    if rowmap is not None:
        r = RowMap()
        r.nI, r.nJ, r.OI, r.OJ, r.si, r.sj, r.oi, r.oj = (rowmap[k] for k in ("nI", "nJ", "OI", "OJ", "si", "sj", "oi", "oj"))
        keep.append(r)
        d.rowmap = C.cast(C.pointer(r), C.c_void_p)
    if GEMM_PROFILE is None:
        check(lib.mi355x_gemm(C.byref(d), _stream()), "gemm")
        return
    e0, e1 = torch.cuda.Event(enable_timing=True), torch.cuda.Event(enable_timing=True)
    e0.record()
    check(lib.mi355x_gemm(C.byref(d), _stream()), "gemm")
    e1.record()
    variant = ("bf16" if d.in_dtype == BF16 else "f32") + "_" + ("T" if transA else "N") + ("N" if transB else "T")
    GEMM_PROFILE.append((variant, M, N, K, batch, e0, e1))


def logmel(audio, audio_len, window, fb_sparse, n_mels, *, hop=160, n_fft=512, preemph=0.97, dither=0.0, seed=0,
           log_guard=2.0 ** -24, out=None):
    B, S = audio.shape
    T = 1 + S // hop
    if out is None:
        out = torch.empty(B, n_mels, T, device=audio.device, dtype=torch.float32)
    st, ln, off, w = fb_sparse
    check(lib.mi355x_logmel_fwd(_ptr(audio), _ptr(audio_len), _ptr(window), window.numel(), hop, n_fft, _ptr(st), _ptr(ln),
                                _ptr(off), _ptr(w), n_mels, preemph if preemph is not None else 0.0, dither, seed & 0xFFFFFFFF,
                                log_guard, _ptr(out), B, S, T, _stream()), "logmel_fwd")
    return out


def feat_normalize(x, seq_len, out=None, normalize=True, pad_value=0.0, out_dtype=torch.float32):
    B, n_mels, T = x.shape
    if out is None:
        out = torch.empty(B, n_mels, T, device=x.device, dtype=out_dtype)
    check(lib.mi355x_feat_normalize(_ptr(x), _ptr(seq_len), _ptr(out), dt(out), B, n_mels, T, int(normalize), pad_value,
                                    _stream()), "feat_normalize")
    return out


def half_len(n, pad=1):
    return (n + pad - 2) // 2 + 1


def conv1_fwd(mel, w, bias, out, len0, len1, C_, pad=1):
    B, F, T = mel.shape
    check(lib.mi355x_subsample_conv1_fwd_pad(_ptr(mel), _ptr(w), _ptr(bias), _ptr(out), dt(out), _ptr(len0), _ptr(len1), B, F, T,
                                             C_, pad, _stream()), "subsample_conv1_fwd")


def conv1_bwd(dout, mel, len0, dw, db, C_, pad=1):
    B, F, T = mel.shape
    T1 = half_len(T, pad)
    n = ((T1 + 31) // 32) * B * 10 * C_
    sc = _scratch("conv1_bwd", n, dout.device)
    check(lib.mi355x_subsample_conv1_bwd_pad(_ptr(dout), dt(dout), _ptr(mel), _ptr(len0), _ptr(dw), _ptr(db), B, F, T, C_, pad,
                                             _ptr(sc), n, _stream()), "subsample_conv1_bwd")


def im2col(x, col, B, T1, F1, C_, pad=1):
    check(lib.mi355x_im2col_3x3s2_pad(_ptr(x), _ptr(col), dt(x), B, T1, F1, C_, pad, _stream()), "im2col")


def col2im_relu(dcol, act, din, B, T1, F1, C_, pad=1):
    check(lib.mi355x_col2im_3x3s2_relu_pad(_ptr(dcol), _ptr(act), _ptr(din), dt(dcol), B, T1, F1, C_, pad, _stream()), "col2im")


def dwconv2d_s2_fwd(x, w, bias, out, B, T1, F1, C_, pad=1):
    check(lib.mi355x_dwconv2d_s2_fwd_pad(_ptr(x), _ptr(w), _ptr(bias), _ptr(out), dt(x), B, T1, F1, C_, pad, _stream()),
          "dwconv2d_s2_fwd")


def dwconv2d_s2_bwd(dout, x, w, din, dw, dbias, B, T1, F1, C_, pad=1):
    T2, F2 = half_len(T1, pad), half_len(F1, pad)
    npos = B * T2 * F2
    nblk = (npos + 63) // 64 if npos < 1024 * 64 else 1024
    n = nblk * 10 * C_
    sc = _scratch("dwconv2d_bwd", n, dout.device)
    check(lib.mi355x_dwconv2d_s2_bwd_pad(_ptr(dout), _ptr(x), _ptr(w), _ptr(din), _ptr(dw), _ptr(dbias), dt(x), B, T1, F1, C_, pad,
                                         _ptr(sc), n, _stream()), "dwconv2d_s2_bwd")


def embed_sos_fwd(targets, emb, out, B, U, H, blank):
    check(lib.mi355x_embed_sos_fwd(_ptr(targets), _ptr(emb), _ptr(out), dt(out), B, U, H, blank, _stream()), "embed_sos_fwd")


def embed_sos_bwd(targets, dx, demb, B, U, H, blank):
    check(lib.mi355x_embed_sos_bwd(_ptr(targets), _ptr(dx), dt(dx), _ptr(demb), B, U, H, blank, _stream()), "embed_sos_bwd")


def lstm_cell_fwd(z, b_hh, c_prev, c, h, h_lp, B, H):
    check(lib.mi355x_lstm_cell_fwd(_ptr(z), _ptr(b_hh), _ptr(c_prev), _ptr(c), _ptr(h), _ptr(h_lp), dt(h_lp), B, H, _stream()),
          "lstm_cell_fwd")


def lstm_cell_bwd(dh, dc, act, c, c_prev, dz, B, H):
    check(lib.mi355x_lstm_cell_bwd(_ptr(dh), _ptr(dc), _ptr(act), _ptr(c), _ptr(c_prev), _ptr(dz), dt(dz), B, H, _stream()),
          "lstm_cell_bwd")


def joint_combine_fwd(f, g, h, B, T, U1, J, drop: Dropout = NO_DROP):
    check(lib.mi355x_joint_combine_fwd(_ptr(f), _ptr(g), _ptr(h), dt(h), drop.key, drop.threshold, drop.scale, B, T, U1, J,
                                       _stream()), "joint_combine_fwd")


def joint_combine_bwd(dh, h, df, B, T, U1, J, drop_scale=1.0):
    check(lib.mi355x_joint_combine_bwd(_ptr(dh), _ptr(h), _ptr(df), dt(h), drop_scale, B, T, U1, J, _stream()), "joint_combine_bwd")


def cast_rows(src, ld_in, dst, ld_out, M, N, Np, alpha=1.0):
    check(lib.mi355x_cast_rows(_ptr(src), ld_in, _ptr(dst), dt(dst), ld_out, M, N, Np, alpha, _stream()), "cast_rows")


def ffn_fwd(y, w1p, b1, w2p, b2, x, h, out, M, d, dff, alpha=0.5, drop_in: Dropout = NO_DROP, drop_res: Dropout = NO_DROP):
    check(lib.mi355x_ffn_fwd(_ptr(y), d, _ptr(w1p), _ptr(b1), _ptr(w2p), _ptr(b2), _ptr(x), d, _ptr(h), dff, _ptr(out), d, M, d, dff,
                             alpha, drop_in.key, drop_in.threshold, drop_in.scale, drop_res.key, drop_res.threshold,
                             drop_res.scale, _stream()), "ffn_fwd")


def ffn_pack(table_dev, n_entries, max_dff):
    check(lib.mi355x_ffn_pack(_ptr(table_dev), n_entries, max_dff, _stream()), "ffn_pack")


def ffn_bwd_dgrad(df, w2tp, w1tp, h, dh, act, dy, M, d, dff, drop_in: Dropout = NO_DROP):
    check(lib.mi355x_ffn_bwd_dgrad(_ptr(df), d, _ptr(w2tp), _ptr(w1tp), _ptr(h), dff, _ptr(dh), _ptr(act), _ptr(dy), d, M, d, dff,
                                   drop_in.key, drop_in.threshold, drop_in.scale, _stream()), "ffn_bwd_dgrad")


def layernorm2_fwd(x, gamma1, beta1, y1, mean1, rstd1, gamma2, beta2, y2, mean2, rstd2, M, d, eps=1e-5):
    check(lib.mi355x_layernorm2_fwd(_ptr(x), _ptr(gamma1), _ptr(beta1), _ptr(y1), _ptr(mean1), _ptr(rstd1), _ptr(gamma2), _ptr(beta2),
                                    _ptr(y2), dt(y2), _ptr(mean2), _ptr(rstd2), M, d, eps, _stream()), "layernorm2_fwd")


def layernorm_fwd(x, gamma, beta, y, mean, rstd, M, d, eps=1e-5):
    check(lib.mi355x_layernorm_fwd(_ptr(x), dt(x), _ptr(gamma), _ptr(beta), _ptr(y), dt(y), _ptr(mean), _ptr(rstd), M, d, eps,
                                   _stream()), "layernorm_fwd")


def layernorm_bwd(dy, x, gamma, mean, rstd, dres, accumulate, dgamma, dbeta, M, d, cast_out=None, cast_scale=1.0,
                  cast_drop: "Dropout" = None):
# ... 555 lines not shown
```

Baseline: 17710 audio-sec/s.

## Fuse conv1 weight-gradient tap reduction into the conv2 dgrad GEMM epilogue

The subsampling conv2 data-gradient GEMM epilogue now computes the ReLU-gated conv1 output gradient and immediately contracts it with the 3x3 mel taps plus a bias column. It writes per-tile partial weight and bias gradients, which a fold kernel and a tap-reduce kernel then combine. This avoids materialising the dout1 tensor and running a separate conv1_bwd kernel over it. The cost is extra LDS use, more epilogue arithmetic in the GEMM, and two small reduction kernels.

```diff
diff --git a/include/mi355x_asr.h b/include/mi355x_asr.h
--- a/include/mi355x_asr.h
+++ b/include/mi355x_asr.h
@@ -50,6 +50,18 @@
 int mi355x_gemm(const mi355x_gemm_desc* desc, void* stream);
 int mi355x_gemm_config(int key, int value);
 int mi355x_gemm_plan(const mi355x_gemm_desc* desc, int out[8]);
+typedef struct mi355x_conv1_taps {
+  const void* mel;
+  const void* len0;
+  int B, F, T, pad;
+  void* partial;
+  long long partial_elems;
+  int part_begin;
+} mi355x_conv1_taps;
+int mi355x_gemm_conv1_taps(const mi355x_gemm_desc* desc, const mi355x_conv1_taps* taps, void* stream);
+int mi355x_gemm_conv1_taps_plan(const mi355x_gemm_desc* desc, const mi355x_conv1_taps* taps, int out[8]);
+int mi355x_conv1_taps_reduce(const void* partial, int nparts, int C, void* fold, long long fold_elems, void* dw, void* db,
+                             void* stream);
 int mi355x_gemm_grouped(const mi355x_gemm_desc* descs, int n, void* stream);
 
 int mi355x_ffn_fwd(const void* y, long long ldy, const void* w1_packed, const void* b1, const void* w2_packed, const void* b2,
diff --git a/nemo_amd/_lib.py b/nemo_amd/_lib.py
--- a/nemo_amd/_lib.py
+++ b/nemo_amd/_lib.py
@@ -41,6 +41,11 @@
     _fields_ = [("nI", i32), ("nJ", i32), ("OI", i32), ("OJ", i32), ("si", i32), ("sj", i32), ("oi", i32), ("oj", i32)]
 
 
+class Conv1Taps(C.Structure):
+    _fields_ = [("mel", vp), ("len0", vp), ("B", i32), ("F", i32), ("T", i32), ("pad", i32), ("partial", vp),
+                ("partial_elems", i64), ("part_begin", i32)]
+
+
 class FfnPackEntry(C.Structure):
     _fields_ = [("src", vp), ("k512", vp), ("kchunk", vp), ("d_ff", i32), ("is_w2", i32)]
 
@@ -59,6 +64,9 @@
     "mi355x_gemm_grouped": [C.POINTER(GemmDesc), i32, vp],
     "mi355x_gemm_config": [i32, i32],
     "mi355x_gemm_plan": [C.POINTER(GemmDesc), C.POINTER(i32 * 8)],
+    "mi355x_gemm_conv1_taps": [C.POINTER(GemmDesc), C.POINTER(Conv1Taps), vp],
+    "mi355x_gemm_conv1_taps_plan": [C.POINTER(GemmDesc), C.POINTER(Conv1Taps), C.POINTER(i32 * 8)],
+    "mi355x_conv1_taps_reduce": [vp, i32, i32, vp, i64, vp, vp, vp],
     "mi355x_set_step_counter": [vp],
     "mi355x_set_null_launch": [i32],
     "mi355x_ffn_fwd": [vp, i64, vp, vp, vp, vp, vp, i64, vp, i64, vp, i64, i32, i32, i32, f32, u32, u32, f32, u32, u32, f32, vp],
diff --git a/nemo_amd/csrc/common.h b/nemo_amd/csrc/common.h
--- a/nemo_amd/csrc/common.h
+++ b/nemo_amd/csrc/common.h
@@ -204,6 +204,10 @@
     *reinterpret_cast<float4*>(p) = make_float4(v[0], v[1], v[2], v[3]);
   }
 };
+
+__device__ __forceinline__ float conv1_mel_at(const float* __restrict__ mel, int b, int f, int t, int F, int T, int tlim) {
+  return (f >= 0 && f < F && t >= 0 && t < tlim) ? mel[((long long)b * F + f) * T + t] : 0.f;
+}
 
 static __global__ __launch_bounds__(256) void tap_reduce_kernel(const float* __restrict__ partial, int nparts, int KS, int d,
                                                                 float* __restrict__ dw, float* __restrict__ dbias) {
diff --git a/nemo_amd/csrc/gemm.hip b/nemo_amd/csrc/gemm.hip
--- a/nemo_amd/csrc/gemm.hip
+++ b/nemo_amd/csrc/gemm.hip
@@ -37,6 +37,7 @@
   int g_on, g_nI, g_nJ, g_SI, g_SJ, g_C, g_si, g_sj, g_ntaps;
   unsigned long long g_dip, g_djp;
   int r_on, r_nI, r_nJ, r_OI, r_OJ, r_si, r_sj, r_oi, r_oj;
+  const float* t_mel; const long long* t_len0; float* t_part; int t_F, t_T, t_pad;
 };
 
 __device__ __forceinline__ int tap_delta(unsigned long long packed, int tap) {
@@ -64,6 +65,42 @@
   const int r = m - b * per_b;
   const int j = r - i * p.r_nJ;
   return ((long long)b * p.r_OI + i * p.r_si + p.r_oi) * p.r_OJ + j * p.r_sj + p.r_oj;
+}
+
+#define TAPS_LD 12
+__device__ __forceinline__ float tap_value(const GemmP& p, int m, int k) {
+  const int per_b = p.r_nI * p.r_nJ;
+  int b, i;
+  if ((unsigned)p.M < (1u << 24)) {
+    b = fdiv24(m, per_b, __builtin_amdgcn_rcpf((float)per_b));
+    i = fdiv24(m - b * per_b, p.r_nJ, __builtin_amdgcn_rcpf((float)p.r_nJ));
+  } else {
+    b = m / per_b;
+    i = (m - b * per_b) / p.r_nJ;
+  }
+  const int j = m - b * per_b - i * p.r_nJ;
+  if (k >= 9) return 1.f;
+  const int t1 = i * p.r_si + p.r_oi, f1 = j * p.r_sj + p.r_oj;
+  const int kh = k / 3, kw = k - kh * 3;
+  const int tlim = (int)min((long long)p.t_T, p.t_len0[b]);
+  return conv1_mel_at(p.t_mel, b, 2 * f1 + kw - p.t_pad, 2 * t1 + kh - p.t_pad, p.t_F, p.t_T, tlim);
+}
+__device__ __forceinline__ void taps_round8(const GemmP& p, long long ci, float (&v)[8]) {
+  const u32x4 t = {pack_bf2(v[0], v[1]), pack_bf2(v[2], v[3]), pack_bf2(v[4], v[5]), pack_bf2(v[6], v[7])};
+  if (p.C) *reinterpret_cast<u32x4*>((bf16_t*)p.C + ci) = t;
+#pragma unroll
+  for (int j = 0; j < 4; ++j) { v[2 * j] = __uint_as_float(t[j] << 16); v[2 * j + 1] = __uint_as_float(t[j] & 0xffff0000u); }
+}
+typedef float taps_f2 __attribute__((ext_vector_type(2)));
+__device__ __forceinline__ void taps_fma(float (&acc)[10], float g, const float* trow) {
+  const taps_f2 g2 = {g, g};
+#pragma unroll
+  for (int i = 0; i < 5; ++i) {
+    const taps_f2 t = *reinterpret_cast<const taps_f2*>(trow + 2 * i);
+    taps_f2 a = {acc[2 * i], acc[2 * i + 1]};
+    a = __builtin_elementwise_fma(g2, t, a);
+    acc[2 * i] = a.x; acc[2 * i + 1] = a.y;
+  }
 }
 
 __device__ __forceinline__ float ldx(const void* p, long long i, int dt) {
@@ -311,10 +348,21 @@
 }
 
 
-template <int EPI, int ITERS, int ROW_STEP, int TW = BN, bool UNAL = false, bool PART = false>
+template <int EPI, int ITERS, int ROW_STEP, int TW = BN, bool UNAL = false, bool PART = false, bool TAPS = false>
 __device__ __forceinline__ void fast_epilogue(const GemmP& p, const float* sC, int z, long long coff, int m_first, int n0,
-                                              int row_l0) {
+                                              int row_l0, float* taps = nullptr) {
   constexpr int LDS_C = TW + 4;
+  static_assert(!TAPS || (EPI == EPI_MUL_POS && !PART && !UNAL), "tap gradients: the gated input gradient");
+  if constexpr (TAPS) {
+    const int k = threadIdx.x & (TW / 8 - 1);
+    if (k < 10) {
+#pragma unroll
+      for (int it = 0; it < ITERS; ++it) {
+        const int m = m_first + it * ROW_STEP;
+        taps[(row_l0 + it * ROW_STEP) * TAPS_LD + k] = m < p.M ? tap_value(p, m, k) : 0.f;
+      }
+    }
+  }
   constexpr bool AUX_IN = EPI == EPI_RESID || EPI == EPI_DSWISH || EPI == EPI_MUL_POS;
   const int c8 = (threadIdx.x & (TW / 8 - 1)) * 8;
   const int n = n0 + c8;
@@ -369,6 +417,13 @@
 #pragma unroll
   for (int it = 0; it < ITERS; ++it) {
     const int m = m_first + it * ROW_STEP;
+    if constexpr (TAPS) {
+      if (m >= p.M) {
+        float* dst = const_cast<float*>(sC) + (row_l0 + it * ROW_STEP) * LDS_C + c8;
+        *reinterpret_cast<float4*>(dst) = make_float4(0.f, 0.f, 0.f, 0.f);
+        *reinterpret_cast<float4*>(dst + 4) = make_float4(0.f, 0.f, 0.f, 0.f);
+      }
+    }
     if (m >= p.M) continue;
     const float4 a = ra[it], b = rb[it];
     float v[8] = {a.x + b8[0], a.y + b8[1], a.z + b8[2], a.w + b8[3], b.x + b8[4], b.y + b8[5], b.z + b8[6], b.w + b8[7]};
@@ -412,6 +467,13 @@
     } else {
 #pragma unroll
       for (int j = 0; j < 8; ++j) v[j] = aux[AUX_IN ? it : 0][j] > 0.f ? v[j] : 0.f;
+    }
+    if constexpr (TAPS) {
+      taps_round8(p, ci, v);
+      float* dst = const_cast<float*>(sC) + (row_l0 + it * ROW_STEP) * LDS_C + c8;
+      *reinterpret_cast<float4*>(dst) = make_float4(v[0], v[1], v[2], v[3]);
+      *reinterpret_cast<float4*>(dst + 4) = make_float4(v[4], v[5], v[6], v[7]);
+      continue;
     }
 #if defined(V8_EPI_ABL) && V8_EPI_ABL == 3
     asm volatile("" :: "v"(v[0]), "v"(v[1]), "v"(v[2]), "v"(v[3]), "v"(v[4]), "v"(v[5]), "v"(v[6]), "v"(v[7]), "v"(ci));
@@ -829,7 +891,7 @@
   return v;
 }
 
-template <bool TA, bool TB, bool REG = false>
+template <bool TA, bool TB, bool REG = false, bool TAPS = false>
 __device__ __forceinline__ void gemm_v2_body(const GemmP& p, bf16_t* smem2, const int bid, const int kslice, const int z
                                              , const bool direct = false
 ) {
@@ -1163,6 +1225,29 @@
     }
     return;
   }
+  if constexpr (TAPS) {
+    static_assert(3 * NT2_STAGE * 2 >= (BM2 * LDS_C + BM2 * TAPS_LD) * 4, "image + tap table");
+    float* taps = sC + BM2 * LDS_C;
+    fast_epilogue<EPI_MUL_POS, 8, 32, BN, false, false, true>(p, sC, z, coff, m0 + (threadIdx.x >> 4), n0, threadIdx.x >> 4, taps);
+    __syncthreads();
+    const int c = threadIdx.x & (BN - 1), q = threadIdx.x >> 7;
+    float tacc[10];
+#pragma unroll
+    for (int k = 0; k < 10; ++k) tacc[k] = 0.f;
+#pragma unroll 4
+    for (int i = 0; i < 64; ++i) {
+      const int row = q * 64 + i;
+      taps_fma(tacc, sC[row * LDS_C + c], taps + row * TAPS_LD);
+    }
+    __syncthreads();
+#pragma unroll
+    for (int k = 0; k < 10; ++k) sC[(q * 10 + k) * BN + c] = tacc[k];
+    __syncthreads();
+    for (int e = threadIdx.x; e < 10 * BN; e += 512)
+      p.t_part[(long long)tile_m * 10 * p.N + (long long)(e >> 7) * p.N + n0 + (e & (BN - 1))] =
+          (sC[e] + sC[10 * BN + e]) + (sC[20 * BN + e] + sC[30 * BN + e]);
+    return;
+  }
   if ((p.vec_ok & 1) && !(p.N & 3)) {
     if (n0 + BN <= p.N) {
       if (p.N & 7) fast_epilogue_any<8, 32, BN, true>(p, sC, z, coff, m0 + (threadIdx.x >> 4), n0, threadIdx.x >> 4);
@@ -1189,11 +1274,11 @@
   }
 }
 
-template <bool TA, bool TB, bool REG = false>
+template <bool TA, bool TB, bool REG = false, bool TAPS = false>
 __global__ __launch_bounds__(512) void gemm_bf16_v2_kernel(GemmP p) {
   drop_resolve(p.drop);
   extern __shared__ __attribute__((aligned(16))) bf16_t smem2[];
-  gemm_v2_body<TA, TB, REG>(p, smem2, blockIdx.x, blockIdx.y, blockIdx.z);
+  gemm_v2_body<TA, TB, REG, TAPS>(p, smem2, blockIdx.x, blockIdx.y, blockIdx.z);
 }
 
 #define GRP_MAX 40
@@ -1684,10 +1769,11 @@
   asm volatile("ds_read_b128 %0, %1 offset:%2" : "=v"(dst) : "v"(addr), "n"(OFF) : "memory");
 }
 
-template <int EPI>
+template <int EPI, bool TAPS = false>
 __device__ __forceinline__ void v8_round_fast(const GemmP& p, const float* win, const float (&b8)[8], int z, long long coff, int m_base,
                                               int hstride, int n0) {
   constexpr bool AUX_IN = EPI == EPI_RESID || EPI == EPI_DSWISH || EPI == EPI_MUL_POS;
+  static_assert(!TAPS || EPI == EPI_MUL_POS, "tap gradients: the gated input gradient");
   const int k = threadIdx.x & 31, rl0 = threadIdx.x >> 5;
   const int n = n0 + k * 8;
   const bool lin = (EPI != EPI_MUL_POS) || !p.r_on;
@@ -1718,6 +1804,13 @@
 #pragma unroll
   for (int it = 0; it < 4; ++it) {
     const int m = mrow[it];
+    if constexpr (TAPS) {
+      if (m >= p.M) {
+        float* row = const_cast<float*>(win) + (rl0 + 16 * it) * 256;
+        *reinterpret_cast<float4*>(row + (((2 * k) ^ sw) << 2)) = make_float4(0.f, 0.f, 0.f, 0.f);
+        *reinterpret_cast<float4*>(row + (((2 * k + 1) ^ sw) << 2)) = make_float4(0.f, 0.f, 0.f, 0.f);
+      }
+    }
     if (m >= p.M) continue;
     const float4 a = hi ? y[it] : x[it], b = hi ? x[it] : y[it];
     float v[8] = {a.x + b8[0], a.y + b8[1], a.z + b8[2], a.w + b8[3], b.x + b8[4], b.y + b8[5], b.z + b8[6], b.w + b8[7]};
@@ -1758,6 +1851,13 @@
 #pragma unroll
       for (int j = 0; j < 8; ++j) v[j] = aux[AUX_IN ? it : 0][j] > 0.f ? v[j] : 0.f;
     }
+    if constexpr (TAPS) {
+      taps_round8(p, ci[it], v);
+      float* row = const_cast<float*>(win) + (rl0 + 16 * it) * 256;
+      *reinterpret_cast<float4*>(row + (((2 * k) ^ sw) << 2)) = make_float4(v[0], v[1], v[2], v[3]);
+      *reinterpret_cast<float4*>(row + (((2 * k + 1) ^ sw) << 2)) = make_float4(v[4], v[5], v[6], v[7]);
+      continue;
+    }
 #if defined(V8_EPI_ABL) && V8_EPI_ABL == 3
     asm volatile("" :: "v"(v[0]), "v"(v[1]), "v"(v[2]), "v"(v[3]), "v"(v[4]), "v"(v[5]), "v"(v[6]), "v"(v[7]), "v"(ci[it]));
 #else
@@ -1770,6 +1870,8 @@
 #define V8_ES_SWISH_G 2
 #define V8_ES_DSWISH_G 3
 #define V8_ES_STORE 4
+#define V8_ES_TAPS 5
+#define V8_TAPS_LDS (256 * TAPS_LD * 4 + 2 * 10 * 256 * 4)
 template <int OFF>
 __device__ __forceinline__ void v8_rdw(f32x4& dst, uint32_t addr) {
   asm volatile("ds_read_b128 %0, %1 offset:%2" : "=v"(dst) : "v"(addr), "n"(OFF) : "memory");
@@ -1849,6 +1951,7 @@
                                              const int z) {
   const int tn = (p.N + BN4 - 1) / BN4;
   static_assert(AH == 2 || (AH == 1 && G == 0 && !TN), "the one-A-half tile: dense K-contiguous operands");
+  static_assert(ES != V8_ES_TAPS || (G == 1 && !TN && AH == 2), "tap gradients: the gathered-A 256x256 kernel");
   constexpr int BMT = 128 * AH;
   constexpr int BUF_B = (AH + 2) * V8_HALF_B;
   const int m0 = tile_m * BMT, n0 = tile_n * BN4;
@@ -1864,6 +1967,11 @@
       const int b0 = m0 / p.rows_per_b, b1 = mlast / p.rows_per_b;
       const int t0 = (m0 - b0 * p.rows_per_b) / p.rows_inner;
       if (b0 == b1 && (long long)t0 >= p.row_len[b0]) {
+        if constexpr (ES == V8_ES_TAPS) {
+          for (int e = threadIdx.x; e < 10 * BN4; e += 512)
+            p.t_part[(long long)tile_m * 10 * p.N + (long long)(e >> 8) * p.N + n0 + (e & (BN4 - 1))] = 0.f;
+          if (!p.C) return;
+        }
         bf16_t* Cz = (bf16_t*)p.C + coff;
         const int ncol = min(BN4, p.N - n0), nrow = mlast - m0 + 1, cpr = ncol >> 3;
         const u32x4 zero = {0u, 0u, 0u, 0u};
@@ -2261,6 +2369,12 @@
 #pragma unroll
       for (int j = 0; j < 8; ++j) b8[j] = 0.f;
     }
+    float tv[ES == V8_ES_TAPS ? 5 : 1];
+    if constexpr (ES == V8_ES_TAPS) {
+      const int m = m0 + (threadIdx.x >> 1), k0 = (threadIdx.x & 1) * 5;
+#pragma unroll
+      for (int j = 0; j < 5; ++j) tv[j] = m < p.M ? tap_value(p, m, k0 + j) : 0.f;
+    }
 #pragma nounroll
     for (int r = 0; r < 2 * AH; ++r) {
       f32x4 tq[2][2][2];
@@ -2282,6 +2396,29 @@
 #endif
       __syncthreads();
       const int mb = m0 + (r >> 1) * 128 + (r & 1) * 32;
+      if constexpr (ES == V8_ES_TAPS) {
+        float* taps = sC + 2 * (64 * 256);
+        float* tsum = taps + 256 * TAPS_LD;
+        v8_round_fast<EPI_MUL_POS, true>(p, win, b8, z, coff, mb, 64, n0);
+        if (r == 0) {
+#pragma unroll
+          for (int j = 0; j < 5; ++j) taps[(threadIdx.x >> 1) * TAPS_LD + (threadIdx.x & 1) * 5 + j] = tv[ES == V8_ES_TAPS ? j : 0];
+        }
+        __syncthreads();
+        const int c = threadIdx.x & 255, h = threadIdx.x >> 8;
+        float tacc[10];
+#pragma unroll
+        for (int k = 0; k < 10; ++k) tacc[k] = r ? tsum[(h * 10 + k) * 256 + c] : 0.f;
+#pragma unroll 4
+        for (int i = 0; i < 32; ++i) {
+          const int w = h * 32 + i;
+          const int row = (r >> 1) * 128 + (r & 1) * 32 + (w >> 5) * 64 + (w & 31);
+          taps_fma(tacc, win[w * 256 + ((((c >> 2) ^ (w & 7)) << 2) | (c & 3))], taps + row * TAPS_LD);
+        }
+#pragma unroll
+        for (int k = 0; k < 10; ++k) tsum[(h * 10 + k) * 256 + c] = tacc[k];
+        continue;
+      } else
       if constexpr (ES != 0) {
         static_assert(G == 0 && !TN && AH == 2, "specialised rounds: the dense NT 256x256 kernel");
 #define V8_SPEC(EPI_, DROP_) \
@@ -2302,6 +2439,12 @@
         case EPI_RELU_MASK: v8_round_fast<EPI_RELU_MASK>(p, win, b8, z, coff, mb, 64, n0); break;
         default: v8_round_fast<EPI_MUL_POS>(p, win, b8, z, coff, mb, 64, n0); break;
       }
+    }
+    if constexpr (ES == V8_ES_TAPS) {
+      const float* tsum = sC + 2 * (64 * 256) + 256 * TAPS_LD;
+      __syncthreads();
+      for (int e = threadIdx.x; e < 10 * 256; e += 512)
+        p.t_part[(long long)tile_m * 10 * p.N + (long long)(e >> 8) * p.N + n0 + (e & 255)] = tsum[e] + tsum[10 * 256 + e];
     }
   } else {
     constexpr int LDS_C = BN4 + 4;
@@ -2855,6 +2998,7 @@
   GK_V8_HALF,
   GK_V5_STORE, GK_V5_SWISH_DROP, GK_V5_RESID, GK_V5_DSWISH,
   GK_F32, GK_F32_MFMA,
+  GK_V8_NT_GA_TAPS, GK_V2_NT_TAPS,
   GK_COUNT
 };
 struct GemmPlan {
@@ -2881,8 +3025,8 @@
 static bool off_ok(long long rows, long long ld, int bits) { return rows * ld < (1LL << bits); }
 static bool dense_nt_whole(const GemmP& p) { return !p.transA && !p.transB && !p.g_on && !(p.K % BK); }
 
-static int gemm_fill(const mi355x_gemm_desc* d, GemmP* out) {
-  if (!d || !d->A || !d->B || !d->C || d->M <= 0 || d->N <= 0 || d->K <= 0) return MI_ERR_ARG;
+static int gemm_fill(const mi355x_gemm_desc* d, GemmP* out, bool c_optional = false) {
+  if (!d || !d->A || !d->B || (!d->C && !c_optional) || d->M <= 0 || d->N <= 0 || d->K <= 0) return MI_ERR_ARG;
   if (d->in_dtype != MI_DT_F32 && d->in_dtype != MI_DT_BF16) return MI_ERR_ARG;
   if ((d->transA && d->lda * 64 >= (1LL << 31)) || (d->transB && d->ldb * 64 >= (1LL << 31))) return MI_ERR_ARG;
   GemmP& p = *out;
@@ -2902,6 +3046,7 @@
   p.drop = mi_drop(d->drop_key, d->drop_threshold, d->drop_scale);
   p.colsum_out = (float*)d->colsum_out; p.colsum_stride = d->colsum_stride;
   p.g_on = 0; p.r_on = 0; p.v8_delay = 0;
+  p.t_mel = nullptr; p.t_len0 = nullptr; p.t_part = nullptr; p.t_F = p.t_T = p.t_pad = 0;
   if (d->gather) {
     const mi355x_conv_gather& g = *d->gather;
     if (d->in_dtype != MI_DT_BF16 || g.C <= 0 || (g.C & 7) || g.ntaps < 1 || g.ntaps > 9 || g.nI <= 0 || g.nJ <= 0 ||
@@ -3066,7 +3211,8 @@
       (const void*)gemm_bf16_v8_kernel<0, false, 1>,
       (const void*)gemm_bf16_v5_kernel<EPI_STORE>, (const void*)gemm_bf16_v5_kernel<EPI_SWISH_DROP>,
       (const void*)gemm_bf16_v5_kernel<EPI_RESID>, (const void*)gemm_bf16_v5_kernel<EPI_DSWISH>,
-      (const void*)gemm_f32_kernel, (const void*)gemm_f32_mfma_kernel};
+      (const void*)gemm_f32_kernel, (const void*)gemm_f32_mfma_kernel,
+      (const void*)gemm_bf16_v8_kernel<1, false, 2, V8_ES_TAPS>, (const void*)gemm_bf16_v2_kernel<false, false, false, true>};
   static std::atomic<int> attr[GK_COUNT];
   const void* fn = kernels[pl.kernel];
   if (!lds_attr_once(attr[pl.kernel], fn, pl.lds)) { (void)hipGetLastError(); return MI_ERR_LAUNCH; }
@@ -3100,6 +3246,79 @@
   const int v[8] = {pl.kernel, pl.path, pl.gx, pl.gy, pl.gz, pl.block, pl.lds, pl.v8_delay};
   for (int i = 0; i < 8; ++i) out[i] = v[i];
   return MI_OK;
+}
+
+static int taps_fill_plan(const mi355x_gemm_desc* d, const mi355x_conv1_taps* t, GemmP* p, GemmPlan* pl) {
+  if (!d || !t || !t->mel || !t->len0 || !t->partial || t->F <= 0 || t->T <= 0 || t->pad < 1 || t->pad > 2 || t->part_begin < 0)
+    return MI_ERR_ARG;
+  int rc = gemm_fill(d, p, true);
+  if (rc != MI_OK) return rc;
+  if (d->in_dtype != MI_DT_BF16 || p->epi != EPI_MUL_POS || !p->r_on || p->g_on != 1 || p->atomic || p->bias || p->splitk > 1 ||
+      p->c_dt != MI_DT_BF16 || p->auxin_dt != MI_DT_BF16 || !(p->vec_ok & 1) || (p->N % BN4) || p->r_si != 2 || p->r_sj != 2)
+    return MI_ERR_ARG;
+  const int T1 = (t->T + t->pad - 2) / 2 + 1, F1 = (t->F + t->pad - 2) / 2 + 1;
+  if (p->r_OI != T1 || p->r_OJ != F1 || t->B != p->M / (p->r_nI * p->r_nJ)) return MI_ERR_ARG;
+  if ((p->r_nI - 1) * 2 + p->r_oi >= T1 || (p->r_nJ - 1) * 2 + p->r_oj >= F1 || p->r_oi < 0 || p->r_oj < 0) return MI_ERR_ARG;
+  *pl = gemm_plan(*p, true, gemm_modes_now());
+  if (pl->kernel == GK_NONE) return MI_ERR_ARG;
+  if (pl->kernel == GK_V8_NT_GA) { pl->kernel = GK_V8_NT_GA_TAPS; pl->lds += V8_TAPS_LDS; }
+  else if (pl->kernel == GK_V2_NT) pl->kernel = GK_V2_NT_TAPS;
+  else {
+    *pl = GemmPlan{};
+    pl->kernel = GK_V2_NT_TAPS; pl->gx = cdiv(p->M, BM2) * cdiv(p->N, BN); pl->gy = 1; pl->gz = 1; pl->block = 512;
+    pl->lds = 3 * NT2_STAGE * 2;
+  }
+  if ((long long)(t->part_begin + cdiv(p->M, BM2)) * 10 * p->N > t->partial_elems) return MI_ERR_ARG;
+  p->t_mel = (const float*)t->mel; p->t_len0 = (const long long*)t->len0;
+  p->t_part = (float*)t->partial + (long long)t->part_begin * 10 * p->N;
+  p->t_F = t->F; p->t_T = t->T; p->t_pad = t->pad;
+  p->v8_delay = pl->v8_delay;
+  return MI_OK;
+}
+extern "C" int mi355x_gemm_conv1_taps(const mi355x_gemm_desc* d, const mi355x_conv1_taps* t, void* stream) {
+  mi_clear_errors();
+  g_last_path = 0;
+  GemmP p;
+  GemmPlan pl;
+  int rc = taps_fill_plan(d, t, &p, &pl);
+  if (rc != MI_OK) return rc;
+  rc = gemm_launch(pl, p, (hipStream_t)stream);
+  if (rc != MI_OK) return rc;
+  g_last_path = pl.path;
+  return mi_check_launch();
+}
+extern "C" int mi355x_gemm_conv1_taps_plan(const mi355x_gemm_desc* d, const mi355x_conv1_taps* t, int out[8]) {
+  GemmP p;
+  GemmPlan pl;
+  const int rc = taps_fill_plan(d, t, &p, &pl);
+  if (rc != MI_OK) return rc;
+  const int v[8] = {pl.kernel, pl.path, pl.gx, pl.gy, pl.gz, pl.block, pl.lds, pl.v8_delay};
+  for (int i = 0; i < 8; ++i) out[i] = v[i];
+  return MI_OK;
+}
+#define TAPS_FOLD 64
+static __global__ __launch_bounds__(256) void taps_fold_kernel(const float* __restrict__ partial, int nparts, int n, float* __restrict__ out) {
+  const int e = blockIdx.x * 256 + threadIdx.x;
+  if (e >= n) return;
+  const int per = (nparts + gridDim.y - 1) / gridDim.y;
+  const int p0 = blockIdx.y * per, p1 = min(nparts, p0 + per);
+  float a0 = 0.f, a1 = 0.f, a2 = 0.f, a3 = 0.f;
+  int q = p0;
+  for (; q + 4 <= p1; q += 4) {
+    a0 += partial[(long long)(q + 0) * n + e]; a1 += partial[(long long)(q + 1) * n + e];
+    a2 += partial[(long long)(q + 2) * n + e]; a3 += partial[(long long)(q + 3) * n + e];
+  }
+  for (; q < p1; ++q) a0 += partial[(long long)q * n + e];
+  out[(long long)blockIdx.y * n + e] = (a0 + a1) + (a2 + a3);
+}
+extern "C" int mi355x_conv1_taps_reduce(const void* partial, int nparts, int C, void* fold, long long fold_elems, void* dw, void* db,
+                                        void* stream) {
+  mi_clear_errors();
+  if (!partial || !fold || !dw || !db || nparts <= 0 || C <= 0 || fold_elems < (long long)TAPS_FOLD * 10 * C) return MI_ERR_ARG;
+  hipStream_t s = (hipStream_t)stream;
+  MI_LAUNCH(taps_fold_kernel, dim3((10 * C + 255) / 256, TAPS_FOLD), dim3(256), 0, s, (const float*)partial, nparts, 10 * C, (float*)fold);
+  MI_LAUNCH(tap_reduce_kernel, dim3((10 * C + 255) / 256, 1), dim3(256), 0, s, (const float*)fold, TAPS_FOLD, 9, C, (float*)dw, (float*)db);
+  return mi_check_launch();
 }
 
 static int group_tiles(GroupP& g, int bn) {
diff --git a/nemo_amd/csrc/subsample.hip b/nemo_amd/csrc/subsample.hip
--- a/nemo_amd/csrc/subsample.hip
+++ b/nemo_amd/csrc/subsample.hip
@@ -81,10 +81,7 @@
   const int tlim = (int)min((long long)T, len0[b]);
   for (int i = threadIdx.x; i < FW * TW; i += 256) {
     const int fi = i / TW, tt = i - fi * TW;
-    const int f = fi - pad, t = tbase + tt;
-    float v = 0.f;
-    if (f >= 0 && f < F && t >= 0 && t < tlim) v = mel[((long long)b * F + f) * T + t];
-    mel_s[i] = v;
+    mel_s[i] = conv1_mel_at(mel, b, fi - pad, tbase + tt, F, T, tlim);
   }
   __syncthreads();
   const int wave = __builtin_amdgcn_readfirstlane(threadIdx.x >> 6), lane = threadIdx.x & 63;
diff --git a/nemo_amd/modules/conformer_encoder.py b/nemo_amd/modules/conformer_encoder.py
--- a/nemo_amd/modules/conformer_encoder.py
+++ b/nemo_amd/modules/conformer_encoder.py
@@ -296,6 +296,7 @@
         self.posproj_side = os.environ.get("MI355X_POSPROJ_SIDE", "1") != "0"
         self._wg_pending, self._wg_rows = None, None
         self.conv2_implicit = os.environ.get("MI355X_CONV2_IMPLICIT", "1") != "0"
+        self.conv1_bwd_fused = os.environ.get("MI355X_CONV1_BWD_FUSED", "1") != "0"
         self.fuse_bn_dwconv_bwd = os.environ.get("MI355X_BN_DW_FUSE", "1") != "0"
         self.fuse_glu_dwconv_bwd = os.environ.get("MI355X_GLU_DW_FUSE", "1") != "0"
         self.tap_reduce_side = os.environ.get("MI355X_TAP_REDUCE_SIDE", "1") != "0"
@@ -1730,8 +1731,27 @@
             ops.gemm(dout2, col, pe.conv[2].weight.grad, C_, C_, M2, C_, 9 * C_, 9 * C_, transA=True, transB=True,
                      atomic=True, splitk=self._splitk(tiles, M2), batch=9, nb0=9, sB=(C_, 0), sC=(1, 0), c_col_stride=9,
                      c_dtype=ops.F32)
-        dout1 = self._buf("dout1", (B, T1, F1, C_), cdt, dev)
-        if self.conv2_implicit and self._conv2_implicit(cdt, C_, M2):
+        implicit_d = self.conv2_implicit and self._conv2_implicit(cdt, C_, M2)
+        fused = self.conv1_bwd_fused and implicit_d and cdt == torch.bfloat16 and pe._pad == 1 and C_ % 256 == 0
+        dout1 = None if fused else self._buf("dout1", (B, T1, F1, C_), cdt, dev)
+        if fused:
+            classes = [(pt, pf, (T1 - pt + 1) // 2, (F1 - pf + 1) // 2) for pt in (0, 1) for pf in (0, 1)]
+            nparts = sum((B * nI * nJ + 255) // 256 for _, _, nI, nJ in classes)
+            part = ops.conv1_taps_scratch(nparts, C_, dev)
+            begin = 0
+            for pt, pf, nI, nJ in classes:
+                slots = self._dgrad_slots(pt, pf, pe._pad)
+                name = f"pre.w2d{pt}{pf}"
+                ops.gemm(dout2, W[name], None, B * nI * nJ, C_, len(slots) * C_, C_, W.pitch(name), C_, c_dtype=ops.BF16,
+                         epi=ops.EPI_MUL_POS, aux_in=S.out1, ldaux=C_, row_len=S.len2 if self.pad_tile_skip else None,
+                         rows_per_b=nI * nJ, rows_inner=nJ,
+                         gather=dict(nI=nI, nJ=nJ, SI=T2, SJ=F2, C=C_, si=1, sj=1,
+                                     taps=[((pt + pe._pad - kh) // 2, (pf + pe._pad - kw) // 2) for kh, kw in slots]),
+                         rowmap=dict(nI=nI, nJ=nJ, OI=T1, OJ=F1, si=2, sj=2, oi=pt, oj=pf),
+                         taps=dict(mel=S.mel, len0=S.len0, pad=pe._pad, partial=part, part_begin=begin))
+                begin += (B * nI * nJ + 255) // 256
+            ops.conv1_taps_reduce(part, nparts, C_, pe.conv[0].weight.grad, pe.conv[0].bias.grad)
+        elif implicit_d:
             for pt in (0, 1):
                 for pf in (0, 1):
                     nI, nJ = (T1 - pt + 1) // 2, (F1 - pf + 1) // 2
@@ -1747,7 +1767,8 @@
             dcol = self._buf("dcol", (M2, 9 * C_), cdt, dev)
             ops.gemm(dout2, W["pre.w2t"], dcol, M2, 9 * C_, C_, C_, W.pitch("pre.w2t"), 9 * C_)
             ops.col2im_relu(dcol, S.out1, dout1, B, T1, F1, C_, pad=pe._pad)
-        ops.conv1_bwd(dout1, S.mel, S.len0, pe.conv[0].weight.grad, pe.conv[0].bias.grad, C_, pad=pe._pad)
+        if not fused:
+            ops.conv1_bwd(dout1, S.mel, S.len0, pe.conv[0].weight.grad, pe.conv[0].bias.grad, C_, pad=pe._pad)
         self._wgrad_join()
         if self.grad_ready_hook is not None:
             self._hook(*fp.range_of("pre_encode."))
diff --git a/nemo_amd/ops.py b/nemo_amd/ops.py
--- a/nemo_amd/ops.py
+++ b/nemo_amd/ops.py
@@ -6,7 +6,7 @@
 
 import torch
 
-from ._lib import ConvGather, GemmDesc, PackEntry, RowMap, check, lib
+from ._lib import Conv1Taps, ConvGather, GemmDesc, PackEntry, RowMap, check, lib
 
 F32, BF16 = 0, 1
 EPI_STORE, EPI_SWISH_DROP, EPI_RESID, EPI_DSWISH, EPI_RELU_MASK, EPI_MUL_POS, EPI_SWISH_DROP_G, EPI_DSWISH_G = range(8)
@@ -112,12 +112,12 @@
          sA=(0, 0), sB=(0, 0), sC=(0, 0), bias=None, alpha=1.0, epi=EPI_STORE, atomic=False, splitk=1, aux_in=None,
          aux_out=None, ldaux=0, drop: Dropout = NO_DROP, row_len=None, rows_per_b=1, rows_inner=1,
          a_off=0, b_off=0, c_off=0, c_col_stride=1, colsum_out=None, colsum_off=0, colsum_stride=0, gather=None,
-         rowmap=None):
+         rowmap=None, taps=None):
     d = GemmDesc()
-    esA, esC = A.element_size(), Cm.element_size()
+    esA = A.element_size()
     d.A = _ptr(A) + a_off * esA
     d.B = _ptr(B) + b_off * B.element_size()
-    d.C = _ptr(Cm) + c_off * esC
+    d.C = (_ptr(Cm) + c_off * Cm.element_size()) if Cm is not None else 0
     d.M, d.N, d.K = M, N, K
     d.lda, d.ldb, d.ldc = lda, ldb, ldc
     d.c_col_stride = c_col_stride
@@ -156,12 +156,20 @@
         r.nI, r.nJ, r.OI, r.OJ, r.si, r.sj, r.oi, r.oj = (rowmap[k] for k in ("nI", "nJ", "OI", "OJ", "si", "sj", "oi", "oj"))
         keep.append(r)
         d.rowmap = C.cast(C.pointer(r), C.c_void_p)
+    if taps is not None:
+        tp = conv1_taps_desc(taps["mel"], taps["len0"], taps["pad"], taps["partial"], taps["part_begin"])
+
+        def launch():
+            check(lib.mi355x_gemm_conv1_taps(C.byref(d), C.byref(tp), _stream()), "gemm_conv1_taps")
+    else:
+        def launch():
+            check(lib.mi355x_gemm(C.byref(d), _stream()), "gemm")
     if GEMM_PROFILE is None:
-        check(lib.mi355x_gemm(C.byref(d), _stream()), "gemm")
+        launch()
         return
     e0, e1 = torch.cuda.Event(enable_timing=True), torch.cuda.Event(enable_timing=True)
     e0.record()
-    check(lib.mi355x_gemm(C.byref(d), _stream()), "gemm")
+    launch()
     e1.record()
     variant = ("bf16" if d.in_dtype == BF16 else "f32") + "_" + ("T" if transA else "N") + ("N" if transB else "T")
     GEMM_PROFILE.append((variant, M, N, K, batch, e0, e1))
@@ -206,6 +214,24 @@
     sc = _scratch("conv1_bwd", n, dout.device)
     check(lib.mi355x_subsample_conv1_bwd_pad(_ptr(dout), dt(dout), _ptr(mel), _ptr(len0), _ptr(dw), _ptr(db), B, F, T, C_, pad,
                                              _ptr(sc), n, _stream()), "subsample_conv1_bwd")
+
+
+def conv1_taps_desc(mel, len0, pad, partial, part_begin):
+    B, F, T = mel.shape
+    tp = Conv1Taps()
+    tp.mel, tp.len0, tp.B, tp.F, tp.T, tp.pad = _ptr(mel), _ptr(len0), B, F, T, pad
+    tp.partial, tp.partial_elems, tp.part_begin = _ptr(partial), partial.numel(), part_begin
+    return tp
+
+
+def conv1_taps_scratch(nparts, C_, device):
+    return _scratch("conv1_taps", nparts * 10 * C_, device)
+
+
+def conv1_taps_reduce(partial, nparts, C_, dw, db):
+    n = 64 * 10 * C_
+    fold = _scratch("conv1_taps_fold", n, partial.device)
+    check(lib.mi355x_conv1_taps_reduce(_ptr(partial), nparts, C_, _ptr(fold), n, _ptr(dw), _ptr(db), _stream()), "conv1_taps_reduce")
 
 
 def im2col(x, col, B, T1, F1, C_, pad=1):
```

New measurement: 17730 audio-sec/s, median of 5. Within noise of the previous version (+0.1%).
